# apple/ml-stable-diffusion

Measured on AMD Instinct MI355X. Metric: diffusion iter/s (UNet steps/s), SD2.1-base 512x512 fp16, higher is better.
Workload: dtype fp16; 1 GPU; BASELINE config 2: SD2.1-base (865.9 M-parameter UNet), random-init, denoising iteration at 512x512 (64x64 latents), CFG batch 2 per prompt, DDIM, device-resident loop; unet=sd21-base, latent=64, attention=ORIGINAL, prompts_per_gpu=1, global_batch=2, hip_graph=True, parallelism=dp1 (independent prompts per rank, no data-path collective)

## Files before the change

### include/sd_mi355x.h

```cpp
#ifndef SD_MI355X_H
#define SD_MI355X_H

#include <stddef.h>
#include <stdint.h>

#ifdef __cplusplus
extern "C" {
#endif

typedef enum sd_status {
  SD_OK = 0,
  SD_ERR_INVALID_ARGUMENT = -1,
  SD_ERR_NOT_FOUND = -2,
  SD_ERR_HIP = -3,
  SD_ERR_UNSUPPORTED = -4,
  SD_ERR_INTERNAL = -5
} sd_status;

typedef enum sd_dtype { SD_F16 = 0, SD_F32 = 1 } sd_dtype;

typedef enum sd_attention_impl {
  SD_ATTN_ORIGINAL = 0,
  SD_ATTN_SPLIT_EINSUM = 1,
  SD_ATTN_SPLIT_EINSUM_V2 = 2
// ... 77 lines not shown
  const void* const* additional_residuals;
  int32_t num_additional_residuals;
  void* noise_pred;
  void* const* residual_outputs;
  int32_t flags;
  const float* step_noise;
} sd_unet_io;

int sd_unet_forward(sd_unet* u, const sd_unet_io* io);

int sd_unet_time_forward(sd_unet* u, int warmup, int iters, float* ms_per_iter);

int sd_unet_profile(sd_unet* u, int iters, int cap, float* ms, double* flop, char* labels, int label_bytes,
                    int* n_ops);

int sd_tune_set_candidate(int tile, int staging, int splitk);
int sd_tune_set_plan_table(const char* rows, sd_unet* u, int* n_plans);

int sd_unet_denoise_loop(sd_unet* u, const sd_unet_io* io, float* latents, int n_images, int n_steps,
                         const float* timesteps, const float* coef, const float* sample_scale, int history,
                         float guidance_scale, float* history_io, float* ms_per_step);

typedef int (*sd_progress_fn)(void* user, int step, int n_steps, const float* latents, const float* denoised);
int sd_unet_denoise_loop_progress(sd_unet* u, const sd_unet_io* io, float* latents, int n_images, int n_steps,
                                  const float* timesteps, const float* coef, const float* sample_scale, int history,
                                  float guidance_scale, float* history_io, float* ms_per_step,
                                  const float* pred , int every,
                                  sd_progress_fn fn, void* user, int* steps_done);

int sd_unet_attach_controlnets(sd_unet* u, sd_unet* const* controlnets, int n);
int sd_controlnet_set_cond(sd_unet* controlnet, const void* controlnet_cond, int flags);

int sd_vae_decoder_create(const sd_unet_config* cfg, const sd_weights* w, int device, sd_unet** out);
int sd_vae_decode(sd_unet* vae, const void* z, sd_dtype z_dtype, float* image, int flags);
int sd_vae_encoder_create(const sd_unet_config* cfg, const sd_weights* w, int device, sd_unet** out);
int sd_vae_encode(sd_unet* vae, const void* x, sd_dtype x_dtype, float* moments, int flags);
int sd_vae_encode_latents(sd_unet* vae_encoder, const void* x, sd_dtype x_dtype, const float* eps, const float* noise, int n_images,
                          float scale_factor, float sa, float sb, float* latents, int flags);
int sd_op_vae_attention(const void* q, const void* k, const void* v, void* out, int B, int S, int C, int iters, float* ms);

typedef struct sd_text_encoder_config {
  int32_t vocab_size, hidden_size, intermediate_size, num_hidden_layers, num_attention_heads;
  int32_t max_position_embeddings;
  int32_t hidden_act;
  int32_t projection_dim;
  float layer_norm_eps;
  int32_t use_graph;
} sd_text_encoder_config;
typedef struct sd_text_encoder sd_text_encoder;
int sd_text_encoder_create(const sd_text_encoder_config* cfg, const sd_weights* w, int device, sd_text_encoder** out);
void sd_text_encoder_destroy(sd_text_encoder* t);
size_t sd_text_encoder_device_bytes(const sd_text_encoder* t);
int sd_text_encoder_encode(sd_text_encoder* t, const int32_t* input_ids, int eos_index, float* last_hidden_state,
                           float* hidden_embeds, float* pooled);

int sd_op_attention(int impl, const void* q, const void* k, const void* v, void* out, int B, int heads, int d,
                    int Sq, int Sk, int variant, int iters, float* ms);
int sd_op_layernorm(const void* x, const float* weight, const float* bias, void* out, int B, int C, int S, float eps,
                    int iters, float* ms);
int sd_op_groupnorm(const void* x, const float* weight, const float* bias, void* out, int B, int C, int H, int W,
                    int groups, float eps, int silu, int iters, float* ms);
int sd_op_groupnorm_shortcut(const void* x0, const void* x1, const float* gn_weight, const float* gn_bias, const void* w, const float* bias,
                             void* out_gn, void* out_sc, int B, int C0, int C1, int H, int W, int N, int groups, float eps, int silu,
                             int side, int iters, float* ms);
int sd_op_conv2d(const void* x, const void* w, const float* bias, const void* res, void* out, int B, int Cin, int H,
                 int W, int Cout, int ksize, int stride, int upsample, int tile, int splitk, int force_generic,
                 int iters, float* ms);
int sd_op_conv2d_ex(const void* x, const void* x1, const void* w, const float* bias, const float* temb, const void* res, void* out, int B,
                    int Cin, int C1, int H, int W, int Cout, int ksize, int stride, int upsample, int pad_mode, int twin_groups,
                    const float* twin_gamma, const float* twin_beta, float twin_eps, int twin_silu, void* out_twin, int tile, int splitk,
                    int force_generic, int* plan_out, int iters, float* ms);
int sd_op_conv2d_palettized(const void* x, const void* x1, const void* lut, int nbits, const uint8_t* indices, const float* bias,
                            const void* res, void* out, int B, int Cin, int C1, int H, int W, int Cout, int ksize, int upsample, int nw,
                            int* plan_out, int iters, float* ms);
int sd_op_palette_pack(const uint8_t* indices, int Cout, int Ctot, int ksize, int nbits, uint8_t* stream, size_t* bytes);
int sd_op_conv2d_w8a8(const void* x, const void* x1, const int8_t* wq, const float* w_scale, float act_absmax, const float* bias,
                      const void* res, void* out, int B, int Cin, int C1, int H, int W, int Cout, int ksize, int upsample, int nw,
                      int* plan_out, int iters, float* ms);
int sd_op_w8a8_pack(const int8_t* wq, int Cout, int Ctot, int ksize, int8_t* stream, size_t* bytes);
int sd_op_conv2d_w8a8_halo(const void* x, const void* x1, const int8_t* wq, const float* w_scale, float act_absmax, const float* bias,
                           const float* temb, const void* res, void* out, int B, int Cin, int C1, int H, int W, int Cout, int upsample,
                           int staging, int splitk, int* plan_out, int iters, float* ms);
int sd_op_w8a8_pack_halo(const int8_t* wq, int Cout, int Ctot, int8_t* packed, size_t* bytes);
int sd_op_gemm_w8a8(const void* x, const int8_t* wq, const float* w_scale, float act_absmax, const float* bias, const void* res, void* out, int B,
                    int Cin, int H, int W, int Cout, int bm, int* plan_out, int iters, float* ms);
int sd_op_w8a8_pack_gemm(const int8_t* wq, int Cout, int K, int8_t* packed, size_t* bytes);
int sd_op_layernorm_q8(const void* x, const float* ln_weight, const float* ln_bias, float act_absmax, float eps, int8_t* xq, int M, int C,
                       int iters, float* ms);
int sd_op_geglu_w8a8(const int8_t* xq, const int8_t* wq, const float* w_scale, float act_absmax, const float* bias, void* out, int M, int C,
                     int N2, int bm, int* plan_out, int iters, float* ms);
int sd_op_w8a8_pack_geglu(const int8_t* wq, int N2, int K, int8_t* packed, size_t* bytes);
int sd_op_quantize_weight(const float* w, int Cout, size_t per_row, int8_t* q, float* w_scale, double* sq_err);
int sd_op_absmax(const void* x, size_t n, float* absmax);
int sd_op_gemm_palettized(const void* x, const void* lut, int nbits, const uint8_t* indices, const float* bias, const void* res, void* out,
                          int B, int Cin, int H, int W, int Cout, int bm, int* plan_out, int iters, float* ms);
int sd_op_palette_pack_gemm(const uint8_t* indices, int Cout, int K, int nbits, uint8_t* stream, size_t* bytes);
int sd_op_geglu_palettized(const void* x, const float* ln_weight, const float* ln_bias, const void* lut, int nbits, const uint8_t* indices,
                           const float* bias, void* out, int M, int C, int N2, float eps, int bm, int* plan_out, int iters, float* ms);
int sd_op_palette_pack_geglu(const uint8_t* indices, int N2, int K, int nbits, uint8_t* stream, size_t* bytes);
int sd_op_conv2d_groupnorm(const void* x, const void* w, const float* bias, const void* res, const float* gn_weight,
                           const float* gn_bias, void* conv_out, void* out, int B, int Cin, int H, int W, int Cout, int ksize,
                           int groups, float eps, int silu, int tile, int producer_stats, int* entries, int iters, float* ms);
int sd_op_conv2d_groupnorm_proj(const void* x, const void* w, const float* bias, const void* res, const float* gn_weight,
                                const float* gn_bias, const void* proj_w, const float* proj_bias, void* conv_out, void* out, int B,
                                int Cin, int H, int W, int Cout, int ksize, int Nproj, int groups, float eps, int fold, int tile,
                                int* entries, int iters, float* ms);
int sd_op_conv2d_groupnorm_conv3x3(const void* x, const void* w, const float* bias, const void* res, const float* gn_weight,
                                   const float* gn_bias, const void* w2, const float* bias2, const void* res2, void* conv_out, void* out,
                                   int B, int Cin, int H, int W, int Cout, int ksize, int N2, int groups, float eps, int silu, int fold,
                                   int tile, int staging2, int* entries, int iters, float* ms);
int sd_op_ffn_out_proj(const void* g, const void* w1, const float* b1, const void* res1, const void* w2, const float* b2, const void* res2,
                       void* out, float* gn_sums, int B, int C, int S, int groups, int fused, int iters, float* ms);
int sd_op_fold_linear(const void* wp, const float* bp, const void* w2, const float* b2, void* wm_out, float* bm_out, int N, int J, int K);
int sd_op_cross_attention_fused(const void* x, const float* ln_weight, const float* ln_bias, const void* wq, const void* k,
                                const void* v, void* out, int B, int heads, int Sq, int Sk, float eps, int nst, int iters,
                                float* ms);
int sd_op_cross_attention_block(const void* x, const float* ln_weight, const float* ln_bias, const void* wq, const void* k, const void* v,
                                const void* wo, const float* bo, const void* a1, const void* wo1, const float* bo1, void* out, int B, int heads,
                                int Sq, int Sk, float eps, int fused, int iters, float* ms);
int sd_op_geglu(const void* x, const void* w, const float* bias, void* out, int M, int C, int N2, int iters, float* ms);
int sd_op_geglu_ln(const void* x, const float* ln_weight, const float* ln_bias, const void* w, const float* bias, void* out, int M, int C,
                   int N2, float eps, int kernel, int iters, float* ms);
int sd_op_qkv_ln(const void* x, const float* ln_weight, const float* ln_bias, const void* w, void* out_qk, void* out_vt, int B, int HW, int C,
                 float eps, float q_scale, int vt_perm, int kernel, int iters, float* ms);
int sd_op_gn_proj_qkv(const void* x_in, const void* conv_w, const float* gn_weight, const float* gn_bias, const void* proj_w,
                      const float* proj_bias, const float* ln_weight, const float* ln_bias, const void* wqkv, void* out_h, void* out_qk,
                      void* out_vt, int B, int H, int W, int C, int groups, float gn_eps, float ln_eps, float q_scale, int vt_perm, int fused,
                      int* entries, int iters, float* ms);
int sd_op_timestep_embedding(const float* t, float* out, int n, int dim, int flip_sin_to_cos, float freq_shift);
int sd_op_posterior_noise(const float* moments, const float* eps, const float* noise, float* out, int Cz, int h, int w, int n_images,
                          float scale_factor, float sa, float sb, int iters, float* ms);
int sd_op_sched_step(const float* noise_pred, float* latents, float* hist, const float* coef, const float* pred, const float* step_noise,
                     float guidance, int cfg, int history, int n_images, int n, float* denoised, int* step_after);
int sd_op_conv_plan(int ksize, int stride, int up, int C0, int C1, int N, int B, int Ho, int Wo, int out_mode, int flags, int n_trans,
                    int n_twins, int gnf_groups, int tile, int staging, int splitk, int copies, int* plan, unsigned long long* workspace_bytes);
int sd_op_conv_plan_kernel(int ksize, int stride, int up, int C0, int C1, int N, int B, int Ho, int Wo, int out_mode, int flags, int n_trans,
                           int n_twins, int gnf_groups, int tile, int staging, int splitk, int copies, char* text, int text_bytes);
int sd_numpy_randn(uint32_t seed, double* out, size_t n);
int sd_torch_randn(uint32_t seed, double* out, size_t n);
int sd_philox_randn(uint64_t seed, uint32_t offset, double* out, size_t n);
int sd_calibrate(int device, float* out9);
int sd_selftest_mfma(void);

typedef struct sd_safety_checker_config {
  int32_t batch, image_size , patch_size , hidden_size, intermediate_size,
          num_hidden_layers, num_attention_heads, projection_dim, num_concepts ,
          num_special , hidden_act ;
  float layer_norm_eps;
  int32_t use_graph;
} sd_safety_checker_config;
typedef struct sd_safety_checker sd_safety_checker;
int sd_safety_checker_create(const sd_safety_checker_config* cfg, const sd_weights* w, int device, sd_safety_checker** out);
void sd_safety_checker_destroy(sd_safety_checker* c);
size_t sd_safety_checker_device_bytes(const sd_safety_checker* c);
int sd_safety_checker_run(sd_safety_checker* c, const void* clip_input, float adjustment, float* has_nsfw,
                          float* concept_scores, float* image_embeds, float* last_hidden_state, int flags);
float sd_safety_checker_last_ms(const sd_safety_checker* c);
int sd_op_vit_attention(const void* qkv, void* out, int B, int S, int heads, int d, int iters, float* ms);
int sd_op_safety_head(const float* image_embeds, const float* concept_embeds, const float* special_embeds,
                      const float* concept_w, const float* special_w, float adjustment, int B, int P,
                      int n_concepts, int n_special, float* has_nsfw, float* concept_scores);

typedef struct sd_image_post {
  int32_t resize_h, resize_w;
  float image_mean[3], image_std[3];
} sd_image_post;
// ... 27 lines not shown
```

### ml-stable-diffusion_amd/csrc/capi_ops.cpp

```cpp
#include <algorithm>
#include <climits>
#include <cmath>
#include <cstring>
#include <initializer_list>

#include "capi_util.h"
#include "conv_plan.h"
#include "weight_prep.h"

namespace sd {
namespace {

const half_t* f16(const void* p) { return reinterpret_cast<const half_t*>(p); }

half_t* upload_nhwc(Scratch& sc, const void* x, int B, int C, int H, int W) {
  const half_t* src = f16(x);
  std::vector<half_t> t((size_t)B * C * H * W);
  for (int b = 0; b < B; ++b)
    for (int c = 0; c < C; ++c)
      for (int p = 0; p < H * W; ++p) t[((size_t)b * H * W + p) * C + c] = src[((size_t)b * C + c) * H * W + p];
  return sc.dev<half_t>(t.size(), t.data());
}
half_t* upload_tokens(Scratch& sc, const void* x, int B, int C, int S) { return upload_nhwc(sc, x, B, C, 1, S); }

// ... 429 lines not shown
    conv2d_op(x, w, bias, res, out, B, Cin, H, W, Cout, ksize, stride, upsample, tile, splitk, force_generic, iters, ms, e);
  });
}

int sd_op_conv2d_palettized(const void* x, const void* x1, const void* lut, int nbits, const uint8_t* indices, const float* bias,
                            const void* res, void* out, int B, int Cin, int C1, int H, int W, int Cout, int ksize, int upsample, int nw,
                            int* plan_out, int iters, float* ms) {
  return guarded([&] {
    SD_REQUIRE(lut && indices, kInvalidArgument, "NULL argument");
    SD_REQUIRE(palette_bits_ok(nbits), kInvalidArgument, "conv2d_palettized: nbits = %d, not one of 1, 2, 4, 6, 8", nbits);
    SD_REQUIRE(nw == 0 || nw == 4 || nw == 8, kInvalidArgument, "conv2d_palettized: nw = %d, not 0, 4 or 8", nw);
    SD_REQUIRE(B > 0 && Cin > 0 && C1 >= 0 && Cout > 0 && H > 0 && W > 0, kInvalidArgument, "conv2d_palettized: empty problem");
    ConvOpExtra e;
    e.x1 = x1; e.C1 = C1;
    e.plan_out = plan_out;
    e.cw.kind = WeightSource::PalWstream; e.cw.lut = lut; e.cw.indices = indices; e.cw.bits = nbits;
    e.nw = nw;
    conv2d_op(x, nullptr, bias, res, out, B, Cin, H, W, Cout, ksize, 1, upsample, 0, 0, 0, iters, ms, e);
  });
}

int sd_op_conv2d_w8a8(const void* x, const void* x1, const int8_t* wq, const float* w_scale, float act_absmax, const float* bias,
                      const void* res, void* out, int B, int Cin, int C1, int H, int W, int Cout, int ksize, int upsample, int nw,
                      int* plan_out, int iters, float* ms) {
  return guarded([&] {
    SD_REQUIRE(x && wq && w_scale && out, kInvalidArgument, "NULL argument");
    SD_REQUIRE(nw == 0 || nw == 4 || nw == 8, kInvalidArgument, "conv2d_w8a8: nw = %d, not 0, 4 or 8", nw);
    SD_REQUIRE(B > 0 && Cin > 0 && C1 >= 0 && Cout > 0 && H > 0 && W > 0 && (C1 == 0 || x1), kInvalidArgument, "conv2d_w8a8: empty problem");
    SD_REQUIRE((ksize == 1 || ksize == 3) && (upsample == 0 || upsample == 1), kInvalidArgument, "conv2d_w8a8: ksize %d upsample %d", ksize, upsample);
    ConvDesc d;
    d.C0 = Cin;
    if (C1 > 0) d.x1 = f16(x1), d.C1 = C1;
    d.B = B; d.Hi = H; d.Wi = W; d.Ho = H * (upsample ? 2 : 1); d.Wo = W * (upsample ? 2 : 1);
    d.ksize = ksize; d.up = upsample ? 2 : 1; d.N = Cout;
    SD_REQUIRE(conv_fast_path_ok(d) && wstream_shape_ok(d), kInvalidArgument,
               "conv2d_w8a8: shape not eligible for plan tile 17 (wstream.hip: k=%d C0=%d C1=%d N=%d %dx%d)", ksize, Cin, C1, Cout, d.Ho, d.Wo);
    (void)w8a8_host_copy("conv2d_w8a8", wq, w_scale, act_absmax, Cout, Cin + C1, ksize);
    ConvOpExtra e;
    e.x1 = x1; e.C1 = C1;
    e.plan_out = plan_out;
    e.cw.kind = WeightSource::I8Wstream; e.cw.q = wq; e.cw.w_scale = w_scale; e.cw.act_absmax = act_absmax;
    e.nw = nw;
    conv2d_op(x, nullptr, bias, res, out, B, Cin, H, W, Cout, ksize, 1, upsample, 0, 0, 0, iters, ms, e);
  });
}

int sd_op_conv2d_w8a8_halo(const void* x, const void* x1, const int8_t* wq, const float* w_scale, float act_absmax, const float* bias, const float* temb,
                           const void* res, void* out, int B, int Cin, int C1, int H, int W, int Cout, int upsample, int staging, int splitk, int* plan_out,
                           int iters, float* ms) {
  return guarded([&] {
    SD_REQUIRE(x && wq && w_scale && out, kInvalidArgument, "NULL argument");
    SD_REQUIRE(B > 0 && Cin > 0 && C1 >= 0 && Cout > 0 && H > 0 && W > 0 && (C1 == 0 || x1), kInvalidArgument, "conv2d_w8a8_halo: empty problem");
    SD_REQUIRE((upsample == 0 || upsample == 1) && staging >= 0 && staging <= 5 && staging != 1 && splitk >= 0, kInvalidArgument,
               "conv2d_w8a8_halo: upsample %d staging %d (plan tile 7's ring codes 0, 2-5) splitk %d", upsample, staging, splitk);
    ConvDesc d;
    d.C0 = Cin;
    if (C1 > 0) d.x1 = f16(x1), d.C1 = C1;
    d.B = B; d.Hi = H; d.Wi = W; d.Ho = H * (upsample ? 2 : 1); d.Wo = W * (upsample ? 2 : 1);
    d.ksize = 3; d.up = upsample ? 2 : 1; d.N = Cout;
    SD_REQUIRE(conv_fast_path_ok(d) && halo_ks_ok(d), kInvalidArgument,
               "conv2d_w8a8_halo: shape not eligible for plan tile 18 (conv3x3_halo_i8.hip: C0=%d C1=%d N=%d %dx%d)", Cin, C1, Cout, d.Ho, d.Wo);
    SD_REQUIRE(Cin + C1 <= kHaloI8MaxCtot, kInvalidArgument, "conv2d_w8a8_halo: %d input channels, the exact int32 sums of plan tile 18 hold up to %d",
               Cin + C1, kHaloI8MaxCtot);
    (void)w8a8_host_copy("conv2d_w8a8_halo", wq, w_scale, act_absmax, Cout, Cin + C1, 3, WeightSource::I8Halo);
    ConvOpExtra e;
    e.x1 = x1; e.C1 = C1;
    e.temb = temb;
    e.plan_out = plan_out;
    e.cw.kind = WeightSource::I8Halo; e.cw.q = wq; e.cw.w_scale = w_scale; e.cw.act_absmax = act_absmax;
    e.nw = staging;
    conv2d_op(x, nullptr, bias, res, out, B, Cin, H, W, Cout, 3, 1, upsample, 0, splitk, 0, iters, ms, e);
  });
}

int sd_op_w8a8_pack_halo(const int8_t* wq, int Cout, int Ctot, int8_t* packed, size_t* bytes) {
  return guarded([&] {
    SD_REQUIRE(wq && bytes, kInvalidArgument, "NULL argument");
    SD_REQUIRE(Cout > 0 && Ctot > 0 && Ctot % 64 == 0, kInvalidArgument, "w8a8_pack_halo: Cout %d Ctot %d", Cout, Ctot);
    *bytes = (size_t)Cout * Ctot * 9;
    if (packed) halo_i8_pack(wq, Cout, Ctot, 3, packed);
  });
}

int sd_op_gemm_w8a8(const void* x, const int8_t* wq, const float* w_scale, float act_absmax, const float* bias, const void* res, void* out, int B,
                    int Cin, int H, int W, int Cout, int bm, int* plan_out, int iters, float* ms) {
  return guarded([&] {
    SD_REQUIRE(bm == 0 || bm == 32 || bm == 64, kInvalidArgument, "gemm_w8a8: bm = %d, not 0, 32 or 64", bm);
    SD_REQUIRE(x && wq && w_scale && out && plan_out, kInvalidArgument, "NULL argument");
    SD_REQUIRE(B > 0 && Cin > 0 && Cout > 0 && H > 0 && W > 0, kInvalidArgument, "gemm_w8a8: empty problem");
    ConvDesc d;
    d.C0 = Cin;
    d.B = B; d.Hi = H; d.Wi = W; d.Ho = H; d.Wo = W;
    d.N = Cout;
    const int code = conv_plan_pin(WeightSource::I8Gemm, bm).staging;
    SD_REQUIRE(conv_fast_path_ok(d) && smgemm_shape_ok(d, code), kInvalidArgument,
               "gemm_w8a8: shape not eligible for plan tile 19 (smgemm_i8.hip: Cin=%d Cout=%d M=%d bm=%d - Cin a multiple of 64, Cout of 80, M of the "
               "tile height, at least 2 x 2 tiles and a multiple of 8 of them)", Cin, Cout, B * H * W, bm);
    SD_REQUIRE(smgemm_i8_shape_ok(d, code), kInvalidArgument, "gemm_w8a8: K = %d, the exact int32 sums of plan tile 19 hold up to %d", Cin, kSmI8MaxK);
    (void)w8a8_host_copy("gemm_w8a8", wq, w_scale, act_absmax, Cout, Cin, 1, WeightSource::I8Gemm);
    Scratch sc;
    d.x0 = upload_nhwc(sc, x, B, Cin, H, W);
    d.bias = bias ? sc.dev<float>(Cout, bias) : nullptr;
    if (res) d.res = upload_nhwc(sc, res, B, Cout, H, W);
    half_t* dout = sc.dev<half_t>((size_t)B * H * W * Cout);
    d.out = dout;
    HostWeights h;
    h.kind = WeightSource::I8Gemm; h.q = wq; h.w_scale = w_scale; h.act_absmax = act_absmax;
    upload_compressed(sc, d, "gemm_w8a8", h, bm);
    const ConvPlan p = conv_plan(d);
    plan_out[0] = p.tile; plan_out[1] = p.staging; plan_out[2] = p.splitk; plan_out[3] = p.slab ? 1 : 0;
    ConvWorkspace ws;
    sc.timed(iters, ms, [&] { launch_conv(d, ws, sc.stream); });
    download_nchw(dout, out, B, Cout, H, W);
  });
}

int sd_op_w8a8_pack_gemm(const int8_t* wq, int Cout, int K, int8_t* packed, size_t* bytes) {
  return guarded([&] {
    SD_REQUIRE(wq && bytes, kInvalidArgument, "NULL argument");
    SD_REQUIRE(Cout > 0 && K > 0 && Cout % 16 == 0 && K % 64 == 0, kInvalidArgument, "w8a8_pack_gemm: Cout %d K %d", Cout, K);
    *bytes = smgemm_i8_bytes(Cout, K);
    if (packed) smgemm_i8_pack(wq, Cout, K, packed);
  });
}

int sd_op_layernorm_q8(const void* x, const float* ln_weight, const float* ln_bias, float act_absmax, float eps, int8_t* xq, int M, int C,
                       int iters, float* ms) {
  return guarded([&] {
    SD_REQUIRE(x && xq, kInvalidArgument, "NULL argument");
    SD_REQUIRE(M > 0 && C > 0, kInvalidArgument, "layernorm_q8: empty problem");
    SD_REQUIRE((ln_weight == nullptr) == (ln_bias == nullptr), kInvalidArgument, "layernorm_q8: ln_weight and ln_bias go together");
    SD_REQUIRE(C % 8 == 0 && C <= 2048, kInvalidArgument, "layernorm_q8: C = %d, not a multiple of 8 up to 2048", C);
    SD_REQUIRE(w8a8_absmax_ok(act_absmax), kInvalidArgument, "layernorm_q8: act_absmax = %g, not a positive finite number", (double)act_absmax);
    const float inv_s = 1.0f / (act_absmax / 127.0f);
    SD_REQUIRE(std::isfinite(inv_s) && inv_s > 0.f, kInvalidArgument, "layernorm_q8: act_absmax = %g has no finite inverse scale", (double)act_absmax);
    Scratch sc;
    const half_t* dx = sc.dev<half_t>((size_t)M * C, f16(x));
    const float* dw = ln_weight ? sc.dev<float>(C, ln_weight) : nullptr;
    const float* db = ln_bias ? sc.dev<float>(C, ln_bias) : nullptr;
    int8_t* dq = sc.dev<int8_t>((size_t)M * C);
    sc.timed(iters, ms, [&] { launch_layernorm_q8(dx, dw, db, dq, M, C, eps, inv_s, sc.stream); });
    SD_HIP(hipMemcpy(xq, dq, (size_t)M * C, hipMemcpyDeviceToHost));
  });
}

int sd_op_geglu_w8a8(const int8_t* xq, const int8_t* wq, const float* w_scale, float act_absmax, const float* bias, void* out, int M, int C,
                     int N2, int bm, int* plan_out, int iters, float* ms) {
  return guarded([&] {
    SD_REQUIRE(bm == 0 || bm == 128 || bm == 256, kInvalidArgument, "geglu_w8a8: bm = %d, not 0, 128 or 256", bm);
    SD_REQUIRE(xq && wq && w_scale && out && plan_out, kInvalidArgument, "NULL argument");
    SD_REQUIRE(M > 0 && C > 0 && N2 > 0, kInvalidArgument, "geglu_w8a8: empty problem");
    ConvDesc d = token_gemm(nullptr, C, nullptr, nullptr, nullptr, nullptr, 1, M, N2);
    d.out_mode = kOutGeglu;
    const int code = conv_plan_pin(WeightSource::I8Geglu, bm).staging;
    SD_REQUIRE(conv_fast_path_ok(d) && smgeglu_shape_ok(d, code), kInvalidArgument,
               "geglu_w8a8: shape not eligible for plan tile 20 (smgeglu_i8.hip: M=%d C=%d N2=%d bm=%d - C a multiple of 64, N2 of 160, M of the "
               "tile height, at least 2 x 2 tiles and a multiple of 8 of them)", M, C, N2, bm);
    SD_REQUIRE(smgeglu_i8_shape_ok(d, code), kInvalidArgument, "geglu_w8a8: K = %d, the exact int32 sums of plan tile 20 hold up to %d", C, kSmI8MaxK);
    (void)w8a8_host_copy("geglu_w8a8", wq, w_scale, act_absmax, N2, C, 1, WeightSource::I8Geglu);
    for (size_t i = 0; i < (size_t)M * C; ++i)
      SD_REQUIRE(xq[i] != -128, kInvalidArgument, "geglu_w8a8: activation value -128 at element %zu, the symmetric range is [-127, 127]", i);
    Scratch sc;
    d.x0_i8 = sc.dev<int8_t>((size_t)M * C, xq);
    if (bias) {
      std::vector<float> bi(N2);
      for (int o = 0; o < N2; ++o) bi[geglu_row(o, N2)] = bias[o];
// ... 631 lines not shown
    half_t* dvt = sc.dev<half_t>((size_t)B * C * HW);
    half_t* dwp_t = sc.dev<half_t>((size_t)C * C);
    half_t* dwq_t = sc.dev<half_t>((size_t)N * C);
    launch_xattn_out_retile_nk(dwp, dwp_t, C, C, sc.stream);
    launch_xattn_out_retile_nk(fq.w, dwq_t, N, C, sc.stream);
    ConvDesc pd = conv_desc(dnorm, C, dwp, dpb, nullptr, dh, B, H, W, C);
    ConvDesc qd = qkv_desc(dh, fq, ln_eps, dqk, dvt, B, H, W, C, q_scale, vt_perm);
    SD_REQUIRE(conv_fast_path_ok(d) && conv_fast_path_ok(pd) && conv_fast_path_ok(qd), kInvalidArgument, "gn_proj_qkv: off the MFMA path");
    ConvWorkspace ws = workspace_for(sc, {d, pd, qd});
    int n_entries = 0;
    static const bool want_clk = tune_env_set("SD_GQ_CLOCK");
    const size_t n_clk = (size_t)(M / 32) * 5 * 16;
    long long* dclk = want_clk && fused ? sc.dev<long long>(n_clk) : nullptr;
    sc.timed(iters, ms, [&] {
      n_entries = launch_conv(d, ws, sc.stream);
      const bool have = n_entries >= 1 && n_entries <= 128;
      if (fused) {
        GnProjQkvDesc g;
        g.clk = dclk;
        g.tok = fused == 2 ? 64 : (fused == 3 ? 32 : 0);
        g.x = dx;
        if (have) {
          g.gn_partial = partial; g.gn_gamma = dgw; g.gn_beta = dgb; g.gn_entries = n_entries;
        } else {
          launch_groupnorm(dx, C, nullptr, 0, partial, dgw, dgb, dnorm, B, HW, groups, gn_eps, 0, sc.stream, n_entries);
          g.x = dnorm;
        }
        g.gn_groups = groups; g.gn_eps = gn_eps;
        g.wp_t = dwp_t; g.p_bias = dpb; g.h = dh;
        g.wqkv_t = dwq_t; g.qkv_bias = fq.bias; g.qkv_colsum = fq.colsum; g.ln_eps = ln_eps;
        g.qk = dqk; g.vt = dvt; g.M = M; g.C = C; g.S = HW; g.ldT = HW; g.vt_perm = vt_perm != 0; g.q_scale = q_scale;
        launch_gn_proj_qkv(g, sc.stream);
      } else {
        launch_groupnorm(dx, C, nullptr, 0, partial, dgw, dgb, dnorm, B, HW, groups, gn_eps, 0, sc.stream, n_entries);
        launch_conv(pd, ws, sc.stream);
        launch_conv(qd, ws, sc.stream);
      }
    });
    if (entries) *entries = (fused && n_entries >= 1 && n_entries <= 128) ? n_entries : 0;
    if (dclk) {
      std::vector<long long> hc(n_clk);
      SD_HIP(hipMemcpy(hc.data(), dclk, n_clk * sizeof(long long), hipMemcpyDeviceToHost));
      static const char* names[13] = {"start -> group statistics folded", "-> constants in LDS", "-> normalised tile in LDS", "-> proj_in MFMAs issued",
                                      "-> h tile in LDS", "-> q MFMAs", "-> q stored", "-> k MFMAs", "-> k stored", "-> v MFMAs", "-> V^T stored", "", ""};
      const size_t nw = n_clk / 16;
      double total = 0;
      for (int ph = 1; ph <= 11; ++ph) {
        double sum = 0, mx = 0;
        for (size_t w = 0; w < nw; ++w) {
          const double dlt = (double)(hc[w * 16 + ph] - hc[w * 16 + ph - 1]);
          sum += dlt;
          mx = std::max(mx, dlt);
        }
        total += sum / nw;
        fprintf(stderr, "gn_proj_qkv phase %2d  mean %8.0f  max %8.0f cycles   %s\n", ph, sum / nw, mx, names[ph - 1]);
      }
      fprintf(stderr, "gn_proj_qkv mean wave %8.0f cycles (%zu waves; the XCDs' counters are not synchronised: no launch-wide span)\n", total, nw);
    }
    SD_HIP(hipMemcpy(out_h, dh, (size_t)M * C * 2, hipMemcpyDeviceToHost));
    SD_HIP(hipMemcpy(out_qk, dqk, (size_t)M * 2 * C * 2, hipMemcpyDeviceToHost));
    SD_HIP(hipMemcpy(out_vt, dvt, (size_t)B * C * HW * 2, hipMemcpyDeviceToHost));
  });
}

static ConvPlan query_conv_plan(int ksize, int stride, int up, int C0, int C1, int N, int B, int Ho, int Wo, int out_mode, int flags, int n_trans,
                                int n_twins, int gnf_groups, int tile, int staging, int splitk, int copies, ConvWeightCopies& c) {
  SD_REQUIRE(ksize >= 1 && stride >= 1 && up >= 1 && C0 >= 1 && C1 >= 0 && N >= 1 && B >= 1 && Ho >= 1 && Wo >= 1 &&
                 n_trans >= 0 && n_twins >= 0 && n_twins <= 2 && gnf_groups >= 0 && copies >= -1 && copies <= 7,
             kInvalidArgument, "bad conv_plan arguments");
  static const float present[4] = {};
  const half_t* ph = reinterpret_cast<const half_t*>(present);
  ConvDesc d;
  d.x0 = d.w = ph;
  d.C0 = C0;
  if (C1 > 0) d.x1 = ph, d.C1 = C1;
  d.B = B; d.Ho = Ho; d.Wo = Wo; d.Hi = Ho * stride / up; d.Wi = Wo * stride / up;
  d.ksize = ksize; d.stride = stride; d.up = up; d.N = N; d.out_mode = out_mode;
  if (flags & 1) d.ln_colsum = present;
  if (flags & 2) d.temb = present;
  if (flags & 4) d.res = ph;
  if (flags & 8) d.gn_partial = const_cast<float*>(present), d.gn_groups = 32;
  if (flags & 16) d.bias = present;
  if (flags & 32) d.pad = 0;
  if (n_trans > 0) d.out_t = const_cast<half_t*>(ph), d.n_trans = n_trans, d.ldT = Ho * Wo;
  d.n_twins = n_twins;
  if (gnf_groups > 0) {
    d.gnf_partial = d.gnf_gamma = d.gnf_beta = present;
    d.gnf_groups = gnf_groups;
    d.gnf_entries = 1;
    d.gnf_silu = ksize == 3 ? 1 : 0;
  }
  d.tile = tile; d.staging = staging; d.splitk = splitk;
  if (tile == 17) {
    d.w = nullptr;
    d.cw.kind = WeightSource::I8Wstream;
    d.cw.stream = d.cw.scale = present;
    d.cw.inv_s = 1.f;
  }
  if (tile == 18) {
    d.w = nullptr;
    d.cw.kind = WeightSource::I8Halo;
    d.cw.stream = d.cw.scale = present;
    d.cw.inv_s = 1.f;
  }
  if (tile == 19) {
    d.w = nullptr;
    d.cw.kind = WeightSource::I8Gemm;
    d.cw.stream = d.cw.scale = present;
    d.cw.inv_s = 1.f;
  }
  if (tile == 20) {
    d.w = nullptr;
    d.cw.kind = WeightSource::I8Geglu;
    d.cw.stream = d.cw.scale = present;
    d.cw.inv_s = 1.f;
    d.x0_i8 = reinterpret_cast<const int8_t*>(present);
  }
  c = conv_plan_copies(d);
  if (copies < 0) copies = (c.wstream ? 1 : 0) | (c.wsgemm ? 2 : 0) | (c.bvgemm ? 4 : 0);
  if (copies & 1) d.w_tiled = ph;
  if (copies & 2) d.w_ws = ph;
  if (copies & 4) d.w_bv = ph;
  return conv_plan(d);
}

int sd_op_conv_plan(int ksize, int stride, int up, int C0, int C1, int N, int B, int Ho, int Wo, int out_mode, int flags, int n_trans,
                    int n_twins, int gnf_groups, int tile, int staging, int splitk, int copies, int* plan, unsigned long long* workspace_bytes) {
  return guarded([&] {
    SD_REQUIRE(plan && workspace_bytes, kInvalidArgument, "bad conv_plan arguments");
    ConvWeightCopies c;
    const ConvPlan p = query_conv_plan(ksize, stride, up, C0, C1, N, B, Ho, Wo, out_mode, flags, n_trans, n_twins, gnf_groups, tile, staging, splitk, copies, c);
    plan[0] = p.tile; plan[1] = p.staging; plan[2] = p.splitk; plan[3] = p.slab ? 1 : 0;
    plan[4] = c.wstream ? 1 : 0; plan[5] = c.wsgemm ? 1 : 0; plan[6] = c.bvgemm ? 1 : 0;
    *workspace_bytes = p.workspace_bytes;
  });
}

int sd_op_conv_plan_kernel(int ksize, int stride, int up, int C0, int C1, int N, int B, int Ho, int Wo, int out_mode, int flags, int n_trans,
                           int n_twins, int gnf_groups, int tile, int staging, int splitk, int copies, char* text, int text_bytes) {
  return guarded([&] {
    SD_REQUIRE(text && text_bytes >= 1, kInvalidArgument, "bad conv_plan_kernel arguments");
    ConvWeightCopies c;
    const std::string name = conv_plan_kernel_name(
        query_conv_plan(ksize, stride, up, C0, C1, N, B, Ho, Wo, out_mode, flags, n_trans, n_twins, gnf_groups, tile, staging, splitk, copies, c));
    SD_REQUIRE((int)name.size() < text_bytes, kInvalidArgument, "conv_plan_kernel: the text buffer holds %d bytes, the line needs %zu", text_bytes, name.size() + 1);
    memcpy(text, name.c_str(), name.size() + 1);
  });
}

int sd_op_timestep_embedding(const float* t, float* out, int n, int dim, int flip_sin_to_cos, float freq_shift) {
  return guarded([&] {
    SD_REQUIRE(t && out && n > 0 && dim > 0 && dim % 2 == 0, kInvalidArgument, "bad arguments");
    SD_REQUIRE(flip_sin_to_cos == 1, kUnsupported, "flip_sin_to_cos=False is not on the path");
    Scratch sc;
    float* dt = sc.dev<float>(n, t);
    float* dout = sc.dev<float>((size_t)n * dim);
    std::vector<float> f = timestep_freq_table(dim, freq_shift);
    float* df = sc.dev<float>(f.size(), f.data());
    launch_timestep_embedding(dt, df, dout, n, dim, sc.stream);
    SD_HIP(hipStreamSynchronize(sc.stream));
    SD_HIP(hipMemcpy(out, dout, (size_t)n * dim * sizeof(float), hipMemcpyDeviceToHost));
  });
}

int sd_op_posterior_noise(const float* moments, const float* eps, const float* noise, float* out, int Cz, int h, int w, int n_images,
                          float scale_factor, float sa, float sb, int iters, float* ms) {
// ... 440 lines not shown
```

### ml-stable-diffusion_amd/csrc/conv_plan.cpp

```cpp
#include "conv_plan.h"

#include <algorithm>
#include <cstring>

namespace sd {

namespace {

constexpr int BK = kConvBK;

struct Dims {
  int Ctot, M, N, K, HoWo, nk_total, tiles_x, tiles_y;
};
Dims dims_of(const ConvDesc& d) {
  Dims a;
  a.Ctot = d.C0 + (d.x1 ? d.C1 : 0);
  a.M = d.B * d.Ho * d.Wo;
  a.N = d.N;
  a.K = d.ksize * d.ksize * a.Ctot;
  a.HoWo = d.Ho * d.Wo;
  a.nk_total = a.K / BK;
  a.tiles_x = cdiv(d.Wo, 16);
  a.tiles_y = cdiv(d.Ho, 8);
  return a;
// ... 104 lines not shown
    tile_dims(c, bm, bn);
    if (geglu && c != 1 && c != 4) return false;
    if (d.out_t && d.n_trans % bn != 0) return false;
    return true;
  };
  if (!tile_ok(p.tile)) p.tile = 0;
  auto blocks_of = [&](int c) {
    int bm, bn;
    tile_dims(c, bm, bn);
    const long mt = is_halo(c) ? (long)d.B * a.tiles_x * a.tiles_y : cdiv(a.M, bm);
    return mt * cdiv(a.N, bn);
  };
  auto ksteps = [&](int c) { return is_halo(c) ? a.Ctot / BK : a.nk_total; };
  auto max_split = [&](int c) {
    const int per_min = is_halo(c) ? 2 : 16;
    int s = 1;
    while (split_ok && s < 16 && ksteps(c) / (s * 2) >= per_min) s *= 2;
    return s;
  };
  const bool pinned = p.tile != 0 || p.splitk != 0 || p.staging != 0 || i8_halo(d);
  if (i8_halo(d)) p.tile = 7;
  if (!pinned && g_tune.tile != 0 && tile_ok(g_tune.tile)) {
    p.tile = g_tune.tile;
    p.staging = g_tune.staging;
    p.splitk = g_tune.splitk;
  } else if (!pinned) {
    auto match = [&](const TunedConv& t) { return table_match(t, d, a) && tile_ok(t.tile); };
    const TunedConv* hit = nullptr;
    for (const TunedConv& t : runtime_table())
      if (!hit && match(t)) hit = &t;
    for (int i = 0; i < kNumTuned && !hit; ++i)
      if (match(kTuned[i])) hit = &kTuned[i];
    if (hit) {
      p.tile = hit->tile;
      p.staging = hit->staging;
      p.splitk = hit->splitk;
    }
  }
  if (p.tile == 0 && tile_ok(9) && d.ksize == 3 && a.HoWo <= 64 && a.M <= 256) p.tile = 9;
  if (p.tile == 9) {
    p.splitk = 1;
    return p;
  }
  if (p.tile == 0 && tile_ok(7)) {
    p.tile = 7;
    if (p.staging == 0) p.staging = 3;
  }
  if (p.tile == 0) {
    p.tile = 3;
    for (int c : {1, 2, 4, 3}) {
      if (!tile_ok(c)) continue;
      if (blocks_of(c) * max_split(c) >= 384 || c == 3) { p.tile = c; break; }
    }
    if (!tile_ok(p.tile)) p.tile = 4;
  }
  if (p.splitk == 0) {
    p.splitk = 1;
    const int ms = max_split(p.tile);
    const long want = p.tile == 7 ? 192 : 384;
    while (blocks_of(p.tile) * p.splitk < want && p.splitk < ms) p.splitk *= 2;
  }
  if (!split_ok) p.splitk = 1;
  if (p.splitk > ksteps(p.tile)) p.splitk = ksteps(p.tile);
  if (p.splitk < 1) p.splitk = 1;
  return p;
}

bool plan_is_wstream(const ConvDesc& d0) {
  if (!wstream_shape_ok(d0)) return false;
  ConvDesc d = d0;
  static const half_t present = 0;
  d.w_tiled = &present;
  return choose_plan(d, dims_of(d)).tile == 9;
}

}

bool halo_ks_ok(const ConvDesc& d) {
  const int c1 = d.x1 ? d.C1 : 0;
  return d.ksize == 3 && d.stride == 1 && (d.up == 1 || d.up == 2) && d.pad < 0 && d.out_mode == kOutHalf && d.Wo >= 8 && d.Ho >= 8 &&
         d.C0 % BK == 0 && c1 % BK == 0 && d.N % 4 == 0;
}

bool gemm_pipe_ok(int ksize, int stride, int up, int M, int N, int K, int C0, int C1) {
  const size_t lim = (size_t)1 << 31;
  return ksize == 1 && stride == 1 && up == 1 && (size_t)M * std::max(C0, C1) * 2 < lim && (size_t)N * K * 2 < lim;
}

bool conv_fast_path_ok(const ConvDesc& d) {
  const int c1 = d.x1 ? d.C1 : 0;
  if (d.C0 % BK != 0 || c1 % BK != 0) return false;
  if (d.N % 4 != 0) return false;
  if (d.out_mode == kOutGeglu && d.N % 64 != 0) return false;
  if (!(d.ksize == 1 || d.ksize == 3)) return false;
  if (!(d.up == 1 || d.up == 2)) return false;
  return true;
}

namespace {

ConvPlan plan_codes(const ConvDesc& d) {
  const CompressedWeights& cw = d.cw;
  if (i8_halo(d))
    SD_REQUIRE(conv_fast_path_ok(d) && cw.stream && cw.scale && halo_i8_ok(d), kInvalidArgument,
               "plan tile 18 (conv3x3_halo_i8.hip, int8) needs the int8 weights, the scales and a 3x3 / stride-1 shape of the halo conv with "
               "at most %d input channels (k=%d stride=%d up=%d C0=%d C1=%d N=%d)", kHaloI8MaxCtot, d.ksize, d.stride, d.up, d.C0, d.x1 ? d.C1 : 0, d.N);
  if (i8_gemm(d))
    SD_REQUIRE(conv_fast_path_ok(d) && cw.stream && cw.scale && d.staging >= 0 && d.staging <= 2 && smgemm_i8_shape_ok(d, d.staging), kInvalidArgument,
               "plan tile 19 (smgemm_i8.hip, int8) needs the int8 weights, the scales and a single-source shape of the small-M GEMM with K <= %d "
               "(k=%d C0=%d C1=%d N=%d M=%d mode=%d)", kSmI8MaxK, d.ksize, d.C0, d.x1 ? d.C1 : 0, d.N, d.B * d.Ho * d.Wo, d.out_mode);
  if (i8_geglu(d))
    SD_REQUIRE(conv_fast_path_ok(d) && cw.stream && cw.scale && d.staging >= 0 && d.staging <= 2 && smgeglu_i8_shape_ok(d, d.staging), kInvalidArgument,
               "plan tile 20 (smgeglu_i8.hip, int8) needs the int8 weights, the scales and an un-folded shape of the GEGLU kernel with K <= %d "
               "(k=%d C0=%d C1=%d N=%d M=%d mode=%d ln=%d)", kSmI8MaxK, d.ksize, d.C0, d.x1 ? d.C1 : 0, d.N, d.B * d.Ho * d.Wo, d.out_mode, d.ln_colsum ? 1 : 0);
  if (!conv_fast_path_ok(d)) return ConvPlan{-1, 0, 1, false, 0};
  switch (cw.kind) {
    case WeightSource::Fp16: break;
    case WeightSource::PalWstream:
    case WeightSource::I8Wstream: {
      const bool i8 = i8_stream(d);
      SD_REQUIRE(cw.stream && (i8 ? cw.scale != nullptr : cw.lut != nullptr) && can_split(d) && wstream_shape_ok(d), kInvalidArgument, "%s",
                 i8 ? "plan tile 17 (wstream.hip, int8) needs the int8 stream, the scales and a shape of the weight stream"
                    : "plan tile 14 (wstream.hip, palettized) needs the index stream, the LUT and a shape of the weight stream");
      ConvPlan r{i8 ? 17 : 14, d.staging, 1, true, 0};
      r.splitk = wstream_splits(d, wstream_waves(d.staging));
      r.workspace_bytes = slab_bytes(dims_of(d), r.splitk, true);
      return r;
    }
    case WeightSource::I8Halo: {
      const Dims a = dims_of(d);
      const Plan p = choose_plan(d, a);
      ConvPlan r{18, p.staging, 1, true, 0};
      const int steps = a.Ctot / BK;
      r.splitk = cdiv(steps, cdiv(steps, p.splitk));
      r.slab = r.splitk > 1 || d.n_twins > 0;
      r.workspace_bytes = slab_bytes(a, r.splitk, r.slab);
      return r;
    }
    case WeightSource::PalGemm:
      SD_REQUIRE(cw.stream && cw.lut && palette_bits_ok(cw.bits) && !d.x1 && d.staging >= 0 && d.staging <= 2 && smgemm_shape_ok(d, d.staging), kInvalidArgument,
                 "plan tile 15 (smgemm.hip, palettized) needs the index stream, the LUT and a single-source shape of the small-M GEMM");
      return ConvPlan{15, smgemm_bm(d, d.staging) == 32 ? 1 : 2, 1, false, 0};
    case WeightSource::I8Gemm:
      return ConvPlan{19, smgemm_bm(d, d.staging) == 32 ? 1 : 2, 1, false, 0};
    case WeightSource::PalGeglu:
      SD_REQUIRE(cw.stream && cw.lut && palette_bits_ok(cw.bits) && (cw.ln_gamma != nullptr) == (d.ln_colsum != nullptr) && smgeglu_pal_shape_ok(d, d.staging),
                 kInvalidArgument,
                 "plan tile 16 (smgeglu.hip, palettized) needs the index stream, the LUT, the norm weight with the LayerNorm fold and a shape of "
                 "the GEGLU kernel with 128-row tiles");
      return ConvPlan{16, 1, 1, false, 0};
    case WeightSource::I8Geglu:
      return ConvPlan{20, smgeglu_bm(d, d.staging) == 128 ? 1 : 2, 1, false, 0};
  }
  const Switches& sw = switches();
  const bool free_choice = d.tile == 0 && d.splitk == 0 && d.staging == 0 && g_tune.tile == 0;
  if (d.w_ws && wsgemm_shape_ok(d) && (d.tile == 10 || (sw.wsgemm && free_choice && wsgemm_wanted(d)))) return ConvPlan{10, 0, 1, false, 0};
  SD_REQUIRE(d.tile != 10, kInvalidArgument, "plan tile 10 (wsgemm.hip) needs the pre-tiled weights and an eligible GEGLU shape");
  if (sw.bvgemm && d.w_bv && free_choice && bvgemm_wanted(d)) return ConvPlan{11, 0, 1, false, 0};
  if (d.tile == 11) {
    SD_REQUIRE(d.w_bv && bvgemm_shape_ok(d), kInvalidArgument, "plan tile 11 (bvgemm.hip) needs the pre-tiled weights and an eligible 1x1 shape");
    return ConvPlan{11, d.staging, 1, false, 0};
  }
  if (d.tile == 12 || (sw.smgemm && free_choice && smgemm_wanted(d))) return ConvPlan{12, d.tile == 12 ? d.staging : 0, 1, false, 0};
  if (d.tile == 13 || (sw.smgeglu && free_choice && smgeglu_wanted(d))) return ConvPlan{13, d.tile == 13 ? d.staging : 0, 1, false, 0};

  const Dims a = dims_of(d);
  Plan p = choose_plan(d, a);
  const bool twins = d.n_twins > 0;
  if (d.gnf_partial && d.ksize == 3) {
    SD_REQUIRE(conv_gn_loader_ok(d) && d.gnf_silu == 1 && d.gnf_gamma && d.gnf_beta && d.gnf_entries >= 1 && d.gnf_entries <= 128 && !twins, kInvalidArgument,
               "GroupNorm in the conv loader: Ctot=%d groups=%d entries=%d up=%d", a.Ctot, d.gnf_groups, d.gnf_entries, d.up);
    p.tile = 7;
    if (p.staging != 2 && p.staging != 3) p.staging = 3;
    p.splitk = 1;
  } else if (d.gnf_partial) {
    SD_REQUIRE(d.ksize == 1 && d.stride == 1 && !d.x1 && d.out_mode == kOutHalf && !d.ln_colsum && !d.out_t && !twins &&
                   gemm_pipe_ok(d.ksize, d.stride, d.up, a.M, a.N, a.K, d.C0, 0) &&
                   d.gnf_gamma && d.gnf_beta && d.gnf_groups >= 1 && d.gnf_groups <= 32 && a.K % d.gnf_groups == 0 && a.K <= 2048 &&
                   d.gnf_entries >= 1 && d.gnf_entries <= 128 && a.HoWo % 64 == 0,
               kInvalidArgument, "GroupNorm fold: K=%d groups=%d entries=%d HoWo=%d", a.K, d.gnf_groups, d.gnf_entries, a.HoWo);
    p.tile = 3;
    if (p.staging != 6 && p.staging != 7 && p.staging != 8) p.staging = 6;
    p.splitk = 1;
  }
  ConvPlan r{p.tile, p.staging, 1, true, 0};
  if (p.tile == 9) {
    r.splitk = wstream_splits(d, wstream_waves(p.staging));
  } else {
    const int steps = p.tile == 7 ? a.Ctot / BK : a.nk_total;
    r.splitk = cdiv(steps, cdiv(steps, p.splitk));
    r.slab = r.splitk > 1 || twins;
  }
  r.workspace_bytes = slab_bytes(a, r.splitk, r.slab);
  return r;
}

void decode_plan(const ConvDesc& d, ConvPlan& p) {
  const Dims a = dims_of(d);
  int code = p.staging;
  switch (p.tile) {
    case -1: p.kernel = ConvKernel::Generic; return;
    case 9: case 14: case 17:
      p.kernel = p.tile == 9 ? ConvKernel::Wstream : p.tile == 14 ? ConvKernel::WstreamPal : ConvKernel::WstreamI8;
      p.waves = wstream_waves(code);
      return;
    case 10: p.kernel = ConvKernel::Wsgemm; return;
    case 11:
      p.kernel = ConvKernel::Bvgemm;
      p.variant = code >= 1 && code <= 6 ? code : bvgemm_auto_variant(d);
      return;
    case 12: case 15: case 19:
      p.kernel = p.tile == 12 ? ConvKernel::Smgemm : p.tile == 15 ? ConvKernel::SmgemmPal : ConvKernel::SmgemmI8;
      p.bm = code >= 0 && code <= 2 ? smgemm_bm(d, code) : 0;
      return;
    case 13: case 16: case 20:
      p.kernel = p.tile == 13 ? ConvKernel::Smgeglu : p.tile == 16 ? ConvKernel::SmgegluPal : ConvKernel::SmgegluI8;
      p.bm = code >= 0 && code <= 2 ? smgeglu_bm(d, code) : 0;
      return;
    default: break;
  }
  if (p.tile == 18) {
    tile_dims(7, p.bm, p.bn);
    p.kernel = ConvKernel::HaloI8;
    p.stages = code >= 3 ? 4 : code == 2 ? 3 : 2;
    return;
  }
  tile_dims(p.tile, p.bm, p.bn);
  if (p.tile == 7) {
    p.kernel = ConvKernel::HaloKs;
    if (d.gnf_partial) p.stages = code >= 3 && halo_gnl_lds_bytes(4, a.Ctot) <= kLdsBudget ? 4 : 3;
    else p.stages = code >= 5 ? 8 : code == 4 ? 6 : code == 3 ? 4 : code == 2 ? 3 : 2;
    return;
  }
  p.kernel = ConvKernel::Igemm;
  p.stages = 2;
  const bool lnf = d.ln_colsum != nullptr;
  auto fits = [&](int nst, int kgroups = 1) { return ring_fits(p.bm, p.bn, nst, kgroups); };
  if (lnf && code == 1) code = 0;
  if (code == 1) {
    p.reg_staged = true;
    return;
  }
  if (!lnf && d.out_mode == kOutHalfT) {
    if (code >= 2) p.stages = 3;
    return;
  }
  if (code == 12 || code == 13) {
    const bool two_groups = !lnf && cdiv(a.nk_total, p.splitk) >= 4;
    if (two_groups && code == 13 && fits(4, 2)) p.stages = 4, p.kgroups = 2;
    else if (two_groups && fits(3, 2)) p.stages = 3, p.kgroups = 2;
    if (p.kgroups == 2) return;
    code -= 10;
  }
  if (code >= 6 && code <= 8 && gemm_pipe_ok(d.ksize, d.stride, d.up, a.M, a.N, a.K, d.C0, d.x1 ? d.C1 : 0)) {
    p.kernel = ConvKernel::GemmPipe;
    p.stages = code == 8 ? 2 : (code == 7 && fits(4)) ? 4 : 3;
    return;
  }
  if (code >= 6) code = 3;
  const int asked = code >= 5 ? 8 : code == 4 ? 6 : code == 3 ? 4 : code == 2 ? 3 : 2;
  for (int nst : {8, 6, 4, 3, 2})
    if (nst <= asked && fits(nst)) {
      p.stages = nst;
      return;
    }
}

}

ConvPlan conv_plan(const ConvDesc& d) {
  ConvPlan p = plan_codes(d);
  decode_plan(d, p);
  return p;
}

std::string conv_plan_kernel_name(const ConvPlan& p) {
  const std::string tile = std::to_string(p.bm) + "x" + std::to_string(p.bn), ring = " ring" + std::to_string(p.stages);
  switch (p.kernel) {
    case ConvKernel::Igemm: return "igemm " + tile + ring + (p.kgroups == 2 ? " kg2" : "") + (p.reg_staged ? " regs" : "");
    case ConvKernel::GemmPipe: return "gemm_pipe " + tile + ring;
    case ConvKernel::HaloKs: return "halo_ks" + ring;
    case ConvKernel::HaloI8: return "halo_i8" + ring;
    case ConvKernel::Wstream: return "wstream waves" + std::to_string(p.waves);
    case ConvKernel::WstreamPal: return "wstream_pal waves" + std::to_string(p.waves);
    case ConvKernel::WstreamI8: return "wstream_i8 waves" + std::to_string(p.waves);
    case ConvKernel::Wsgemm: return "wsgemm";
    case ConvKernel::Bvgemm: return "bvgemm v" + std::to_string(p.variant);
    case ConvKernel::Smgemm: return "smgemm bm" + std::to_string(p.bm);
    case ConvKernel::SmgemmPal: return "smgemm_pal bm" + std::to_string(p.bm);
    case ConvKernel::SmgemmI8: return "smgemm_i8 bm" + std::to_string(p.bm);
    case ConvKernel::Smgeglu: return "smgeglu bm" + std::to_string(p.bm);
    case ConvKernel::SmgegluPal: return "smgeglu_pal bm" + std::to_string(p.bm);
    case ConvKernel::SmgegluI8: return "smgeglu_i8 bm" + std::to_string(p.bm);
    default: return "generic";
  }
}

size_t conv_workspace_bytes(const ConvDesc& d) {
  if (!conv_fast_path_ok(d) || pal_gemm(d) || pal_geglu(d) || i8_gemm(d) || i8_geglu(d)) return 0;
  const Dims a = dims_of(d);
  const Plan p = choose_plan(d, a);
  int splits = (switches().tuning && can_split(d)) ? std::max(p.splitk, 16) : p.splitk;
  const bool stream = can_stream(d) || ((pal_stream(d) || i8_stream(d)) && can_split(d) && wstream_shape_ok(d));
  if (stream) splits = std::max(splits, wstream_splits(d, 4));
  return slab_bytes(a, splits, d.n_twins > 0 || stream);
}

ConvWeightCopies conv_plan_copies(const ConvDesc& d0) {
  ConvWeightCopies c{false, false, false};
  if (!conv_fast_path_ok(d0)) return c;
  ConvDesc d = d0;
  d.w_tiled = d.w_ws = d.w_bv = nullptr;
  const Switches& sw = switches();
  const int k = d.ksize, M = d.B * d.Ho * d.Wo;
  const bool ws_candidate = sw.tuning ? ((k == 3 && M <= 512) || (k == 1 && M <= 128)) : plan_is_wstream(d);
  c.wstream = sw.wstream && wstream_shape_ok(d) && ws_candidate;
  c.wsgemm = sw.wsgemm && wsgemm_wanted(d);
  c.bvgemm = sw.bvgemm && !c.wsgemm && bvgemm_wanted(d);
  return c;
}

namespace {
ConvPlan fp16_plan(const ConvDesc& d0, const ConvWeightCopies& c) {
  static const half_t present = 0;
  ConvDesc d = d0;
  d.cw = CompressedWeights{};
  d.w_tiled = c.wstream ? &present : nullptr;
  d.w_ws = c.wsgemm ? &present : nullptr;
  d.w_bv = c.bvgemm ? &present : nullptr;
  return conv_plan(d);
}
}

WeightPin conv_plan_pin(WeightSource kind, int n) {
  switch (kind) {
    case WeightSource::PalWstream: return {kind, 14, n == 4 ? 4 : 0};
    case WeightSource::I8Wstream: return {kind, 17, n == 4 ? 4 : 0};
    case WeightSource::I8Halo: return {kind, 18, n};
    case WeightSource::PalGemm: return {kind, 15, n == 32 ? 1 : n == 64 ? 2 : 0};
    case WeightSource::I8Gemm: return {kind, 19, n == 32 ? 1 : n == 64 ? 2 : 0};
    case WeightSource::PalGeglu: return {kind, 16, n == 128 ? 1 : n == 256 ? 2 : 0};
    case WeightSource::I8Geglu: return {kind, 20, n == 128 ? 1 : n == 256 ? 2 : 0};
    default: return {};
  }
}

WeightPin conv_plan_weights(const ConvDesc& d, StoredWeights held, bool opt_in) {
  if (held == StoredWeights::Fp16 || !conv_fast_path_ok(d)) return {};
  const Switches& sw = switches();
  const bool palette = held == StoredWeights::Palette, one_by_one = opt_in && palette && d.ksize == 1 && !d.x1;
  if (one_by_one && d.out_mode == kOutGeglu && sw.smgeglu) {
    const ConvPlan p = fp16_plan(d, conv_plan_copies(d));
    if (p.kernel == ConvKernel::Smgeglu && smgeglu_pal_shape_ok(d, 0)) return conv_plan_pin(WeightSource::PalGeglu, p.bm);
  }
  if (opt_in && held == StoredWeights::W8A8 && d.ksize == 1 && !d.x1 && d.out_mode == kOutGeglu && sw.smgeglu) {
    const ConvPlan p = fp16_plan(d, conv_plan_copies(d));
    ConvDesc plain = d;
    plain.ln_colsum = nullptr;
    if (p.kernel == ConvKernel::Smgeglu && smgeglu_i8_shape_ok(plain, p.bm == 128 ? 1 : 2)) return conv_plan_pin(WeightSource::I8Geglu, p.bm);
  }
  if (sw.wstream && !d.ln_colsum && plan_is_wstream(d)) {
    const ConvPlan p = fp16_plan(d, {true, false, false});
    if (p.kernel == ConvKernel::Wstream) return conv_plan_pin(palette ? WeightSource::PalWstream : WeightSource::I8Wstream, p.waves);
  }
  if (one_by_one && d.out_mode == kOutHalf && sw.smgemm && !d.ln_colsum) {
    const ConvPlan p = fp16_plan(d, conv_plan_copies(d));
    if (p.kernel == ConvKernel::Smgemm) return conv_plan_pin(WeightSource::PalGemm, p.bm);
  }
  if (opt_in && held == StoredWeights::W8A8 && d.ksize == 1 && !d.x1 && d.out_mode == kOutHalf && sw.smgemm && !d.ln_colsum) {
    const ConvPlan p = fp16_plan(d, conv_plan_copies(d));
    if (p.kernel == ConvKernel::Smgemm && smgemm_i8_shape_ok(d, 0)) return conv_plan_pin(WeightSource::I8Gemm, p.bm);
  }
  if (held == StoredWeights::W8A8 && halo_i8_ok(d)) {
    const ConvPlan p = fp16_plan(d, conv_plan_copies(d));
    if (p.kernel == ConvKernel::HaloKs) {
      WeightPin pin = conv_plan_pin(WeightSource::I8Halo, p.staging);
      pin.splitk = p.splitk;
      return pin;
    }
  }
  return {};
}

bool conv_plan_is_tuned(const ConvDesc& d) {
  if (!conv_fast_path_ok(d)) return false;
  const Dims a = dims_of(d);
  for (int i = 0; i < kNumTuned; ++i)
    if (table_match(kTuned[i], d, a)) return true;
  return false;
}

int conv_plan_table_set(const char* text) {
  std::vector<TunedConv>& t = runtime_table();
  t.clear();
  if (!text) return 0;
  const char* p = text;
  while (*p) {
    const char* e = strchr(p, '\n');
    std::string line(p, e ? (size_t)(e - p) : strlen(p));
    TunedConv r;
    if (parse_plan_row(line.c_str(), r)) t.push_back(r);
    if (!e) break;
    p = e + 1;
  }
  return (int)t.size();
}

void conv_tune_set_candidate(int tile, int staging, int splitk) {
  g_tune.tile = tile;
  g_tune.staging = staging;
  g_tune.splitk = splitk;
}

void conv_plan_log(const ConvDesc& d, const ConvPlan& p, int n_fast) {
  static const bool on = tune_env_set("SD_LOG_CONVS");
  if (!on) return;
  const Dims a = dims_of(d);
  const int c1 = d.x1 ? d.C1 : 0;
  if (p.tile == 9 || p.tile == 14 || p.tile == 17)
    fprintf(stderr, "[sd conv] k%d up%d C0=%d C1=%d M=%d N=%d K=%d tile=%d nw=%d slabs=%d twins=%d bits=%d\n", d.ksize, d.up, d.C0, c1, a.M, a.N,
            a.K, p.tile, p.waves, p.splitk, d.n_twins, p.tile == 14 ? d.cw.bits : p.tile == 17 ? 8 : 16);
  else if (p.tile == 12 || p.tile == 13)
    fprintf(stderr, "[sd conv] k1 s1 up1 C0=%d C1=%d M=%d N=%d K=%d mode=%d tile=%d bm=%d n_fast=%d\n", d.C0, c1, a.M, a.N, a.K, d.out_mode, p.tile, p.bm,
            n_fast);
  else if (p.tile == 15 || p.tile == 16)
    fprintf(stderr, "[sd conv] k1 s1 up1 C0=%d C1=%d M=%d N=%d K=%d mode=%d tile=%d bm=%d n_fast=%d bits=%d\n", d.C0, c1, a.M, a.N, a.K, d.out_mode,
            p.tile, p.bm, n_fast, d.cw.bits);
  else if (p.tile == 19 || p.tile == 20)
    fprintf(stderr, "[sd conv] k1 s1 up1 C0=%d C1=%d M=%d N=%d K=%d mode=%d tile=%d bm=%d n_fast=%d bits=8\n", d.C0, c1, a.M, a.N, a.K, d.out_mode, p.tile,
            p.bm, n_fast);
  else if (p.tile == 18)
    fprintf(stderr, "[sd conv] k%d s%d up%d C0=%d C1=%d M=%d N=%d K=%d mode=%d tile=%d splitk=%d bits=8\n", d.ksize, d.stride, d.up, d.C0, c1, a.M, a.N,
            a.K, d.out_mode, p.tile, p.splitk);
  else
    fprintf(stderr, "[sd conv] k%d s%d up%d C0=%d C1=%d M=%d N=%d K=%d mode=%d tile=%d splitk=%d\n", d.ksize, d.stride, d.up, d.C0, c1, a.M, a.N,
            a.K, d.out_mode, p.tile, p.splitk);
}

bool choose_tile_order(double a_bytes, double w_bytes, double nbm, double nbn, bool ab_switch) {
  const double l2 = 3.5e6;
  const double m_fast_cost = w_bytes + a_bytes * (a_bytes <= l2 ? std::min(8.0, nbn) : nbn);
  const double n_fast_cost = a_bytes + w_bytes * (w_bytes <= l2 ? std::min(8.0, nbm) : nbm);
  static const int forced = tune_env_int("SD_TILE_ORDER", -1);
  if (ab_switch && forced == 2) return nbn > 1 && a_bytes * (nbn - 1) > 7.0 * w_bytes;
  if (ab_switch && forced >= 0) return forced != 0;
  return nbn > 1 && n_fast_cost < m_fast_cost;
}

bool conv_reduce_stats_on() { return switches().reduce_stats; }

}
```

### ml-stable-diffusion_amd/csrc/conv_plan.h

```cpp
#pragma once
#include <string>

#include "kernels.h"

namespace sd {

enum class ConvKernel { Generic, Igemm, GemmPipe, HaloKs, HaloI8, Wstream, WstreamPal, WstreamI8, Wsgemm, Bvgemm, Smgemm, SmgemmPal, SmgemmI8, Smgeglu, SmgegluPal, SmgegluI8 };

struct ConvPlan {
  int tile;
  int staging;
  int splitk;
  bool slab;
  size_t workspace_bytes;
  ConvKernel kernel = ConvKernel::Generic;
  int bm = 0, bn = 0;
  int stages = 0;
  int kgroups = 1;
  bool reg_staged = false;
  int waves = 0;
  int variant = 0;
};
ConvPlan conv_plan(const ConvDesc& d);

struct ConvWeightCopies {
  bool wstream, wsgemm, bvgemm;
};
ConvWeightCopies conv_plan_copies(const ConvDesc& d);

enum class StoredWeights { Fp16, Palette, W8A8 };
struct WeightPin {
  WeightSource kind = WeightSource::Fp16;
  int tile = 0, staging = 0;
  int splitk = 0;
};
WeightPin conv_plan_weights(const ConvDesc& d, StoredWeights held, bool opt_in);
WeightPin conv_plan_pin(WeightSource kind, int n);

void conv_plan_log(const ConvDesc& d, const ConvPlan& p, int n_fast = 0);

std::string conv_plan_kernel_name(const ConvPlan& p);

bool choose_tile_order(double a_bytes, double w_bytes, double nbm, double nbn, bool ab_switch);

bool conv_reduce_stats_on();

constexpr int kConvBK = 64;
bool halo_ks_ok(const ConvDesc& d);
bool gemm_pipe_ok(int ksize, int stride, int up, int M, int N, int K, int C0, int C1);

constexpr size_t kLdsBudget = 160 * 1024;
constexpr size_t ring_bytes(int bm, int bn, int nst) { return (size_t)nst * (bm + bn) * kConvBK * sizeof(half_t); }
constexpr bool ring_fits(int bm, int bn, int nst, int kgroups = 1) { return kgroups * ring_bytes(bm, bn, nst) + 2 * bn * sizeof(float) <= kLdsBudget; }
constexpr int kHaloLdsRows = 184;
constexpr size_t halo_lds_bytes(int bn, int d) {
  return ((size_t)2 * kHaloLdsRows * kConvBK + (size_t)d * bn * kConvBK) * sizeof(half_t) + bn * sizeof(float);
}
constexpr size_t halo_gnl_lds_bytes(int d, int ctot) {
  const size_t k_loop = halo_lds_bytes(64, d) - 64 * sizeof(float) + (((size_t)6 * ctot + 15) & ~(size_t)15);
  const size_t epilogue = 32 * 1024 + 128 * (64 + 8) * 2 + 64 * sizeof(float);
  return k_loop > epilogue ? k_loop : epilogue;
}
constexpr int kHaloI8Pitch = 20, kHaloI8Rows = 204;
constexpr size_t halo_i8_lds_bytes(int d) {
  return (size_t)kHaloLdsRows * kConvBK * sizeof(half_t) + (size_t)2 * kHaloI8Rows * kConvBK + (size_t)d * 64 * kConvBK + 2 * 64 * sizeof(float);
}
constexpr int kHaloI8MaxCtot = 14784;
static_assert(127LL * 127 * 9 * kHaloI8MaxCtot < (1LL << 31) && 127LL * 127 * 9 * (kHaloI8MaxCtot + 64) >= (1LL << 31), "int32 bound of plan tile 18");
constexpr int kSmI8MaxK = 133120;
static_assert(127LL * 127 * kSmI8MaxK < (1LL << 31) && 127LL * 127 * (kSmI8MaxK + 64) >= (1LL << 31), "int32 bound of plan tile 19");

}
```

### ml-stable-diffusion_amd/csrc/igemm.hip

```cpp
#include "igemm_device.h"

namespace sd {

namespace {

template <int BM, int BN, int WGM, int WGN, bool TRANS_OUT, bool GLDS, int NST, int DBG = 0, bool LNF = false, int KG = 1>
__global__ __launch_bounds__(256 * KG) void igemm_kernel(IgemmArgs a) {
  static_assert(WGM * WGN == 4, "4 waves");
  static_assert(KG == 1 || (KG == 2 && GLDS && NST >= 3 && !LNF && !TRANS_OUT && DBG == 0), "in-workgroup split-K: ring variants of the plain epilogue");
  static_assert(!(LNF && TRANS_OUT), "LayerNorm fold uses the in-lane row layout of the non-transposed tile");
  constexpr int TM = BM / WGM / 32;
  constexpr int TN = BN / WGN / 32;
  constexpr int XR = BM / 32;
  constexpr int WR = BN / 32;
  constexpr int ROW = GLDS ? BK : LDS_ROW;

  const bool prof = (DBG & 4) && blockIdx.x == 0 && blockIdx.y == 0 && threadIdx.x == 0;
  long long prof_t[4];
  long long prof_w0 = 0;
  if (prof) { prof_t[0] = clock64(); prof_w0 = wall_clock64(); }
  extern __shared__ __attribute__((aligned(16))) char smem[];
  const int kg = KG > 1 ? __builtin_amdgcn_readfirstlane((int)threadIdx.x >> 8) : 0;
  half_t* Xs = reinterpret_cast<half_t*>(smem) + (size_t)kg * NST * (BM + BN) * ROW;
  half_t* Ws = Xs + NST * BM * ROW;
// ... 926 lines not shown
int launch_slab_combine(const ConvDesc& d, IgemmArgs& a, hipStream_t s) {
  a.gn_partial = nullptr;
  if (conv_reduce_stats_on() && d.gn_partial && d.gn_groups >= 1 && d.gn_groups <= 256 && a.N % d.gn_groups == 0 && (a.N / d.gn_groups) % 4 == 0 &&
      a.HoWo <= 256 && d.out_mode == kOutHalf && !d.out_t) {
    int ppb = std::max(1, a.B * a.HoWo / 512);
    const int slabs = cdiv(a.HoWo, ppb);
    const size_t lds = (size_t)ppb * (a.N / 4) * 2 * sizeof(float);
    if (slabs <= kGnMaxSlabs && lds <= 64 * 1024) {
      a.gn_partial = d.gn_partial;
      a.gn_G = d.gn_groups;
      a.gn_cpg = a.N / d.gn_groups;
      a.gn_T = slabs;
      hipLaunchKernelGGL(splitk_reduce_stats_kernel, dim3(slabs, a.B), dim3(256), lds, s, a, ppb);
      return slabs;
    }
  }
  const size_t total4 = (size_t)a.M * a.N / 4;
  const int blocks = (int)std::min<size_t>((total4 + 255) / 256, 2048);
  hipLaunchKernelGGL(splitk_reduce_kernel, dim3(blocks), dim3(256), 0, s, a);
  return 0;
}

half_t* g_zero_chunk = nullptr;

}

const half_t* device_zero_chunk() {
  if (!g_zero_chunk) {
    SD_HIP(hipMalloc(reinterpret_cast<void**>(&g_zero_chunk), 256));
    SD_HIP(hipMemset(g_zero_chunk, 0, 256));
    SD_HIP(hipDeviceSynchronize());
  }
  return g_zero_chunk;
}

const half_t* zero_chunk() {
  SD_REQUIRE(g_zero_chunk, kInternal, "conv launch before any handle allocated the zero chunk (device_zero_chunk)");
  return g_zero_chunk;
}

int launch_conv(const ConvDesc& d, const ConvWorkspace& ws, hipStream_t s) {
  SD_REQUIRE(conv_fast_path_ok(d), kInvalidArgument, "launch_conv: shape not MFMA-tileable (C0=%d C1=%d N=%d k=%d)",
             d.C0, d.C1, d.N, d.ksize);
  SD_REQUIRE(!d.ln_colsum || (d.ksize == 1 && !d.x1 && d.bias && d.out_mode != kOutHalfT), kInvalidArgument,
             "LayerNorm fold needs a 1x1 single-source GEMM with a (folded) bias");
  SD_REQUIRE(!d.out_t || (d.out_mode == kOutHalf && d.n_trans % 64 == 0 && d.n_trans < d.N && (d.Ho * d.Wo) % 8 == 0 &&
                          d.ldT % 8 == 0 && !d.res && !d.temb),
             kInvalidArgument, "fused q|k|v: n_trans %d N %d HoWo %d ldT %d", d.n_trans, d.N, d.Ho * d.Wo, d.ldT);
  SD_REQUIRE(!d.vt_perm || (d.out_t && (d.Ho * d.Wo) % 16 == 0), kInvalidArgument, "permuted V^T needs the fused q|k|v epilogue and HoWo %% 16 == 0");
  SD_REQUIRE(d.q_cols == 0 || (d.out_t && d.q_cols % 4 == 0 && d.q_cols <= d.n_trans), kInvalidArgument, "pre-scaled queries need the fused q|k|v epilogue (q_cols %d)", d.q_cols);
  const ConvPlan p = conv_plan(d);
  switch (p.kernel) {
    case ConvKernel::Wsgemm: launch_wsgemm(d, s); return 0;
    case ConvKernel::Bvgemm: launch_bvgemm(d, p, s); return 0;
    case ConvKernel::Smgemm: launch_smgemm(d, p, s); return 0;
    case ConvKernel::Smgeglu: launch_smgeglu(d, p, s); return 0;
    case ConvKernel::SmgegluPal: launch_smgeglu_pal(d, p, s); return 0;
    case ConvKernel::SmgemmPal: launch_smgemm_pal(d, p, s); return 0;
    case ConvKernel::SmgemmI8: launch_smgemm_i8(d, p, s); return 0;
    case ConvKernel::SmgegluI8: launch_smgeglu_i8(d, p, s); return 0;
    default: break;
  }
  IgemmArgs a = planned_args(d, p, ws.partial);
  const bool twins = d.n_twins > 0;
  SD_REQUIRE(!twins || (d.out_mode == kOutHalf && !d.ln_colsum && !d.out_t && !d.debug && reduce_twin_ok(a.HoWo, a.N, d.n_twins, d.twin)),
             kInvalidArgument, "GroupNorm twins need a plain fp16 output and whole (sample, group) slices (HoWo=%d N=%d)", a.HoWo, a.N);
  const bool have_ws = !p.slab || (ws.partial && ws.partial_bytes >= p.workspace_bytes);
  if (p.kernel == ConvKernel::Wstream || p.kernel == ConvKernel::WstreamPal || p.kernel == ConvKernel::WstreamI8) SD_REQUIRE(have_ws, kInternal, "wstream workspace too small (%zu < %zu)", ws.partial_bytes, p.workspace_bytes);
  SD_REQUIRE(have_ws, kInternal, "split-K workspace too small (%zu < %zu)", ws.partial_bytes, p.workspace_bytes);
  conv_plan_log(d, p);
  int gn_entries = 0;
  switch (p.kernel) {
    case ConvKernel::Wstream:
      launch_wstream(d, ws.partial, p.waves, s);
      break;
    case ConvKernel::WstreamPal:
      launch_wstream_pal(d, ws.partial, p.waves, s);
      break;
    case ConvKernel::WstreamI8:
      launch_wstream_i8(d, ws.partial, p.waves, s);
      break;
    case ConvKernel::HaloKs: gn_entries = launch_halo_ks(d, p, ws.partial, s); break;
    case ConvKernel::HaloI8: gn_entries = launch_halo_i8(d, p, ws.partial, s); break;
    case ConvKernel::Igemm:
    case ConvKernel::GemmPipe: {
      const bool trans = d.out_mode == kOutHalfT;
      set_tile_order(a, p.bm, p.bn);
      if (d.debug && d.debug < 64) {
        const bool ok = p.bm == 128 && p.bn == 128 ? launch_debug_mode<128, 128>(a, d.debug, s) : launch_debug_mode<64, 64>(a, d.debug, s);
        SD_REQUIRE(ok && !trans, kInvalidArgument, "no ablation kernel for debug mode %d", d.debug);
        return 0;
      }
      if (!trans) gn_entries = setup_gn_stats(d, a, p.bm);
      if (p.bm == 128 && p.bn == 128) launch_tile<128, 128>(a, p, trans, s);
      else if (p.bm == 128) launch_tile<128, 64>(a, p, trans, s);
      else if (p.bn == 64) launch_tile<64, 64>(a, p, trans, s);
      else launch_tile<64, 128>(a, p, trans, s);
      break;
    }
    default: SD_REQUIRE(false, kInternal, "launch_conv: plan '%s' has no launcher here", conv_plan_kernel_name(p).c_str());
  }
  if (twins) {
    launch_reduce_twin(a.partial, a.splitk, a.M, a.N, a.HoWo, a.bias, a.temb, a.temb_stride, a.res, a.out, d.n_twins, d.twin, s);
  } else if (a.slab) {
    gn_entries = launch_slab_combine(d, a, s);
  }
  SD_HIP(hipGetLastError());
  return gn_entries;
}

bool gn_side_gemm_ok(const ConvDesc& d) {
  if (!(d.ksize == 1 && d.stride == 1 && d.up == 1 && d.out_mode == kOutHalf && !d.ln_colsum && !d.out_t && d.n_twins == 0 && !d.gnf_partial &&
        !d.gn_partial && !d.temb && !d.debug && conv_fast_path_ok(d)))
    return false;
  const int M = d.B * d.Ho * d.Wo, c1 = d.x1 ? d.C1 : 0;
  return gemm_pipe_ok(d.ksize, d.stride, d.up, M, d.N, d.C0 + c1, d.C0, c1) && M >= 256;
}

namespace {
constexpr int kSideD = 4;
IgemmArgs side_args(const ConvDesc& d) {
  SD_REQUIRE(gn_side_gemm_ok(d), kInvalidArgument, "side GEMM: not a plain 1x1 GEMM of the pipelined kernel (C0=%d C1=%d N=%d)", d.C0, d.C1, d.N);
  IgemmArgs a = make_args(d);
  a.splitk = 1;
  a.slab = 0;
  set_tile_order(a, 64, 64);
  return a;
}
constexpr size_t kSideLds = (size_t)kSideD * (64 + 64) * BK * sizeof(half_t) + 2 * 64 * sizeof(float);
}

void launch_gn_apply_side(const half_t* x0, int C0, const half_t* x1, int C1, const float* partial, int entries, const float* gamma,
                          const float* beta, half_t* y, int B, int HW, int G, float eps, int silu, int slabs, int ppb, const ConvDesc& side,
                          hipStream_t s) {
  IgemmArgs a = side_args(side);
  GnSideArgs g{x0, x1, C0, x1 ? C1 : 0, partial, entries, gamma, beta, y, HW, G, eps, silu, ppb, slabs, B, 0};
  g.n_gn_pad = (slabs * B + 7) / 8 * 8;
  auto k = gn_apply_side_kernel<kSideD>;
  static DynLdsOnce once;
  once.set(k, kSideLds);
  hipLaunchKernelGGL(k, dim3(g.n_gn_pad + cdiv(a.M, 64) * cdiv(a.N, 64)), dim3(256), kSideLds, s, g, a);
  SD_HIP(hipGetLastError());
}

void launch_gn_fused_side(int vw, const half_t* x0, int C0, const half_t* x1, int C1, const float* gamma, const float* beta, half_t* y, int B,
                          int HW, int G, float eps, int silu, const ConvDesc& side, hipStream_t s) {
  IgemmArgs a = side_args(side);
  GnSideArgs g{x0, x1, C0, x1 ? C1 : 0, nullptr, 0, gamma, beta, y, HW, G, eps, silu, 0, G, B, 0};
  g.n_gn_pad = (G * B + 7) / 8 * 8;
  const dim3 grid(g.n_gn_pad + cdiv(a.M, 64) * cdiv(a.N, 64));
  static DynLdsOnce o8, o4, o2;
  if (vw == 8) {
    auto k = gn_fused_side_kernel<8, kSideD>;
    o8.set(k, kSideLds);
    hipLaunchKernelGGL(k, grid, dim3(256), kSideLds, s, g, a);
  } else if (vw == 4) {
    auto k = gn_fused_side_kernel<4, kSideD>;
    o4.set(k, kSideLds);
    hipLaunchKernelGGL(k, grid, dim3(256), kSideLds, s, g, a);
  } else {
    auto k = gn_fused_side_kernel<2, kSideD>;
    o2.set(k, kSideLds);
    hipLaunchKernelGGL(k, grid, dim3(256), kSideLds, s, g, a);
  }
  SD_HIP(hipGetLastError());
}
// ... 3 lines not shown
```

### ml-stable-diffusion_amd/csrc/igemm_device.h

```cpp
#pragma once
#include <cstdio>
#include <cstdlib>
#include <cstring>
#include <string>
#include <type_traits>

#include "conv_plan.h"

namespace sd {

const half_t* zero_chunk();

int launch_halo_ks(const ConvDesc& d, const ConvPlan& p, float* partial, hipStream_t s);
int launch_halo_i8(const ConvDesc& d, const ConvPlan& p, float* partial, hipStream_t s);

namespace {

constexpr int BK = kConvBK;
constexpr int LDS_ROW = BK + 8;

struct IgemmArgs {
  const half_t* x0;
  const half_t* x1;
  const half_t* w;
  const float* bias;
  const float* temb;
  const half_t* res;
  half_t* out;
  float* partial;
  int C0, C1, Ctot;
  int B, Hi, Wi, Ho, Wo, HoWo;
  int ksize, stride, up, pad;
  int M, N, K;
  int temb_stride;
  int nk_total, nk_per_split, splitk;
  int slab;
  int out_mode, ldT;
  int debug;
  long long* prof;
  const half_t* zeros;
  int tiles_x, tiles_y;
  const float* ln_colsum;
  float ln_eps;
  int n_trans, ldo;
  half_t* out_t;
  int vt_perm;
  int res_pre;
  float* gn_partial;
  int gn_G, gn_cpg, gn_T;
  int n_fast;
  const float* gnf_partial;
  const float* gnf_gamma;
  const float* gnf_beta;
  float gnf_eps;
  int gnf_G, gnf_entries;
  float q_scale;
  int q_cols;
};

constexpr int kGnScratchFloats = 256 * 17;

template <int BN>
__device__ __forceinline__ void tile_gn_stats(const IgemmArgs& a, float* scratch, const float (&fs)[8], const float (&fq)[8],
                                              int n_blk, int b, int mt) {
  constexpr int OWC = BN / 8;
  const int tid = threadIdx.x;
  float* chan = scratch + kGnScratchFloats;
#pragma unroll
  for (int e = 0; e < 8; ++e) {
    scratch[tid * 17 + e] = fs[e];
    scratch[tid * 17 + 8 + e] = fq[e];
  }
  __syncthreads();
  for (int cc = tid; cc < 2 * BN; cc += 256) {
    const int which = cc / BN, ch = cc - which * BN;
    const int cl = ch >> 3, e = ch & 7;
    float s = 0.f;
#pragma unroll 4
    for (int k = 0; k < 256 / OWC; ++k) s += scratch[(k * OWC + cl) * 17 + which * 8 + e];
    chan[cc] = s;
  }
  __syncthreads();
  const int g0 = n_blk / a.gn_cpg;
  const int g = g0 + tid;
  const int n_end = min(n_blk + BN, a.N);
  if (tid < BN && g < a.gn_G && g * a.gn_cpg < n_end) {
    const int gs = g * a.gn_cpg, ge = gs + a.gn_cpg;
    const int lo = max(gs, n_blk), hi = min(ge, n_end);
    float s = 0.f, q = 0.f;
    for (int c = lo; c < hi; ++c) {
      s += chan[c - n_blk];
      q += chan[BN + c - n_blk];
    }
    float* dst = a.gn_partial + (((size_t)b * a.gn_G + g) * kGnMaxSlabs + (size_t)mt * 2) * 2;
    if (gs < n_blk) {
      dst[2] = s;
      dst[3] = q;
// ... 352 lines not shown
```

### ml-stable-diffusion_amd/csrc/kernels.h

```cpp
#pragma once
#include "sd_common.h"

namespace sd {

enum OutMode : int {
  kOutHalf = 0,
  kOutHalfT = 1,
  kOutGeglu = 2,
};

struct GnTwin {
  half_t* y = nullptr;
  int ld = 0, c_off = 0;
  int cpg = 0;
  const float* gamma = nullptr;
  const float* beta = nullptr;
  float eps = 1e-5f;
  int silu = 0;
};

enum class WeightSource { Fp16, PalWstream, PalGemm, PalGeglu, I8Wstream, I8Halo, I8Gemm, I8Geglu };
struct CompressedWeights {
  WeightSource kind = WeightSource::Fp16;
  const void* stream = nullptr;
  const half_t* lut = nullptr;
  int bits = 0;
  const float* ln_gamma = nullptr;
  const float* scale = nullptr;
  float inv_s = 0.f;
  bool palettized() const { return kind == WeightSource::PalWstream || kind == WeightSource::PalGemm || kind == WeightSource::PalGeglu; }
  const uint8_t* pal() const { return palettized() ? static_cast<const uint8_t*>(stream) : nullptr; }
  bool int8() const { return kind == WeightSource::I8Wstream || kind == WeightSource::I8Halo || kind == WeightSource::I8Gemm || kind == WeightSource::I8Geglu; }
  const int8_t* i8() const { return int8() ? static_cast<const int8_t*>(stream) : nullptr; }
};

struct ConvDesc {
  const half_t* x0 = nullptr;
  const half_t* x1 = nullptr;
  const int8_t* x0_i8 = nullptr;
  int C0 = 0, C1 = 0;
  const half_t* w = nullptr;
  const float* bias = nullptr;
  const float* temb = nullptr;
  int temb_stride = 0;
  const half_t* res = nullptr;
  half_t* out = nullptr;
  int B = 1, Hi = 1, Wi = 1;
  int Ho = 1, Wo = 1;
  int ksize = 1, stride = 1, up = 1;
  int pad = -1;
  int N = 0;
  int out_mode = kOutHalf;
  int ldT = 0;
  int tile = 0;
  int splitk = 0;
  long long* prof = nullptr;
  int debug = 0;
  int staging = 0;
  const float* ln_colsum = nullptr;
  float ln_eps = 1e-5f;
  half_t* out_t = nullptr;
  int n_trans = 0;
  int vt_perm = 0;
  float q_scale = 1.f;
  int q_cols = 0;
  float* gn_partial = nullptr;
  int gn_groups = 0;
  const float* gnf_partial = nullptr;
  const float* gnf_gamma = nullptr;
  const float* gnf_beta = nullptr;
  float gnf_eps = 1e-6f;
  int gnf_groups = 0, gnf_entries = 0;
  int gnf_silu = 0;
  const half_t* w_tiled = nullptr;
  CompressedWeights cw;
  const half_t* w_ws = nullptr;
  const half_t* w_bv = nullptr;
  GnTwin twin[2];
  int n_twins = 0;
};

constexpr int kGnMaxSlabs = 256;

struct ConvWorkspace {
  float* partial = nullptr;
  size_t partial_bytes = 0;
};

size_t conv_workspace_bytes(const ConvDesc& d);
const half_t* device_zero_chunk();
int launch_conv(const ConvDesc& d, const ConvWorkspace& ws, hipStream_t s);
struct ConvPlan;
bool conv_fast_path_ok(const ConvDesc& d);
bool conv_gn_loader_ok(const ConvDesc& d);
void conv_tune_set_candidate(int tile, int staging, int splitk);
bool conv_plan_is_tuned(const ConvDesc& d);
int conv_plan_table_set(const char* text);

bool wstream_shape_ok(const ConvDesc& d);
int wstream_splits(const ConvDesc& d, int nw);
size_t wstream_tiled_halves(int N, int Ctot, int ksize);
void launch_wstream_retile(const half_t* w, half_t* wt, int N, int Ctot, int ksize, hipStream_t s);
int launch_wstream(const ConvDesc& d, float* partial, int nw, hipStream_t s);
int launch_wstream_pal(const ConvDesc& d, float* partial, int nw, hipStream_t s);
int launch_wstream_i8(const ConvDesc& d, float* partial, int nw, hipStream_t s);
bool reduce_twin_ok(int HW, int N, int n_twins, const GnTwin* tw);
void launch_reduce_twin(const float* partial, int S, int M, int N, int HW, const float* bias, const float* temb, int temb_stride,
                        const half_t* res, half_t* out, int n_twins, const GnTwin* tw, hipStream_t s);

bool wsgemm_shape_ok(const ConvDesc& d);
bool wsgemm_wanted(const ConvDesc& d);
size_t wsgemm_tiled_halves(int N);
void launch_wsgemm_retile(const half_t* w, half_t* wt, int N, bool geglu, hipStream_t s);
void launch_wsgemm(const ConvDesc& d, hipStream_t s);

bool bvgemm_shape_ok(const ConvDesc& d);
size_t bvgemm_tiled_halves(int N, int K);
void launch_bvgemm_retile(const half_t* w, half_t* wt, int N, int K, bool geglu, hipStream_t s);
void launch_bvgemm(const ConvDesc& d, const ConvPlan& p, hipStream_t s);
int bvgemm_auto_variant(const ConvDesc& d);
bool bvgemm_wanted(const ConvDesc& d);

bool smgemm_shape_ok(const ConvDesc& d, int variant);
bool smgemm_wanted(const ConvDesc& d);
void launch_smgemm(const ConvDesc& d, const ConvPlan& p, hipStream_t s);
int smgemm_bm(const ConvDesc& d, int variant);
void launch_smgemm_pal(const ConvDesc& d, const ConvPlan& p, hipStream_t s);
bool smgemm_i8_shape_ok(const ConvDesc& d, int variant);
void launch_smgemm_i8(const ConvDesc& d, const ConvPlan& p, hipStream_t s);

void launch_wfold(const half_t* wp, const float* bp, const half_t* w2, const float* b2, half_t* merged, float* bm, int N, int J, int K,
                  hipStream_t s);

bool smgeglu_shape_ok(const ConvDesc& d, int variant);
bool smgeglu_wanted(const ConvDesc& d);
int smgeglu_bm(const ConvDesc& d, int variant);
void launch_smgeglu(const ConvDesc& d, const ConvPlan& p, hipStream_t s);
size_t smgeglu_prof_entries(const ConvDesc& d, int variant);
bool smgeglu_pal_shape_ok(const ConvDesc& d, int variant);
void launch_smgeglu_pal(const ConvDesc& d, const ConvPlan& p, hipStream_t s);
bool smgeglu_i8_shape_ok(const ConvDesc& d, int variant);
void launch_smgeglu_i8(const ConvDesc& d, const ConvPlan& p, hipStream_t s);

void run_calibration(int device, float* out);

int launch_conv_generic(const ConvDesc& d, int act_silu_out, hipStream_t s);

void launch_conv_small_n(const ConvDesc& d, float* out_nchw_f32, hipStream_t s);

enum AttnImpl : int { kAttnOriginal = 0, kAttnSplitEinsum = 1, kAttnSplitEinsumV2 = 2 };

struct AttnDesc {
  const half_t* q = nullptr;
  const half_t* k = nullptr;
  const half_t* vt = nullptr;
  half_t* out = nullptr;
  int B = 1, heads = 1, d = 64, Sq = 0, Sk = 0;
  int ldq = 0, ldk = 0, ldv = 0, ldo = 0;
  int impl = kAttnOriginal;
  int variant = 0;
  int vt_perm = 0;
  int q_prescaled = 0;
// ... 199 lines not shown
```

### ml-stable-diffusion_amd/csrc/net.cpp

```cpp
#include "net.h"

#include <algorithm>
#include <type_traits>

#include "conv_plan.h"
#include "weight_prep.h"

namespace sd {

Net::Net(const sd_unet_config& cfg, const WeightStore& ws, int device)
    : cfg_(cfg), ws_(&ws), f32_(cfg.compute_fp32 != 0), pal_tensors_((int)ws.palettes()), i8_marked_((int)ws.w8a8_marks()) {
  SD_REQUIRE(cfg.n_levels >= 1 && cfg.n_levels <= SD_MAX_LEVELS, kInvalidArgument, "n_levels=%d", cfg.n_levels);
  SD_REQUIRE(cfg.batch >= 1 && cfg.height >= 1 && cfg.width >= 1, kInvalidArgument, "bad batch/size");
  SD_REQUIRE(cfg.norm_num_groups >= 1 && cfg.norm_num_groups <= 64, kUnsupported, "norm_num_groups=%d",
             cfg.norm_num_groups);
  open(device);
}

void Net::seal() {
  ll_.seal();
  ws_ = nullptr;
}

Tensor Net::new_tensor(int B, int H, int W, int C) {
  Tensor t;
  t.B = B;
  t.H = H;
  t.W = W;
  t.C = C;
  t.p = ll_.arena.alloc_n<half_t>(t.numel() * (f32_ ? 2 : 1));
  return t;
}

half_t* Net::upload_conv_weight(const std::string& name, int cout, int cin, int k, bool geglu) {
  const HostTensor& t = ws_->get(name + ".weight");
  const size_t expect = (size_t)cout * cin * k * k;
  SD_REQUIRE(t.numel() == expect, kInvalidArgument, "%s.weight has %zu elements, expected %zu (%d,%d,%d,%d)",
             name.c_str(), t.numel(), expect, cout, cin, k, k);
  std::vector<half_t> host(expect);
  retile_ohwi(t.data.data(), cout, cin, k, geglu, host.data());
  half_t* d = ll_.arena.alloc_n<half_t>(expect);
  SD_HIP(hipMemcpy(d, host.data(), expect * sizeof(half_t), hipMemcpyHostToDevice));
  return d;
}

float* Net::upload_conv_weight_f32(const std::string& name, int cout, int cin, int k) {
  const HostTensor& t = ws_->get(name + ".weight");
  const size_t expect = (size_t)cout * cin * k * k;
  SD_REQUIRE(t.numel() == expect, kInvalidArgument, "%s.weight has %zu elements, expected %zu (%d,%d,%d,%d)", name.c_str(), t.numel(), expect,
             cout, cin, k, k);
  std::vector<float> host(expect);
  retile_ohwi(t.data.data(), cout, cin, k, false, host.data());
  float* d = ll_.arena.alloc_n<float>(expect);
  SD_HIP(hipMemcpy(d, host.data(), expect * sizeof(float), hipMemcpyHostToDevice));
  return d;
}

float* Net::upload_vec(const std::string& name, int n, bool geglu) {
  const HostTensor& t = ws_->get(name);
  SD_REQUIRE((int)t.numel() == n, kInvalidArgument, "%s has %zu elements, expected %d", name.c_str(), t.numel(), n);
  std::vector<float> host(t.data);
  if (geglu)
    for (int o = 0; o < n; ++o) host[geglu_row(o, n)] = t.data[o];
  float* d = ll_.arena.alloc_n<float>(n);
  SD_HIP(hipMemcpy(d, host.data(), (size_t)n * sizeof(float), hipMemcpyHostToDevice));
  return d;
}

namespace {
struct ConvGeom {
  int Ho, Wo, pad;
};
ConvGeom conv_geom(const std::string& name, const Tensor& x, const ConvArgs& a) {
  const int Hup = x.H * a.up, Wup = x.W * a.up, pad = a.k / 2;
  if (a.pad >= 0) {
    SD_REQUIRE(a.pad == 0 && a.stride == 2 && a.k == 3, kUnsupported, "%s: explicit padding %d", name.c_str(), a.pad);
    return {(Hup + 1 - a.k) / a.stride + 1, (Wup + 1 - a.k) / a.stride + 1, 0};
  }
  return {(Hup + 2 * pad - a.k) / a.stride + 1, (Wup + 2 * pad - a.k) / a.stride + 1, -1};
}
}

Tensor Net::conv(std::vector<Op>& ops, const std::string& name, const Tensor& x, const ConvArgs& a) {
  if (f32_) return conv_f32(ops, name, x, a);
  const int cin = x.C + (a.x2 ? a.x2->C : 0);
  const bool geglu = a.out_mode == kOutGeglu;
  const float* b = a.bias ? upload_vec(name + ".bias", a.cout, geglu) : nullptr;
  const WeightPin pin = weight_plan(name, x, a, false);
  const WeightSource could = ws_->observe() && !ws_->palette(name + ".weight") && !a.silu_out
                                 ? conv_plan_weights(conv_shape(name, x, a), StoredWeights::W8A8, ws_->observe_gemms() && a.keep_compressed).kind
                                 : WeightSource::Fp16;
  if (could == WeightSource::I8Wstream || (could == WeightSource::I8Halo && ws_->observe() >= 2) || could == WeightSource::I8Gemm) {
    float* slot = ll_.arena.alloc_n<float>(1);
    observed_.push_back({name + ".weight", slot});
    const half_t *p0 = x.p, *p1 = a.x2 ? a.x2->p : nullptr;
    const size_t n0 = x.numel(), n1 = a.x2 ? a.x2->numel() : 0;
    ops.push_back([=](hipStream_t s) { launch_absmax_half(p0, n0, p1, n1, slot, s); });
    ops.back().label = "absmax " + name;
  }
  if (pin.kind != WeightSource::Fp16) return conv_w(ops, name, upload_compressed(name, pin, cin, a), b, x, a);
  return conv_w(ops, name, upload_conv_weight(name, a.cout, cin, a.k, geglu), b, x, a);
}

WeightPin Net::weight_plan(const std::string& name, const Tensor& x, const ConvArgs& a, bool ln) const {
  if (f32_ || a.silu_out) return {};
  const StoredWeights held = ws_->palette(name + ".weight") ? StoredWeights::Palette
                             : ws_->w8a8(name + ".weight")  ? StoredWeights::W8A8
                                                            : StoredWeights::Fp16;
  ConvDesc d = conv_shape(name, x, a);
  static const float present = 0.f;
  if (ln) d.ln_colsum = d.bias = &present;
  return conv_plan_weights(d, held, a.keep_compressed);
}

bool Net::observes_geglu(const std::string& name, const Tensor& x, const ConvArgs& a, bool ln) const {
  if (f32_ || !ws_->observe() || !ws_->observe_geglus() || ws_->palette(name + ".weight") || a.out_mode != kOutGeglu) return false;
  ConvDesc d = conv_shape(name, x, a);
  static const float present = 0.f;
  if (ln) d.ln_colsum = d.bias = &present;
  return conv_plan_weights(d, StoredWeights::W8A8, a.keep_compressed).kind == WeightSource::I8Geglu;
}

void Net::observe_tensor(std::vector<Op>& ops, const std::string& name, const Tensor& t) {
  float* slot = ll_.arena.alloc_n<float>(1);
  observed_.push_back({name + ".weight", slot});
  const half_t* p0 = t.p;
  const size_t n0 = t.numel();
  ops.push_back([=](hipStream_t s) { launch_absmax_half(p0, n0, nullptr, 0, slot, s); });
  ops.back().label = "absmax " + name;
}

ConvWeights Net::upload_compressed(const std::string& name, const WeightPin& pin, int cin, const ConvArgs& a, const std::string& ln_name) {
  const std::string wname = name + ".weight";
  const size_t expect = (size_t)a.cout * cin * a.k * a.k;
  auto up = [this](const auto* host, size_t n) {
    auto* d = ll_.arena.alloc_n<std::remove_cv_t<std::remove_pointer_t<decltype(host)>>>(n);
    SD_HIP(hipMemcpy(d, host, n * sizeof(*host), hipMemcpyHostToDevice));
    return d;
  };
  size_t bytes = 0;
  CompressedWeights cw;
  if (pin.kind == WeightSource::I8Wstream || pin.kind == WeightSource::I8Halo || pin.kind == WeightSource::I8Gemm ||
      pin.kind == WeightSource::I8Geglu) {
    const W8A8Mark* i8 = ws_->w8a8(wname);
    SD_REQUIRE(i8 && ws_->get(wname).numel() == expect && i8->q.size() == expect && i8->w_scale.size() == (size_t)a.cout, kInvalidArgument,
               "%s: expected %zu W8A8 values (%d,%d,%d,%d)", wname.c_str(), expect, a.cout, cin, a.k, a.k);
    cw = upload_w8a8(up, pin.kind, wname.c_str(), i8->q.data(), i8->w_scale.data(), i8->act_absmax, a.cout, cin, a.k, &bytes);
    ++i8_applied_;
    i8_bytes_ += bytes;
    i8_names_.push_back(wname);
  } else {
    const Palette* pal = ws_->palette(wname);
    SD_REQUIRE(pal && ws_->get(wname).numel() == expect && pal->indices.size() == expect, kInvalidArgument,
               "%s has %zu elements, expected %zu (%d,%d,%d,%d)", wname.c_str(), ws_->get(wname).numel(), expect, a.cout, cin, a.k, a.k);
    SD_REQUIRE(palette_bits_ok(pal->nbits) && pal->lut.size() == (size_t)1 << pal->nbits, kInternal, "%s: a palette of %zu entries for %d bits",
               wname.c_str(), pal->lut.size(), pal->nbits);
    cw = upload_palettized(up, pin.kind, wname.c_str(), reinterpret_cast<const half_t*>(pal->lut.data()), pal->nbits, pal->indices.data(), a.cout,
                           cin, a.k, &bytes);
    if (!ln_name.empty()) cw.ln_gamma = upload_vec(ln_name + ".weight", cin);
    ++pal_streamed_;
    pal_stream_bytes_ += bytes;
  }
  return ConvWeights(cw, pin);
}

int Net::activation_range(int index, std::string* name, float* absmax) {
  if (index < 0 || index >= (int)observed_.size()) return (int)observed_.size();
  SD_HIP(hipSetDevice(ll_.device));
  SD_HIP(hipStreamSynchronize(ll_.stream));
  SD_HIP(hipMemcpy(absmax, observed_[(size_t)index].second, sizeof(float), hipMemcpyDeviceToHost));
  *name = observed_[(size_t)index].first;
  return (int)observed_.size();
}

Tensor Net::conv_f32(std::vector<Op>& ops, const std::string& name, const Tensor& x, const ConvArgs& a) {
  const int cout = a.cout, k = a.k;
  const float* b = a.bias ? upload_vec(name + ".bias", cout) : nullptr;
  SD_REQUIRE(!a.x2 && !a.temb && !a.ln_colsum && a.out_mode == kOutHalf && !a.silu_out, kInternal, "%s: not a VAE conv", name.c_str());
  const float* w = upload_conv_weight_f32(name, cout, x.C, k);
  const ConvGeom g = conv_geom(name, x, a);
  Tensor out = new_tensor(x.B, g.Ho, g.Wo, cout);
  ConvF32Desc fd;
  fd.x = x.f();
  fd.w = w;
  fd.w_kind = 1;
  fd.bias = b;
  fd.res = reinterpret_cast<const float*>(a.res);
  fd.out = out.f();
  fd.B = x.B; fd.Hi = x.H; fd.Wi = x.W; fd.Cin = x.C; fd.Ho = g.Ho; fd.Wo = g.Wo; fd.N = cout;
  fd.ksize = k; fd.stride = a.stride; fd.up = a.up; fd.pad = g.pad;
  ops.push_back([fd](hipStream_t s) { launch_conv_f32(fd, s); });
  char buf[256];
  snprintf(buf, sizeof(buf), "conv%dx%d fp32 %d->%d @%dx%d %s", k, k, x.C, cout, g.Ho, g.Wo, name.c_str());
  ops.back().label = buf;
  ops.back().flop = 2.0 * x.B * g.Ho * g.Wo * (double)cout * x.C * k * k;
  return out;
}

ConvDesc Net::conv_shape(const std::string& name, const Tensor& x, const ConvArgs& a) const {
  const Tensor* x2 = a.x2;
  const bool ln = a.ln_colsum != nullptr;
  ConvDesc d;
  d.x0 = x.p;
  d.C0 = x.C;
  if (x2) {
    SD_REQUIRE(x2->B == x.B && x2->H == x.H && x2->W == x.W, kInternal, "%s: concat shape mismatch", name.c_str());
    d.x1 = x2->p;
    d.C1 = x2->C;
  }
  d.temb = a.temb;
  d.temb_stride = kTembCap;
  d.res = a.res;
  d.B = x.B;
  d.Hi = x.H;
  d.Wi = x.W;
  const ConvGeom g = conv_geom(name, x, a);
  d.Ho = g.Ho;
  d.Wo = g.Wo;
  d.pad = g.pad;
  d.ksize = a.k;
  d.stride = a.stride;
  d.up = a.up;
  d.N = a.cout;
  d.out_mode = a.out_mode;
  d.ldT = a.ldT;
  d.ln_colsum = a.ln_colsum;
  d.x0_i8 = a.x_i8;
  if (ln) {
    d.vt_perm = a.vt_perm ? 1 : 0;
    d.q_scale = a.q_scale;
    d.q_cols = a.q_cols;
  }
  return d;
}

Tensor Net::conv_w(std::vector<Op>& ops, const std::string& name, const ConvWeights& weights, const float* bias, const Tensor& x, const ConvArgs& a) {
  const Tensor* x2 = a.x2;
  const int cout = a.cout, k = a.k;
  const bool geglu = a.out_mode == kOutGeglu, ln = a.ln_colsum != nullptr;
  const half_t* w = weights.w;
  ConvDesc d = conv_shape(name, x, a);
  d.w = w;
  d.bias = bias;
  d.cw = weights.cw;
  d.tile = weights.pin.tile;
  d.staging = weights.pin.staging;
  d.splitk = weights.pin.splitk;
  Tensor out;
  if (ln && a.n_trans > 0) {
    out = new_tensor(x.B, d.Ho, d.Wo, a.n_trans);
    *a.vt_out = ll_.arena.alloc_n<half_t>((size_t)x.B * (cout - a.n_trans) * a.ldT);
    d.out_t = *a.vt_out;
    d.n_trans = a.n_trans;
  } else if (a.out_mode == kOutHalfT) {
    out.B = x.B; out.H = 1; out.W = a.ldT; out.C = cout;
    out.p = ll_.arena.alloc_n<half_t>((size_t)x.B * cout * a.ldT);
  } else {
    out = new_tensor(x.B, d.Ho, d.Wo, geglu ? cout / 2 : cout);
  }
  d.out = out.p;
  SD_REQUIRE(!ln || (conv_fast_path_ok(d) && !a.silu_out), kInternal, "%s: LayerNorm fold / fused q|k|v off the MFMA path",
             name.c_str());
  std::shared_ptr<GnHook> hook;
  if (a.out_mode == kOutHalf && !(ln && a.n_trans > 0)) {
    hook = std::make_shared<GnHook>();
    out.gn = hook;
    hook->ops_pos = (int)ops.size();
    hook->ops_list = &ops;
  }
  auto with_hook = [hook](const ConvDesc& d0) {
    ConvDesc dd = d0;
    if (hook) {
      dd.gn_partial = hook->partial;
      dd.gn_groups = hook->groups;
    }
    return dd;
  };
  const int cin = x.C + (x2 ? x2->C : 0);
  if (conv_fast_path_ok(d) && !a.silu_out) {
    const ConvWeightCopies copies = d.cw.kind != WeightSource::Fp16 ? ConvWeightCopies{false, false, false} : conv_plan_copies(d);
    if (copies.wstream && !ln) {
      half_t* wt = ll_.arena.alloc_n<half_t>(wstream_tiled_halves(cout, cin, k));
      launch_wstream_retile(w, wt, cout, cin, k, ll_.stream);
      d.w_tiled = wt;
    }
    if (copies.wsgemm) {
      half_t* wt = ll_.arena.alloc_n<half_t>(wsgemm_tiled_halves(cout));
      launch_wsgemm_retile(w, wt, cout, geglu, ll_.stream);
      d.w_ws = wt;
    }
    if (copies.bvgemm) {
      half_t* wt = ll_.arena.alloc_n<half_t>(bvgemm_tiled_halves(cout, x.C));
      launch_bvgemm_retile(w, wt, cout, x.C, geglu, ll_.stream);
      d.w_bv = wt;
    }
    ll_.ws_need = std::max(ll_.ws_need, conv_workspace_bytes(d));
    ops.push_back([this, d, hook, with_hook](hipStream_t s) {
      const int n = launch_conv(with_hook(d), ll_.ws_conv, s);
      if (hook) hook->produced(n);
    });
  } else {
    const int so = a.silu_out ? 1 : 0;
    ops.push_back([d, so, hook, with_hook](hipStream_t s) {
      const int n = launch_conv_generic(with_hook(d), so, s);
      if (hook) hook->produced(n);
    });
  }
  char buf[320];
  const int kind = d.out_t ? 3 : (geglu ? 2 : (ln ? 1 : 0));
  const WeightSource src = d.cw.kind;
  const std::string lnmark = ln ? "+ln" : "", palmark = "+pal" + std::to_string(d.cw.bits);
  const std::string mark = src == WeightSource::PalGeglu ? palmark + lnmark : lnmark + (d.cw.i8() ? "+w8a8" : src != WeightSource::Fp16 ? palmark : "");
  snprintf(buf, sizeof(buf), "%s%s %d->%d @%dx%d M=%d K=%d %s #%d,%d,%d,%d,%d,%d,%d",
           k == 3 ? "conv3x3" : (geglu ? (src == WeightSource::PalGeglu ? "geglu" : "geglu1x1") : "gemm1x1"), mark.c_str(), cin, cout, d.Ho, d.Wo,
           x.B * d.Ho * d.Wo, cin * k * k, name.c_str(), kind, k, a.stride, a.up, cin, cout, x.B * d.Ho * d.Wo);
  ops.back().label = buf;
  ops.back().flop = 2.0 * x.B * d.Ho * d.Wo * (double)cout * cin * k * k;
  return out;
}

void Net::conv_small_n(std::vector<Op>& ops, const std::string& name, const Tensor& x, int cout, half_t* out_nhwc, float* out_nchw) {
  if (f32_) {
    ConvF32Desc fd;
    fd.x = x.f(); fd.w = upload_conv_weight_f32(name, cout, x.C, 3); fd.w_kind = 1; fd.bias = upload_vec(name + ".bias", cout);
    fd.out = out_nhwc ? reinterpret_cast<float*>(out_nhwc) : new_tensor(x.B, x.H, x.W, cout).f();
    fd.B = x.B; fd.Hi = x.H; fd.Wi = x.W; fd.Cin = x.C; fd.Ho = x.H; fd.Wo = x.W; fd.N = cout; fd.ksize = 3;
    ops.push_back([=](hipStream_t s) {
      launch_conv_f32(fd, s);
      if (out_nchw) launch_nhwc_to_nchw_f32f32(fd.out, out_nchw, fd.B, fd.N, fd.Ho, fd.Wo, s);
    });
  } else {
    ConvDesc d;
    d.x0 = x.p;
    d.C0 = x.C;
    d.w = upload_conv_weight(name, cout, x.C, 3, false);
    d.bias = upload_vec(name + ".bias", cout);
    d.out = out_nhwc;
    d.B = x.B; d.Hi = x.H; d.Wi = x.W; d.Ho = x.H; d.Wo = x.W;
    d.ksize = 3; d.stride = 1; d.up = 1; d.N = cout;
    ops.push_back([=](hipStream_t s) { launch_conv_small_n(d, out_nchw, s); });
  }
  ops.back().label = "conv3x3 small-N " + name + (out_nchw ? " -> fp32 NCHW" : "");
  ops.back().flop = 2.0 * x.M() * (double)cout * x.C * 9;
}

Tensor Net::group_norm_f32(std::vector<Op>& ops, const std::string& name, const Tensor& x, float eps, bool silu) {
  const int C = x.C, G = cfg_.norm_num_groups;
  void* scratch = ll_.arena.alloc(groupnorm_f32_scratch_bytes(x.B, G));
  const float* gamma = upload_vec(name + ".weight", C);
  const float* beta = upload_vec(name + ".bias", C);
  Tensor y = new_tensor(x.B, x.H, x.W, C);
  const float* xp = x.f();
  float* yp = y.f();
  const int B = x.B, HW = x.H * x.W, si = silu ? 1 : 0;
  ops.push_back([=](hipStream_t s) { launch_groupnorm_f32(xp, scratch, gamma, beta, yp, B, HW, C, G, eps, si, s); });
  ops.back().label = "groupnorm fp32 C=" + std::to_string(C) + " @" + std::to_string(x.H) + "x" + std::to_string(x.W) + " " + name;
  return y;
}

Tensor Net::group_norm(std::vector<Op>& ops, const std::string& name, const Tensor& x, const Tensor* x2, float eps,
                       bool silu, const ConvDesc* side, const std::string& side_label, double side_flop) {
  SD_REQUIRE(!side || !f32_, kInternal, "%s: side GEMM on the fp32 path", name.c_str());
  const int C = x.C + (x2 ? x2->C : 0);
  const int G = cfg_.norm_num_groups;
  SD_REQUIRE(C % G == 0, kUnsupported, "%s: %d channels not divisible by %d groups", name.c_str(), C, G);
  if (f32_) {
    SD_REQUIRE(!x2, kInternal, "%s: concat GroupNorm on the fp32 path", name.c_str());
    return group_norm_f32(ops, name, x, eps, silu);
  }
  const float* gamma = upload_vec(name + ".weight", C);
  const float* beta = upload_vec(name + ".bias", C);
  Tensor y = new_tensor(x.B, x.H, x.W, C);
  float* partial = ll_.arena.alloc_n<float>(groupnorm_scratch_floats(x.B, x.H * x.W, G));
  const half_t* p0 = x.p;
  const half_t* p1 = x2 ? x2->p : nullptr;
  const int C0 = x.C, C1 = x2 ? x2->C : 0, B = x.B, HW = x.H * x.W, si = silu ? 1 : 0;
  half_t* yp = y.p;
  std::shared_ptr<GnHook> hook;
  if (!x2 && x.gn && !x.gn->partial && groupnorm_wants_producer_stats(HW, C, G)) {
    SD_REQUIRE(x.gn->ops_list == &ops && x.gn->ops_pos >= 0 && x.gn->ops_pos < (int)ops.size(), kInternal,
               "%s: GroupNorm producer statistics need the producing op earlier in the same launch list", name.c_str());
    hook = x.gn;
    hook->partial = partial;
    hook->groups = G;
  }
  const std::string label = "groupnorm C=" + std::to_string(C) + " @" + std::to_string(x.H) + "x" + std::to_string(x.W) + " " + name;
  if (side) {
    const ConvDesc sd = *side;
    ops.push_back([=](hipStream_t s) {
      launch_groupnorm(p0, C0, p1, C1, partial, gamma, beta, yp, B, HW, G, eps, si, s, hook ? hook->consume() : 0, &sd);
    });
    ops.back().label = label + " || " + side_label;
    ops.back().flop = side_flop;
    return y;
  }
// ... 154 lines not shown
```

### ml-stable-diffusion_amd/csrc/net.h

```cpp
#pragma once
#include "../../include/sd_mi355x.h"
#include "conv_plan.h"
#include "launch_list.h"

namespace sd {

constexpr int kTembCap = 65536;
inline int round_up(int x, int a) { return (x + a - 1) / a * a; }

struct GnHook {
  float* partial = nullptr;
  int groups = 0;
  int entries = 0;
  bool fresh = false;
  void produced(int n) {
    entries = n;
    fresh = true;
  }
  int consume() {
    const int n = fresh ? entries : 0;
    fresh = false;
    return n;
  }
  int ops_pos = -1;
  const void* ops_list = nullptr;
};

struct Tensor {
  half_t* p = nullptr;
  int B = 0, H = 0, W = 0, C = 0;
  std::shared_ptr<GnHook> gn;
  int M() const { return B * H * W; }
  size_t numel() const { return (size_t)B * H * W * C; }
  float* f() const { return reinterpret_cast<float*>(p); }
};

struct OpTime {
  std::string label;
  double flop;
  float ms;
};

struct ConvArgs {
  const Tensor* x2 = nullptr;
  int cout = 0;
  int k = 1, stride = 1, up = 1;
  bool bias = true;
  const float* temb = nullptr;
  const half_t* res = nullptr;
  int out_mode = kOutHalf;
  int ldT = 0;
  bool silu_out = false;
  int pad = -1;
  const float* ln_colsum = nullptr;
  int n_trans = 0;
  half_t** vt_out = nullptr;
  bool vt_perm = false;
  float q_scale = 1.f;
  int q_cols = 0;
  bool keep_compressed = false;
  const int8_t* x_i8 = nullptr;
};

struct ConvWeights {
  const half_t* w = nullptr;
  CompressedWeights cw;
  WeightPin pin;
  ConvWeights(const half_t* fp16) : w(fp16) {}
  ConvWeights(const CompressedWeights& c, const WeightPin& p) : cw(c), pin(p) {}
};

class Net {
 public:
  virtual ~Net() { close(); }
  Net(const Net&) = delete;
  float time_forward(int warmup, int iters);
  std::vector<OpTime> profile(int iters);
  virtual void set_attention(int impl);
  void drop_graphs() { invalidate_graphs(); }
  size_t device_bytes() const { return ll_.arena.bytes(); }
  size_t arena_used_bytes() const { return ll_.arena.used(); }
  void palette_info(int* n_palettized, int* n_streamed, size_t* stream_bytes) const {
    *n_palettized = pal_tensors_;
    *n_streamed = pal_streamed_;
    *stream_bytes = pal_stream_bytes_;
  }
  void w8a8_info(int* n_marked, int* n_applied, size_t* bytes) const {
    *n_marked = i8_marked_;
    *n_applied = i8_applied_;
    *bytes = i8_bytes_;
  }
  int activation_range(int index, std::string* name, float* absmax);
  const std::vector<std::string>& w8a8_applied() const { return i8_names_; }
  const sd_unet_config& config() const { return cfg_; }

 protected:
  Net(const sd_unet_config& cfg, const WeightStore& ws, int device);
  void open(int device) { ll_.open(device); }
  void seal();
  void close() { ll_.close(); }

  Tensor new_tensor(int B, int H, int W, int C);
  half_t* upload_conv_weight(const std::string& name, int cout, int cin, int k, bool geglu);
  float* upload_conv_weight_f32(const std::string& name, int cout, int cin, int k);
  float* upload_vec(const std::string& name, int n, bool geglu = false);
  Tensor conv(std::vector<Op>& ops, const std::string& name, const Tensor& x, const ConvArgs& a);
  Tensor conv_w(std::vector<Op>& ops, const std::string& name, const ConvWeights& w, const float* bias, const Tensor& x, const ConvArgs& a);
  WeightPin weight_plan(const std::string& name, const Tensor& x, const ConvArgs& a, bool ln) const;
  ConvWeights upload_compressed(const std::string& name, const WeightPin& pin, int cin, const ConvArgs& a, const std::string& ln_name = std::string());
  bool observes_geglu(const std::string& name, const Tensor& x, const ConvArgs& a, bool ln) const;
  void observe_tensor(std::vector<Op>& ops, const std::string& name, const Tensor& t);
  void conv_small_n(std::vector<Op>& ops, const std::string& name, const Tensor& x, int cout, half_t* out_nhwc, float* out_nchw);
  Tensor group_norm(std::vector<Op>& ops, const std::string& name, const Tensor& x, const Tensor* x2, float eps,
                    bool silu, const ConvDesc* side = nullptr, const std::string& side_label = std::string(), double side_flop = 0);
  Tensor resnet(std::vector<Op>& ops, const std::string& p, const Tensor& x, const Tensor* x2, int cout, const float* temb);

  void run_ops(const std::vector<Op>& ops) { run_ops_on(ops, ll_.stream); }
  void run_ops_on(const std::vector<Op>& ops, hipStream_t s);
  virtual void run_eager() { run_ops(ll_.ops); }
  void run_forward();
  virtual void invalidate_graphs();
  virtual std::vector<const std::vector<Op>*> forward_lists() const { return {&ll_.ops}; }

  sd_unet_config cfg_;
  const WeightStore* ws_ = nullptr;
  bool f32_ = false;
  LaunchList ll_;
  bool have_inputs_ = false;

 private:
  ConvDesc conv_shape(const std::string& name, const Tensor& x, const ConvArgs& a) const;
  int pal_tensors_ = 0, pal_streamed_ = 0;
  size_t pal_stream_bytes_ = 0;
  int i8_marked_ = 0, i8_applied_ = 0;
  size_t i8_bytes_ = 0;
  std::vector<std::pair<std::string, float*>> observed_;
  std::vector<std::string> i8_names_;
  Tensor conv_f32(std::vector<Op>& ops, const std::string& name, const Tensor& x, const ConvArgs& a);
  Tensor group_norm_f32(std::vector<Op>& ops, const std::string& name, const Tensor& x, float eps, bool silu);
};

struct EventList {
  std::vector<hipEvent_t> ev;
  explicit EventList(size_t n) {
    ev.reserve(n);
    for (size_t i = 0; i < n; ++i) {
      hipEvent_t e = nullptr;
      SD_HIP(hipEventCreate(&e));
      ev.push_back(e);
    }
  }
  ~EventList() {
    for (hipEvent_t e : ev) (void)hipEventDestroy(e);
  }
  hipEvent_t operator[](size_t i) const { return ev[i]; }
};

}

struct sd_unet {
  std::unique_ptr<sd::Net> impl;
};
```

### ml-stable-diffusion_amd/csrc/unet.cpp

```cpp
#include "unet.h"
#include "conv_plan.h"
#include "weight_prep.h"

#ifndef SD_GN_QKV_DEFAULT
#define SD_GN_QKV_DEFAULT 1
#endif

#include <algorithm>
#include <cmath>
#include <cstdlib>
#include <cstring>

namespace sd {

namespace {

const sd_unet_config& checked_size(const sd_unet_config& cfg) {
  if (!cfg.is_controlnet && cfg.n_levels >= 1 && cfg.n_levels <= SD_MAX_LEVELS) {
    const int q = 1 << (cfg.n_levels - 1);
    SD_REQUIRE(cfg.height % q == 0 && cfg.width % q == 0, kInvalidArgument,
               "latent size %dx%d: a UNet of %d levels needs height and width that divide by %d", cfg.height, cfg.width, cfg.n_levels, q);
  }
  return cfg;
}
// ... 599 lines not shown
    }
  }

  Tensor h;
  if (cn) {
    in_cond_ = ll_.arena.alloc_n<half_t>((size_t)B * 3 * H * 8 * W * 8);
    Tensor c = new_tensor(B, H * 8, W * 8, 3);
    {
      half_t* src = in_cond_;
      Tensor cc = c;
      cond_ops_.push_back([=](hipStream_t s) { launch_nchw_to_nhwc(src, 0, cc.p, B, 3, cc.H, cc.W, s); });
    }
    const std::string p = "controlnet_cond_embedding";
    int ch = (int)ws_->get(p + ".conv_in.weight").shape[0];
    Tensor e = conv(cond_ops_, p + ".conv_in", c, {.cout = ch, .k = 3, .silu_out = true});
    for (int i = 0; ws_->has(p + ".blocks." + std::to_string(i) + ".weight"); ++i) {
      const int co = (int)ws_->get(p + ".blocks." + std::to_string(i) + ".weight").shape[0];
      e = conv(cond_ops_, p + ".blocks." + std::to_string(i), e, {.cout = co, .k = 3, .stride = 1 + (i % 2), .silu_out = true});
    }
    e = conv(cond_ops_, p + ".conv_out", e, {.cout = C0, .k = 3});
    SD_REQUIRE(e.H == H && e.W == W, kInvalidArgument, "controlnet_cond must be 8x the latent size");
    h = conv(ll_.ops, "conv_in", x_in_, {.cout = C0, .k = 3, .res = e.p});
  } else {
    h = conv(ll_.ops, "conv_in", x_in_, {.cout = C0, .k = 3});
  }

  std::vector<Tensor> skips;
  down_and_mid(ll_.ops, h, skips);

  for (auto& t : skips) res_shapes_.push_back({t.B, t.C, t.H, t.W});
  res_shapes_.push_back({h.B, h.C, h.H, h.W});

  if (cn) {
    for (size_t i = 0; i < skips.size(); ++i)
      cn_out_.push_back(conv(ll_.ops, "controlnet_down_blocks." + std::to_string(i), skips[i], {.cout = skips[i].C}));
    cn_out_.push_back(conv(ll_.ops, "controlnet_mid_block", h, {.cout = h.C}));
    for (auto& t : cn_out_) {
      float* o = ll_.arena.alloc_n<float>(t.numel());
      res_out_.push_back(o);
      Tensor tt = t;
      out_ops_.push_back([=](hipStream_t s) { launch_nhwc_to_nchw_f32(tt.p, o, tt.B, tt.C, tt.H, tt.W, s); });
    }
    finalize_temb();
  } else {
    if (cfg_.support_controlnet) {
      std::vector<Tensor> added;
      for (size_t i = 0; i < res_shapes_.size(); ++i) {
        const auto& sh = res_shapes_[i];
        half_t* src = ll_.arena.alloc_n<half_t>((size_t)sh[0] * sh[1] * sh[2] * sh[3]);
        in_res_nchw_.push_back(src);
        Tensor r = new_tensor(sh[0], sh[2], sh[3], sh[1]);
        const Tensor base = (i + 1 == res_shapes_.size()) ? h : skips[i];
        Tensor sum = new_tensor(sh[0], sh[2], sh[3], sh[1]);
        ll_.ops.push_back([=](hipStream_t s) {
          if (attached_.empty()) {
            launch_nchw_to_nhwc(src, 0, r.p, r.B, r.C, r.H, r.W, s);
            launch_add_half(base.p, r.p, sum.p, r.numel(), s);
          } else {
            const half_t* srcs[4] = {base.p, nullptr, nullptr, nullptr};
            for (size_t k = 0; k < attached_.size(); ++k) srcs[1 + k] = attached_[k]->cn_out_[i].p;
            launch_sum_half(srcs, 1 + (int)attached_.size(), sum.p, r.numel(), s);
          }
        });
        ll_.ops.back().label = "controlnet residual add " + std::to_string(i);
        if (cn_join_pos_ < 0) cn_join_pos_ = (int)ll_.ops.size() - 1;
        added.push_back(sum);
      }
      for (size_t i = 0; i < skips.size(); ++i) skips[i] = added[i];
      h = added.back();
    }
    for (int i = 0; i < n; ++i) {
      const int lvl = n - 1 - i;
      const int cout = cfg_.block_out_channels[lvl];
      const std::string p = "up_blocks." + std::to_string(i);
      for (int j = 0; j < cfg_.layers_per_block + 1; ++j) {
        Tensor skip = skips.back();
        skips.pop_back();
        h = time_resnet(ll_.ops, p + ".resnets." + std::to_string(j), h, &skip, cout);
        if (cfg_.up_cross_attn[i])
          h = transformer(ll_.ops, p + ".attentions." + std::to_string(j), h, cfg_.attention_head_dim[lvl],
                          cfg_.transformer_layers_per_block[lvl]);
      }
      if (i != n - 1)
        h = conv(ll_.ops, p + ".upsamplers.0.conv", h, {.cout = cout, .k = 3, .up = 2});
    }
    SD_REQUIRE(skips.empty(), kInternal, "skip stack not empty");
    Tensor t = group_norm(ll_.ops, "conv_norm_out", h, nullptr, cfg_.norm_eps, true);
    noise_pred_ = ll_.arena.alloc_n<float>((size_t)B * cfg_.out_channels * H * W);
    float* np = noise_pred_;
    if (cfg_.out_channels <= 8 && t.C % 8 == 0) {
      conv_small_n(ll_.ops, "conv_out", t, cfg_.out_channels, nullptr, np);
    } else {
      ConvDesc d;
      d.x0 = t.p;
      d.C0 = t.C;
      d.w = upload_conv_weight("conv_out", cfg_.out_channels, t.C, 3, false);
      d.bias = upload_vec("conv_out.bias", cfg_.out_channels);
      d.B = B; d.Hi = H; d.Wi = W; d.Ho = H; d.Wo = W;
      d.ksize = 3; d.stride = 1; d.up = 1; d.N = cfg_.out_channels;
      Tensor o = new_tensor(B, H, W, cfg_.out_channels);
      d.out = o.p;
      ll_.ops.push_back([=](hipStream_t s) {
        launch_conv_generic(d, 0, s);
        launch_nhwc_to_nchw_f32(o.p, np, o.B, o.C, o.H, o.W, s);
      });
    }
    finalize_temb();
  }

  {
    half_t* w = temb_w_all_;
    float* b = temb_b_all_;
    float* emb = emb_;
    float* out = temb_all_;
    const int N = temb_used_;
    time_ops_.push_back([=](hipStream_t s) { launch_gemv(w, b, emb, tdim, out, kTembCap, B, N, tdim, 1, 0, 0, s); });
    time_ops_.back().label = "time_emb_proj of all resnets: one batched GEMV N=" + std::to_string(N);
  }
}

void UNet::invalidate_graphs() {
  Net::invalidate_graphs();
  if (loop_graph_) { (void)hipGraphExecDestroy(loop_graph_); loop_graph_ = nullptr; }
}

void UNet::set_attention(int impl) {
  Net::set_attention(impl);
  for (UNet* cn : attached_) cn->set_attention(impl);
}

void UNet::run_main(bool with_time) {
  if (with_time) run_ops(time_ops_);
  for (size_t i = 0; i < ll_.ops.size(); ++i) {
    if (cn_forked_ && (int)i == cn_join_pos_) {
      SD_HIP(hipStreamWaitEvent(ll_.stream, ev_cn_join_, 0));
      cn_forked_ = false;
    }
    static const bool poison = tune_env_set("SD_POISON_LDS");
    if (poison) launch_lds_poison(ll_.stream);
    ll_.ops[i](ll_.stream);
  }
  SD_REQUIRE(!cn_forked_, kInternal, "forked ControlNets were never joined");
}

void UNet::attach_controlnets(const std::vector<UNet*>& cns) {
  SD_REQUIRE(!cfg_.is_controlnet, kInvalidArgument, "attach_controlnets needs a UNet handle");
  SD_REQUIRE(cns.empty() || cfg_.support_controlnet, kInvalidArgument,
             "this UNet was built without support_controlnet (unet.py:1009-1022)");
  SD_REQUIRE(cns.size() <= 3, kUnsupported, "at most 3 ControlNets per UNet handle, got %zu", cns.size());
  for (UNet* cn : cns) {
    SD_REQUIRE(cn && cn->cfg_.is_controlnet, kInvalidArgument, "attach_controlnets: handle is not a ControlNet");
    SD_REQUIRE(cn->ll_.device == ll_.device, kInvalidArgument, "ControlNet lives on device %d, UNet on %d", cn->ll_.device, ll_.device);
    SD_REQUIRE(cn->cfg_.batch == cfg_.batch && cn->cfg_.height == cfg_.height && cn->cfg_.width == cfg_.width &&
                   cn->cfg_.cross_attention_dim == cfg_.cross_attention_dim && cn->cfg_.context_len == cfg_.context_len,
               kInvalidArgument, "ControlNet static shapes differ from the UNet's");
    SD_REQUIRE(cn->res_shapes_ == res_shapes_, kInvalidArgument, "ControlNet residual shapes differ from the UNet's skips");
  }
  SD_HIP(hipSetDevice(ll_.device));
  SD_HIP(hipStreamSynchronize(ll_.stream));
  for (UNet* old : attached_)
    if (std::find(cns.begin(), cns.end(), old) == cns.end()) old->have_cond_ = false;
  attached_ = cns;
  for (UNet* cn : attached_) cn->set_attention(cfg_.attention_impl);
  invalidate_graphs();
  have_ctx_ = false;
}

// ... 309 lines not shown
```

### ml-stable-diffusion_amd/csrc/weight_prep.h

```cpp
#pragma once
#include <algorithm>
#include <cmath>
#include <cstddef>
#include <cstdint>
#include <vector>

#include "kernels.h"

namespace sd {

inline int geglu_row(int o, int n) {
  const int half_n = n / 2;
  const bool gate = o >= half_n;
  const int j = gate ? o - half_n : o;
  return (j / 32) * 64 + (gate ? 32 : 0) + (j % 32);
}

template <typename S, typename D>
void retile_ohwi(const S* src, int cout, int cin, int k, bool geglu, D* dst) {
  const int kk = k * k;
  for (int o = 0; o < cout; ++o) {
    const int dst_o = geglu ? geglu_row(o, cout) : o;
    for (int c = 0; c < cin; ++c)
      for (int t = 0; t < kk; ++t) dst[((size_t)dst_o * kk + t) * cin + c] = (D)src[((size_t)o * cin + c) * kk + t];
  }
}

template <typename W>
void fold_layernorm_rows(const W* w, const float* bias, const float* gamma, const float* beta, int cout, int cin, int row0,
                         bool geglu, half_t* w_out, float* colsum, float* bias_out) {
  for (int o = 0; o < cout; ++o) {
    const int dst = geglu ? geglu_row(o, cout) : row0 + o;
    double cs = 0.0, bb = bias ? (double)bias[o] : 0.0;
    for (int c = 0; c < cin; ++c) {
      const float wv = (float)w[(size_t)o * cin + c];
      const half_t h = gamma ? (half_t)(wv * gamma[c]) : (half_t)w[(size_t)o * cin + c];
      w_out[(size_t)dst * cin + c] = h;
      cs += (double)(float)h;
      if (beta) bb += (double)wv * (double)beta[c];
    }
    colsum[dst] = (float)cs;
    bias_out[dst] = (float)bb;
  }
}

struct PalLaneWriter {
  int nbits;
  std::vector<uint8_t> bytes;
  uint64_t window = 0;
  int held = 0;
  size_t at = 0;
  PalLaneWriter(int nbits_, int words) : nbits(nbits_), bytes((size_t)words * 16 + 8, (uint8_t)0) {}
  void put(uint64_t index) {
    window |= index << held;
    held += nbits;
    while (held >= 8) {
      bytes[at++] = (uint8_t)window;
      window >>= 8;
      held -= 8;
    }
  }
  void flush(uint8_t* wave_block, int lane) {
    if (held) bytes[at++] = (uint8_t)window;
    for (size_t q = 0; (q + 1) * 16 + 8 <= bytes.size(); ++q)
      std::copy(bytes.begin() + q * 16, bytes.begin() + (q + 1) * 16, wave_block + (q * 64 + lane) * 16);
    std::fill(bytes.begin(), bytes.end(), (uint8_t)0);
    window = 0;
    held = 0;
    at = 0;
  }
};

inline int wstream_pal_words(int taps, int nbits) { return (2 * taps * 8 * nbits + 127) / 128; }
inline size_t wstream_pal_bytes(int N, int Ctot, int ksize, int nbits) {
  return (size_t)(N / 32) * (Ctot / 32) * wstream_pal_words(ksize * ksize, nbits) * 64 * 16;
}
inline void wstream_pal_pack(const uint8_t* indices, int N, int Ctot, int ksize, int nbits, uint8_t* dst) {
  const int taps = ksize * ksize, nslices = Ctot / 32, Q = wstream_pal_words(taps, nbits), nf = 2 * taps;
  PalLaneWriter w(nbits, Q);
  for (int strip = 0; strip < N / 32; ++strip)
    for (int slice = 0; slice < nslices; ++slice)
      for (int lane = 0; lane < 64; ++lane) {
        const int n = strip * 32 + (lane & 31);
        for (int j = 0; j < nf; ++j) {
          const uint8_t* src = indices + ((size_t)n * Ctot + slice * 32 + (j & 1) * 16 + (lane >> 5) * 8) * taps + (j >> 1);
          for (int e = 0; e < 8; ++e) w.put(src[(size_t)e * taps]);
        }
        w.flush(dst + ((size_t)strip * nslices + slice) * Q * 1024, lane);
      }
}

inline double w8a8_quantize_weight(const float* w, int N, size_t per_row, int8_t* q, float* scale) {
  double err = 0.0;
  for (int n = 0; n < N; ++n) {
    const float* row = w + (size_t)n * per_row;
    float amax = 0.f;
    for (size_t i = 0; i < per_row; ++i) {
      SD_REQUIRE(std::isfinite(row[i]), kInvalidArgument, "w8a8 quantizer: row %d element %zu is not finite", n, i);
      amax = std::max(amax, std::fabs(row[i]));
    }
    const float s = amax > 0.f ? amax / 127.0f : 1.0f;
    scale[n] = s;
    for (size_t i = 0; i < per_row; ++i) {
      const float r = std::min(std::max(std::nearbyintf(row[i] / s), -127.0f), 127.0f);
      q[(size_t)n * per_row + i] = (int8_t)r;
      const double dlt = (double)row[i] - (double)r * (double)s;
      err += dlt * dlt;
// ... 134 lines not shown
```

### ml-stable-diffusion_amd/python_hip_stable_diffusion/_lib.py

```python
import ctypes as C
import os

import numpy as np

_HERE = os.path.dirname(os.path.abspath(__file__))
LIB_PATH = os.environ.get("SD_MI355X_LIB", os.path.join(os.path.dirname(_HERE), "lib", "libsdmi355.so"))

SD_MAX_LEVELS = 6
SD_FLAG_DEVICE_PTRS = 1
ATTENTION_IMPLEMENTATIONS = {"ORIGINAL": 0, "SPLIT_EINSUM": 1, "SPLIT_EINSUM_V2": 2}


class LibraryNotBuilt(ImportError):
    pass


class UNetConfig(C.Structure):
    _fields_ = [
        ("batch", C.c_int32), ("in_channels", C.c_int32), ("out_channels", C.c_int32),
        ("height", C.c_int32), ("width", C.c_int32), ("n_levels", C.c_int32),
        ("block_out_channels", C.c_int32 * SD_MAX_LEVELS),
        ("down_cross_attn", C.c_int32 * SD_MAX_LEVELS),
        ("up_cross_attn", C.c_int32 * SD_MAX_LEVELS),
        ("layers_per_block", C.c_int32),
        ("attention_head_dim", C.c_int32 * SD_MAX_LEVELS),
        ("transformer_layers_per_block", C.c_int32 * SD_MAX_LEVELS),
        ("cross_attention_dim", C.c_int32), ("context_len", C.c_int32),
        ("norm_num_groups", C.c_int32), ("norm_eps", C.c_float),
        ("flip_sin_to_cos", C.c_int32), ("freq_shift", C.c_float),
        ("addition_time_embed_dim", C.c_int32), ("projection_class_embeddings_input_dim", C.c_int32),
        ("num_time_ids", C.c_int32), ("support_controlnet", C.c_int32), ("is_controlnet", C.c_int32),
        ("is_vae_decoder", C.c_int32),
        ("attention_impl", C.c_int32), ("use_graph", C.c_int32), ("compute_fp32", C.c_int32),
    ]


class UNetIO(C.Structure):
    _fields_ = [
        ("sample", C.c_void_p), ("timestep", C.c_void_p), ("encoder_hidden_states", C.c_void_p),
        ("time_ids", C.c_void_p), ("text_embeds", C.c_void_p), ("controlnet_cond", C.c_void_p),
        ("additional_residuals", C.POINTER(C.c_void_p)), ("num_additional_residuals", C.c_int32),
        ("noise_pred", C.c_void_p), ("residual_outputs", C.POINTER(C.c_void_p)), ("flags", C.c_int32),
        ("step_noise", C.c_void_p),
    ]


class SafetyCheckerConfig(C.Structure):
    _fields_ = [("batch", C.c_int32), ("image_size", C.c_int32), ("patch_size", C.c_int32), ("hidden_size", C.c_int32),
                ("intermediate_size", C.c_int32), ("num_hidden_layers", C.c_int32), ("num_attention_heads", C.c_int32),
                ("projection_dim", C.c_int32), ("num_concepts", C.c_int32), ("num_special", C.c_int32), ("hidden_act", C.c_int32),
                ("layer_norm_eps", C.c_float), ("use_graph", C.c_int32)]


class ImagePost(C.Structure):
    _fields_ = [("resize_h", C.c_int32), ("resize_w", C.c_int32), ("image_mean", C.c_float * 3), ("image_std", C.c_float * 3)]


class TextEncoderConfig(C.Structure):
    _fields_ = [("vocab_size", C.c_int32), ("hidden_size", C.c_int32), ("intermediate_size", C.c_int32),
                ("num_hidden_layers", C.c_int32), ("num_attention_heads", C.c_int32),
                ("max_position_embeddings", C.c_int32), ("hidden_act", C.c_int32), ("projection_dim", C.c_int32),
                ("layer_norm_eps", C.c_float), ("use_graph", C.c_int32)]


ACTS = {"quick_gelu": 0, "gelu": 1}

PROGRESS_FN = C.CFUNCTYPE(C.c_int, C.c_void_p, C.c_int, C.c_int, C.POINTER(C.c_float), C.POINTER(C.c_float))

_lib = None

_P, _I, _F = C.c_void_p, C.c_int, C.c_float
_FP = C.POINTER(C.c_float)
SYMBOLS = [
    ("sd_last_error", C.c_char_p, []),
    ("sd_version", C.c_char_p, []),
    ("sd_device_count", _I, []),
    ("sd_weights_create", _I, [C.POINTER(_P)]),
    ("sd_weights_add", _I, [_P, C.c_char_p, _P, _I, C.POINTER(C.c_int64), _I]),
    ("sd_weights_load_safetensors", _I, [_P, C.c_char_p, C.c_char_p]),
    ("sd_weights_count", _I, [_P]),
    ("sd_weights_destroy", None, [_P]),
    ("sd_weights_tensor_info", _I, [_P, _I, C.c_char_p, _I, C.POINTER(C.c_int64), C.POINTER(_I)]),
    ("sd_weights_palettize", _I, [_P, C.c_char_p, _I, C.POINTER(C.c_double)]),
    ("sd_weights_add_palettized", _I, [_P, C.c_char_p, _P, _I, _P, C.POINTER(C.c_int64), _I]),
    ("sd_weights_palette_bits", _I, [_P, C.c_char_p]),
    ("sd_weights_read_palette", _I, [_P, C.c_char_p, _P, _P, _FP]),
    ("sd_weights_quantize_w8a8", _I, [_P, C.c_char_p, _F, C.POINTER(C.c_double)]),
    ("sd_weights_w8a8_info", _I, [_P, C.c_char_p, _FP]),
    ("sd_weights_observe_activations", _I, [_P, _I]),
    ("sd_weights_observe_gemms", _I, [_P, _I]),
    ("sd_weights_observe_geglus", _I, [_P, _I]),
    ("sd_unet_w8a8_info", _I, [_P, C.POINTER(_I), C.POINTER(_I), C.POINTER(C.c_size_t)]),
    ("sd_unet_w8a8_layer", _I, [_P, _I, C.c_char_p, _I]),
    ("sd_unet_activation_ranges", _I, [_P, _I, C.c_char_p, _I, _FP]),
    ("sd_op_conv2d_w8a8", _I, [_P, _P, _P, _FP, _F, _FP, _P, _P, _I, _I, _I, _I, _I, _I, _I, _I, _I, C.POINTER(_I), _I, _FP]),
    ("sd_op_w8a8_pack", _I, [_P, _I, _I, _I, _P, C.POINTER(C.c_size_t)]),
    ("sd_op_conv2d_w8a8_halo", _I, [_P, _P, _P, _FP, _F, _FP, _FP, _P, _P, _I, _I, _I, _I, _I, _I, _I, _I, _I, C.POINTER(_I), _I, _FP]),
    ("sd_op_w8a8_pack_halo", _I, [_P, _I, _I, _P, C.POINTER(C.c_size_t)]),
    ("sd_op_gemm_w8a8", _I, [_P, _P, _FP, _F, _FP, _P, _P, _I, _I, _I, _I, _I, _I, C.POINTER(_I), _I, _FP]),
    ("sd_op_w8a8_pack_gemm", _I, [_P, _I, _I, _P, C.POINTER(C.c_size_t)]),
    ("sd_op_layernorm_q8", _I, [_P, _FP, _FP, _F, _F, _P, _I, _I, _I, _FP]),
    ("sd_op_geglu_w8a8", _I, [_P, _P, _FP, _F, _FP, _P, _I, _I, _I, _I, C.POINTER(_I), _I, _FP]),
    ("sd_op_w8a8_pack_geglu", _I, [_P, _I, _I, _P, C.POINTER(C.c_size_t)]),
    ("sd_op_quantize_weight", _I, [_FP, _I, C.c_size_t, _P, _FP, C.POINTER(C.c_double)]),
    ("sd_op_absmax", _I, [_P, C.c_size_t, _FP]),
    ("sd_unet_create", _I, [C.POINTER(UNetConfig), _P, _I, C.POINTER(_P)]),
    ("sd_unet_destroy", None, [_P]),
    ("sd_unet_set_attention", _I, [_P, _I]),
    ("sd_unet_num_residuals", _I, [_P]),
    ("sd_unet_device_bytes", C.c_size_t, [_P]),
    ("sd_unet_arena_used_bytes", C.c_size_t, [_P]),
    ("sd_unet_palette_info", _I, [_P, C.POINTER(_I), C.POINTER(_I), C.POINTER(C.c_size_t)]),
    ("sd_unet_forward", _I, [_P, C.POINTER(UNetIO)]),
    ("sd_unet_time_forward", _I, [_P, _I, _I, _FP]),
    ("sd_unet_denoise_loop", _I, [_P, C.POINTER(UNetIO), _FP, _I, _I, _FP, _FP, _FP, _I, _F, _FP, _FP]),
    ("sd_unet_denoise_loop_progress", _I, [_P, C.POINTER(UNetIO), _FP, _I, _I, _FP, _FP, _FP, _I, _F, _FP, _FP, _FP, _I, _P, _P,
                                           C.POINTER(_I)]),
    ("sd_tune_set_candidate", _I, [_I, _I, _I]),
    ("sd_tune_set_plan_table", _I, [C.c_char_p, C.c_void_p, C.POINTER(C.c_int)]),
    ("sd_unet_profile", _I, [_P, _I, _I, _FP, C.POINTER(C.c_double), C.c_char_p, _I, C.POINTER(_I)]),
    ("sd_unet_attach_controlnets", _I, [_P, C.POINTER(_P), _I]),
    ("sd_controlnet_set_cond", _I, [_P, _P, _I]),
    ("sd_vae_decoder_create", _I, [C.POINTER(UNetConfig), _P, _I, C.POINTER(_P)]),
    ("sd_vae_decode", _I, [_P, _P, _I, _FP, _I]),
    ("sd_vae_encoder_create", _I, [C.POINTER(UNetConfig), _P, _I, C.POINTER(_P)]),
    ("sd_vae_encode", _I, [_P, _P, _I, _FP, _I]),
    ("sd_vae_encode_latents", _I, [_P, _P, _I, _FP, _FP, _I, _F, _F, _F, _FP, _I]),
    ("sd_text_encoder_create", _I, [_P, _P, _I, C.POINTER(_P)]),
    ("sd_text_encoder_destroy", None, [_P]),
    ("sd_text_encoder_device_bytes", C.c_size_t, [_P]),
    ("sd_text_encoder_encode", _I, [_P, C.POINTER(C.c_int32), _I, _FP, _FP, _FP]),
    ("sd_op_attention", _I, [_I, _P, _P, _P, _P, _I, _I, _I, _I, _I, _I, _I, _FP]),
    ("sd_op_layernorm", _I, [_P, _FP, _FP, _P, _I, _I, _I, _F, _I, _FP]),
    ("sd_op_groupnorm", _I, [_P, _FP, _FP, _P, _I, _I, _I, _I, _I, _F, _I, _I, _FP]),
    ("sd_op_groupnorm_shortcut", _I, [_P, _P, _FP, _FP, _P, _FP, _P, _P, _I, _I, _I, _I, _I, _I, _I, _F, _I, _I, _I, _FP]),
    ("sd_op_conv2d", _I, [_P, _P, _FP, _P, _P, _I, _I, _I, _I, _I, _I, _I, _I, _I, _I, _I, _I, _FP]),
    ("sd_op_conv2d_ex", _I, [_P, _P, _P, _FP, _FP, _P, _P, _I, _I, _I, _I, _I, _I, _I, _I, _I, _I, _I, _FP, _FP, _F, _I, _P, _I, _I, _I,
                             C.POINTER(_I), _I, _FP]),
    ("sd_op_conv2d_palettized", _I, [_P, _P, _P, _I, _P, _FP, _P, _P, _I, _I, _I, _I, _I, _I, _I, _I, _I, C.POINTER(_I), _I, _FP]),
    ("sd_op_palette_pack", _I, [_P, _I, _I, _I, _I, _P, C.POINTER(C.c_size_t)]),
    ("sd_op_gemm_palettized", _I, [_P, _P, _I, _P, _FP, _P, _P, _I, _I, _I, _I, _I, _I, C.POINTER(_I), _I, _FP]),
    ("sd_op_palette_pack_gemm", _I, [_P, _I, _I, _I, _P, C.POINTER(C.c_size_t)]),
    ("sd_op_geglu_palettized", _I, [_P, _FP, _FP, _P, _I, _P, _FP, _P, _I, _I, _I, C.c_float, _I, C.POINTER(_I), _I, _FP]),
    ("sd_op_palette_pack_geglu", _I, [_P, _I, _I, _I, _P, C.POINTER(C.c_size_t)]),
    ("sd_op_conv2d_groupnorm", _I, [_P, _P, _FP, _P, _FP, _FP, _P, _P, _I, _I, _I, _I, _I, _I, _I, _F, _I, _I, _I, C.POINTER(_I), _I, _FP]),
    ("sd_op_conv2d_groupnorm_proj", _I, [_P, _P, _FP, _P, _FP, _FP, _P, _FP, _P, _P, _I, _I, _I, _I, _I, _I, _I, _I, _F, _I, _I, C.POINTER(_I), _I, _FP]),
    ("sd_op_conv2d_groupnorm_conv3x3", _I, [_P, _P, _FP, _P, _FP, _FP, _P, _FP, _P, _P, _P, _I, _I, _I, _I, _I, _I, _I, _I, _F, _I, _I, _I, _I,
                                            C.POINTER(_I), _I, _FP]),
    ("sd_op_cross_attention_fused", _I, [_P, _FP, _FP, _P, _P, _P, _P, _I, _I, _I, _I, _F, _I, _I, _FP]),
    ("sd_op_ffn_out_proj", _I, [_P, _P, _FP, _P, _P, _FP, _P, _P, _FP, _I, _I, _I, _I, _I, _I, _FP]),
    ("sd_op_fold_linear", _I, [_P, _FP, _P, _FP, _P, _FP, _I, _I, _I]),
    ("sd_op_cross_attention_block", _I, [_P, _FP, _FP, _P, _P, _P, _P, _FP, _P, _P, _FP, _P, _I, _I, _I, _I, _F, _I, _I, _FP]),
    ("sd_op_geglu", _I, [_P, _P, _FP, _P, _I, _I, _I, _I, _FP]),
    ("sd_op_geglu_ln", _I, [_P, _FP, _FP, _P, _FP, _P, _I, _I, _I, C.c_float, _I, _I, _FP]),
    ("sd_op_qkv_ln", _I, [_P, _FP, _FP, _P, _P, _P, _I, _I, _I, C.c_float, C.c_float, _I, _I, _I, _FP]),
    ("sd_op_gn_proj_qkv", _I, [_P, _P, _FP, _FP, _P, _FP, _FP, _FP, _P, _P, _P, _P, _I, _I, _I, _I, _I, C.c_float, C.c_float, C.c_float, _I, _I,
                               C.POINTER(C.c_int), _I, _FP]),
    ("sd_op_timestep_embedding", _I, [_FP, _FP, _I, _I, _I, _F]),
    ("sd_op_posterior_noise", _I, [_FP, _FP, _FP, _FP, _I, _I, _I, _I, _F, _F, _F, _I, _FP]),
    ("sd_op_sched_step", _I, [_FP, _FP, _FP, _FP, _FP, _FP, _F, _I, _I, _I, _I, _FP, C.POINTER(_I)]),
    ("sd_op_conv_plan", _I, [_I] * 18 + [C.POINTER(C.c_int), C.POINTER(C.c_ulonglong)]),
    ("sd_op_conv_plan_kernel", _I, [_I] * 18 + [C.c_char_p, _I]),
    ("sd_numpy_randn", _I, [C.c_uint32, C.POINTER(C.c_double), C.c_size_t]),
    ("sd_torch_randn", _I, [C.c_uint32, C.POINTER(C.c_double), C.c_size_t]),
    ("sd_philox_randn", _I, [C.c_uint64, C.c_uint32, C.POINTER(C.c_double), C.c_size_t]),
    ("sd_calibrate", _I, [_I, _FP]),
    ("sd_selftest_mfma", _I, []),
    ("sd_safety_checker_create", _I, [C.POINTER(SafetyCheckerConfig), _P, _I, C.POINTER(_P)]),
    ("sd_safety_checker_destroy", None, [_P]),
    ("sd_safety_checker_device_bytes", C.c_size_t, [_P]),
    ("sd_safety_checker_last_ms", C.c_float, [_P]),
    ("sd_safety_checker_run", _I, [_P, _P, _F, _FP, _FP, _FP, _FP, _I]),
    ("sd_op_vit_attention", _I, [_P, _P, _I, _I, _I, _I, _I, _FP]),
    ("sd_op_safety_head", _I, [_FP, _FP, _FP, _FP, _FP, _F, _I, _I, _I, _I, _FP, _FP]),
    ("sd_op_vae_attention", _I, [_P, _P, _P, _P, _I, _I, _I, _I, _FP]),
    ("sd_vae_decode_images", _I, [_P, _P, _I, _FP, _P, _P, C.POINTER(ImagePost), _F, _FP, _FP, _I]),
    ("sd_op_resample_coeffs", _I, [_I, _I, C.POINTER(_I), _P, _P]),
    ("sd_op_image_rgb8", _I, [_FP, _P, _I, _I, _I, _I, _FP]),
    ("sd_op_clip_input", _I, [_P, _P, _I, _I, _I, _I, _I, _I, _FP, _FP, _I, _FP]),
    ("sd_op_conv_f32", _I, [_FP, _P, _I, _FP, _FP, _FP, _I, _I, _I, _I, _I, _I, _I, _I, _I]),
    ("sd_op_groupnorm_f32", _I, [_FP, _FP, _FP, _FP, _I, _I, _I, _I, _I, _F, _I]),
# ... 156 lines not shown
    flags = np.empty(B, np.float32)
    scores = np.empty((B, nc), np.float32)
    check(lib().sd_op_safety_head(fptr(image_embeds), fptr(concept_embeds), fptr(special_embeds), fptr(concept_w), fptr(special_w),
                                  float(adjustment), B, P, nc, ns, fptr(flags), fptr(scores)))
    return flags > 0.5, scores


def resample_coeffs(in_size, out_size):
    ksize = C.c_int(0)
    check(lib().sd_op_resample_coeffs(int(in_size), int(out_size), C.byref(ksize), None, None))
    bounds = np.zeros((out_size, 2), np.int32)
    coeffs = np.zeros((out_size, ksize.value), np.int32)
    check(lib().sd_op_resample_coeffs(int(in_size), int(out_size), C.byref(ksize), ptr(bounds), ptr(coeffs)))
    return ksize.value, bounds, coeffs


def image_rgb8(image, iters=1):
    image = f32(image)
    if image.ndim != 4 or image.shape[1] != 3:
        raise ValueError("image_rgb8: image must be (B, 3, H, W)")
    B, _, H, W = image.shape
    out = np.empty((B, H, W, 3), np.uint8)
    ms = C.c_float(0)
    check(lib().sd_op_image_rgb8(fptr(image), ptr(out), B, H, W, iters, C.byref(ms)))
    return out, ms.value


def clip_input(rgb8, rh, rw, S, mean, std, out=None, iters=1):
    rgb8 = np.ascontiguousarray(rgb8, dtype=np.uint8)
    mean, std = f32(mean), f32(std)
    if rgb8.ndim != 4 or rgb8.shape[3] != 3 or mean.shape != (3,) or std.shape != (3,):
        raise ValueError("clip_input: rgb8 must be (B, H, W, 3), mean and std three floats each")
    B, H, W, _ = rgb8.shape
    n = B * 3 * S * S
    if out is None:
        out = np.empty(n, np.float16)
    if out.dtype != np.float16 or not out.flags.c_contiguous or out.size < n:
        raise ValueError("clip_input: out must be a C-contiguous float16 buffer of at least B * 3 * S * S elements")
    ms = C.c_float(0)
    check(lib().sd_op_clip_input(ptr(rgb8), ptr(out), B, H, W, int(rh), int(rw), int(S), fptr(mean), fptr(std), iters, C.byref(ms)))
    return out.reshape(-1)[:n].reshape(B, 3, S, S), ms.value


def layernorm(x, weight, bias, eps=1e-5, iters=1):
    x, weight, bias = f16(x), f32(weight), f32(bias)
    B, Cn, _, S = x.shape
    out = np.empty_like(x)
    ms = C.c_float(0)
    check(lib().sd_op_layernorm(ptr(x), fptr(weight), fptr(bias), ptr(out), B, Cn, S, eps, iters, C.byref(ms)))
    return out, ms.value


def groupnorm(x, weight, bias, groups=32, eps=1e-5, silu=False, iters=1):
    x, weight, bias = f16(x), f32(weight), f32(bias)
    B, Cn, H, W = x.shape
    out = np.empty_like(x)
    ms = C.c_float(0)
    check(lib().sd_op_groupnorm(ptr(x), fptr(weight), fptr(bias), ptr(out), B, Cn, H, W, groups, eps, int(silu),
                                iters, C.byref(ms)))
    return out, ms.value


def conv2d(x, w, bias=None, res=None, stride=1, upsample=False, tile=0, splitk=0, force_generic=False, iters=1):
    x, w = f16(x), f16(w)
    B, Cin, H, W = x.shape
    Cout, Cin2, k, k2 = w.shape
    if Cin2 != Cin or k != k2:
        raise ValueError("conv2d: weight shape does not match input")
    up = 2 if upsample else 1
    pad = k // 2
    Ho = (H * up + 2 * pad - k) // stride + 1
    Wo = (W * up + 2 * pad - k) // stride + 1
    bias = None if bias is None else f32(bias)
    res = None if res is None else f16(res)
    if res is not None and res.shape != (B, Cout, Ho, Wo):
        raise ValueError(f"conv2d: res must be (B, Cout, Ho, Wo) = {(B, Cout, Ho, Wo)}, got {res.shape}")
    out = np.empty((B, Cout, Ho, Wo), np.float16)
    ms = C.c_float(0)
    check(lib().sd_op_conv2d(ptr(x), ptr(w), fptr(bias), ptr(res), ptr(out), B, Cin, H, W, Cout, k, stride,
                             int(upsample), tile, splitk, int(force_generic), iters, C.byref(ms)))
    return out, ms.value


def conv2d_ex(x, w, bias=None, res=None, x1=None, temb=None, stride=1, upsample=False, pad_mode=0, twin=None, tile=0, splitk=0,
              force_generic=False, iters=1):
    x, w = f16(x), f16(w)
    x1 = None if x1 is None else f16(x1)
    B, Cin, H, W = x.shape
    C1 = 0 if x1 is None else x1.shape[1]
    Cout, Ctot, k, k2 = w.shape
    if Ctot != Cin + C1 or k != k2 or (x1 is not None and x1.shape != (B, C1, H, W)):
        raise ValueError("conv2d_ex: weight / second source shape does not match input")
    up = 2 if upsample else 1
    pad = k // 2
    Ho = (H * up + (1 if pad_mode else 2 * pad) - k) // stride + 1
    Wo = (W * up + (1 if pad_mode else 2 * pad) - k) // stride + 1
    bias = None if bias is None else f32(bias)
    res = None if res is None else f16(res)
    temb = None if temb is None else f32(temb)
    if (temb is not None and temb.shape != (B, Cout)) or (res is not None and res.shape != (B, Cout, Ho, Wo)):
        raise ValueError("conv2d_ex: temb must be (B, Cout), res (B, Cout, Ho, Wo)")
    groups, gamma, beta, eps, silu = (0, None, None, 0.0, False) if twin is None else twin
    gamma = None if gamma is None else f32(gamma)
    beta = None if beta is None else f32(beta)
    out = np.empty((B, Cout, Ho, Wo), np.float16)
    out_twin = None if twin is None else np.empty_like(out)
    plan = (C.c_int * 4)()
    ms = C.c_float(0)
    check(lib().sd_op_conv2d_ex(ptr(x), ptr(x1), ptr(w), fptr(bias), fptr(temb), ptr(res), ptr(out), B, Cin, C1, H, W, Cout, k, stride,
                                int(upsample), pad_mode, groups, fptr(gamma), fptr(beta), eps, int(silu), ptr(out_twin), tile, splitk,
                                int(force_generic), plan, iters, C.byref(ms)))
    return out, out_twin, list(plan), ms.value


def conv2d_palettized(x, lut, indices, nbits, bias=None, res=None, x1=None, upsample=False, nw=0, out=None, iters=1):
    x, lut = f16(x), f16(lut)
    indices = np.ascontiguousarray(indices, dtype=np.uint8)
    x1 = None if x1 is None else f16(x1)
    B, Cin, H, W = x.shape
    C1 = 0 if x1 is None else x1.shape[1]
    if indices.ndim != 4:
        raise ValueError("conv2d_palettized: indices must be (Cout, Cin + C1, k, k)")
    Cout, Ctot, k, k2 = indices.shape
    if Ctot != Cin + C1 or k != k2 or (x1 is not None and x1.shape != (B, C1, H, W)):
        raise ValueError("conv2d_palettized: indices / second source shape does not match input")
    if nbits not in (1, 2, 4, 6, 8) or lut.shape != (1 << nbits,):
        raise ValueError("conv2d_palettized: nbits must be 1, 2, 4, 6 or 8 and lut hold 2 ** nbits entries")
    up = 2 if upsample else 1
    Ho, Wo = H * up, W * up
    bias = None if bias is None else f32(bias)
    res = None if res is None else f16(res)
    if res is not None and res.shape != (B, Cout, Ho, Wo):
        raise ValueError("conv2d_palettized: res must be (B, Cout, Ho, Wo)")
    n = B * Cout * Ho * Wo
    if out is None:
        out = np.empty(n, np.float16)
    if out.dtype != np.float16 or not out.flags.c_contiguous or out.size < n:
        raise ValueError("conv2d_palettized: out must be a C-contiguous float16 buffer of at least B * Cout * Ho * Wo elements")
    plan = (C.c_int * 4)()
    ms = C.c_float(0)
    check(lib().sd_op_conv2d_palettized(ptr(x), ptr(x1), ptr(lut), nbits, ptr(indices), fptr(bias), ptr(res), ptr(out), B, Cin, C1, H, W,
                                        Cout, k, int(upsample), nw, plan, iters, C.byref(ms)))
    return out.reshape(-1)[:n].reshape(B, Cout, Ho, Wo), list(plan), ms.value


def conv2d_w8a8(x, wq, w_scale, act_absmax, bias=None, res=None, x1=None, upsample=False, nw=0, out=None, iters=1):
    x = f16(x)
    wq = np.ascontiguousarray(wq, dtype=np.int8)
    w_scale = f32(w_scale)
    x1 = None if x1 is None else f16(x1)
    B, Cin, H, W = x.shape
    C1 = 0 if x1 is None else x1.shape[1]
    if wq.ndim != 4:
        raise ValueError("conv2d_w8a8: wq must be (Cout, Cin + C1, k, k)")
    Cout, Ctot, k, k2 = wq.shape
    if Ctot != Cin + C1 or k != k2 or (x1 is not None and x1.shape != (B, C1, H, W)) or w_scale.shape != (Cout,):
        raise ValueError("conv2d_w8a8: wq / w_scale / second source shape does not match input")
    up = 2 if upsample else 1
    Ho, Wo = H * up, W * up
    bias = None if bias is None else f32(bias)
    res = None if res is None else f16(res)
    if res is not None and res.shape != (B, Cout, Ho, Wo):
        raise ValueError("conv2d_w8a8: res must be (B, Cout, Ho, Wo)")
    n = B * Cout * Ho * Wo
    if out is None:
        out = np.empty(n, np.float16)
# ... 669 lines not shown
```

Before: 242.3 it/s.

## Fold nearest-upsample 3x3 convs into four 2x2 sub-pixel phase convolutions

Adds a sub-pixel convolution path for the UNet's upsampler convs. Weights are pre-folded into four phase-specific 2x2 kernels, and a new halo-ring MFMA kernel reads the low-resolution input directly. This drops the redundant taps of a 3x3 conv over a nearest-upsampled image, cutting MACs from 9 to 4 per output, and skips materialising the upsampled input. In exchange it adds a new kernel with its own pipelining and wait-count logic, and sums fp16 weights on the host, which could overflow for extreme values (the fold checks for this).

```diff
diff --git a/include/sd_mi355x.h b/include/sd_mi355x.h
--- a/include/sd_mi355x.h
+++ b/include/sd_mi355x.h
@@ -183,6 +183,10 @@
                            const float* temb, const void* res, void* out, int B, int Cin, int C1, int H, int W, int Cout, int upsample,
                            int staging, int splitk, int* plan_out, int iters, float* ms);
 int sd_op_w8a8_pack_halo(const int8_t* wq, int Cout, int Ctot, int8_t* packed, size_t* bytes);
+int sd_op_subpixel_fold(const void* w, int w_f32, int Cout, int Cin, void* folded, size_t* halves);
+int sd_op_subpixel_refusal(int ksize, int stride, int up, int C0, int C1, int N, int B, int Hi, int Wi, int out_mode, char* text, int text_bytes);
+int sd_op_conv2d_subpixel(const void* x, const void* w, const float* bias, const void* res, void* out, int B, int Cin, int H, int W, int Cout,
+                          int splitk, int staging, int* plan_out, int iters, float* ms);
 int sd_op_gemm_w8a8(const void* x, const int8_t* wq, const float* w_scale, float act_absmax, const float* bias, const void* res, void* out, int B,
                     int Cin, int H, int W, int Cout, int bm, int* plan_out, int iters, float* ms);
 int sd_op_w8a8_pack_gemm(const int8_t* wq, int Cout, int K, int8_t* packed, size_t* bytes);
diff --git a/ml-stable-diffusion_amd/csrc/capi_ops.cpp b/ml-stable-diffusion_amd/csrc/capi_ops.cpp
--- a/ml-stable-diffusion_amd/csrc/capi_ops.cpp
+++ b/ml-stable-diffusion_amd/csrc/capi_ops.cpp
@@ -535,6 +535,68 @@
   });
 }
 
+int sd_op_subpixel_fold(const void* w, int w_f32, int Cout, int Cin, void* folded, size_t* halves) {
+  return guarded([&] {
+    SD_REQUIRE(w && halves, kInvalidArgument, "NULL argument");
+    SD_REQUIRE(Cout > 0 && Cin > 0, kInvalidArgument, "subpixel_fold: Cout %d Cin %d", Cout, Cin);
+    *halves = subpixel_fold_halves(Cout, Cin);
+    if (!folded) return;
+    if (w_f32) subpixel_fold(reinterpret_cast<const float*>(w), Cout, Cin, reinterpret_cast<half_t*>(folded));
+    else subpixel_fold(f16(w), Cout, Cin, reinterpret_cast<half_t*>(folded));
+  });
+}
+
+int sd_op_subpixel_refusal(int ksize, int stride, int up, int C0, int C1, int N, int B, int Hi, int Wi, int out_mode, char* text, int text_bytes) {
+  return guarded([&] {
+    SD_REQUIRE(text && text_bytes >= 1, kInvalidArgument, "bad subpixel_refusal arguments");
+    static const half_t present = 0;
+    ConvDesc d;
+    d.C0 = C0;
+    if (C1 > 0) d.x1 = &present, d.C1 = C1;
+    d.B = B; d.Hi = Hi; d.Wi = Wi;
+    d.Ho = stride > 0 ? Hi * up / stride : 0; d.Wo = stride > 0 ? Wi * up / stride : 0;
+    d.ksize = ksize; d.stride = stride; d.up = up; d.N = N; d.out_mode = out_mode;
+    const char* why = halo_sp_refusal(d);
+    const std::string line = why ? why : "";
+    SD_REQUIRE((int)line.size() < text_bytes, kInvalidArgument, "subpixel_refusal: the text buffer holds %d bytes, the line needs %zu", text_bytes, line.size() + 1);
+    memcpy(text, line.c_str(), line.size() + 1);
+  });
+}
+
+int sd_op_conv2d_subpixel(const void* x, const void* w, const float* bias, const void* res, void* out, int B, int Cin, int H, int W, int Cout, int splitk,
+                          int staging, int* plan_out, int iters, float* ms) {
+  return guarded([&] {
+    SD_REQUIRE(x && w && out && plan_out, kInvalidArgument, "NULL argument");
+    SD_REQUIRE(B > 0 && Cin > 0 && Cout > 0 && H > 0 && W > 0 && splitk >= 0 && staging >= 0 && staging <= 5 && staging != 1, kInvalidArgument,
+               "conv2d_subpixel: empty problem, splitk %d or staging %d (plan tile 7's ring codes 0, 2-5)", splitk, staging);
+    ConvDesc d;
+    d.C0 = Cin;
+    d.B = B; d.Hi = H; d.Wi = W; d.Ho = 2 * H; d.Wo = 2 * W;
+    d.ksize = 3; d.up = 2; d.N = Cout;
+    d.subpix = true;
+    d.staging = staging;
+    d.splitk = splitk;
+    SD_REQUIRE(conv_fast_path_ok(d) && halo_sp_ok(d), kInvalidArgument, "conv2d_subpixel: plan tile 21 (conv3x3_halo_sp.hip) does not take this shape: %s (Cin=%d Cout=%d %dx%d)",
+               halo_sp_refusal(d) ? halo_sp_refusal(d) : "off the MFMA path", Cin, Cout, H, W);
+    std::vector<half_t> folded(subpixel_fold_halves(Cout, Cin));
+    subpixel_fold(f16(w), Cout, Cin, folded.data());
+    Scratch sc;
+    d.x0 = upload_nhwc(sc, x, B, Cin, H, W);
+    d.w = sc.dev<half_t>(folded.size(), folded.data());
+    d.bias = bias ? sc.dev<float>(Cout, bias) : nullptr;
+    if (res) d.res = upload_nhwc(sc, res, B, Cout, d.Ho, d.Wo);
+    const size_t n_out = (size_t)B * d.Ho * d.Wo * Cout;
+    half_t* dout = guarded_buf<half_t>(sc, n_out, kOpGuard);
+    d.out = dout;
+    const ConvPlan p = conv_plan(d);
+    plan_out[0] = p.tile; plan_out[1] = p.staging; plan_out[2] = p.splitk; plan_out[3] = p.slab ? 1 : 0;
+    ConvWorkspace ws = workspace_for(sc, {d});
+    sc.timed(iters, ms, [&] { launch_conv(d, ws, sc.stream); });
+    check_guard(sc, dout, n_out, kOpGuard, "conv2d_subpixel");
+    download_nchw(dout, out, B, Cout, d.Ho, d.Wo);
+  });
+}
+
 int sd_op_gemm_w8a8(const void* x, const int8_t* wq, const float* w_scale, float act_absmax, const float* bias, const void* res, void* out, int B,
                     int Cin, int H, int W, int Cout, int bm, int* plan_out, int iters, float* ms) {
   return guarded([&] {
@@ -1332,6 +1394,7 @@
   if (flags & 8) d.gn_partial = const_cast<float*>(present), d.gn_groups = 32;
   if (flags & 16) d.bias = present;
   if (flags & 32) d.pad = 0;
+  if (flags & 64) d.subpix = true;
   if (n_trans > 0) d.out_t = const_cast<half_t*>(ph), d.n_trans = n_trans, d.ldT = Ho * Wo;
   d.n_twins = n_twins;
   if (gnf_groups > 0) {
diff --git a/ml-stable-diffusion_amd/csrc/conv3x3_halo_sp.hip b/ml-stable-diffusion_amd/csrc/conv3x3_halo_sp.hip
--- /dev/null
+++ b/ml-stable-diffusion_amd/csrc/conv3x3_halo_sp.hip
@@ -0,0 +1,363 @@
+#include "igemm_device.h"
+#include "halo_ring.h"
+
+namespace sd {
+
+namespace {
+
+constexpr int SP_TAPS = 4;
+constexpr int sp_mod4(int t) { return ((t % SP_TAPS) + SP_TAPS) % SP_TAPS; }
+constexpr int sp_x_issued(int tap) { return sp_mod4(tap) < 2 ? HALO_PPW / 2 : 0; }
+static_assert(2 * (HALO_PPW / 2) == HALO_PPW, "the halo pieces of a wave go out in two equal steps");
+
+template <int D, int WR>
+constexpr int sp_wait_count(int tap) {
+  int n = 0;
+  for (int i = 2; i <= D - 1; ++i) n += WR + sp_x_issued(tap - D + i);
+  const int halo = 2 * WR + sp_x_issued(2);
+  if (tap == SP_TAPS - 1 && n > halo) n = halo;
+  return n;
+}
+template <int D, int WR>
+constexpr int sp_wait_count_last(int tap) {
+  int n = 0;
+  for (int u = tap - D + 2; u <= tap - 1; ++u) n += (u < 0 || u + D < SP_TAPS) ? WR : 0;
+  return n;
+}
+template <int D, int WR>
+constexpr bool sp_counts_ok() {
+  for (int t = 0; t < SP_TAPS; ++t) {
+    if (sp_wait_count<D, WR>(t) > 63 || sp_wait_count<D, WR>(t) < 1) return false;
+    if (sp_wait_count_last<D, WR>(t) > 63) return false;
+  }
+  return true;
+}
+
+struct HaloSpArgs {
+  IgemmArgs a;
+  int phase_outer;
+};
+
+template <int D>
+__global__ __launch_bounds__(256, halo_lds_bytes(64, D) <= 80 * 1024 ? 2 : 1) void conv3x3_halo_sp_kernel(HaloSpArgs ha) {
+  const IgemmArgs& a = ha.a;
+  constexpr int BN = 64, BM = 128, WR = 2, ROWB = BK * 2;
+  static_assert(D >= 3 && D <= SP_TAPS, "rings of 3 or 4 stages: a weight tile goes out at most one chunk ahead");
+  static_assert(sp_counts_ok<D, WR>() && (D - 1) * WR <= 63, "vmcnt range");
+  static_assert(halo_lds_bytes(64, D) >= 32 * 1024 + BM * (BN + 8) * 2 + BN * 4, "epilogue buffers fit the K-loop buffers");
+  extern __shared__ __attribute__((aligned(16))) char smem[];
+  char* const Xh = smem;
+  char* const Ws = smem + 2 * HALO_LDS_ROWS * ROWB;
+  float* const sconst = reinterpret_cast<float*>(Ws + D * BN * ROWB);
+
+  const int tid = threadIdx.x, lane = tid & 63;
+  const int wave = __builtin_amdgcn_readfirstlane(tid >> 6);
+  const int wm = wave >> 1, wk = wave & 1;
+  const int H = a.Hi, W = a.Wi;
+  const int Ho = a.Ho, Wo = a.Wo;
+
+  const int n_tiles = (a.N + BN - 1) / BN;
+  const int sp_tiles = a.B * a.tiles_y * a.tiles_x;
+  const int m_tiles = 4 * sp_tiles;
+  const int nwg = m_tiles * n_tiles;
+  int bid = blockIdx.x;
+  {
+    int q = nwg >> 3, r = nwg & 7, xcd = bid & 7, idx = bid >> 3;
+    int base = (xcd < r) ? xcd * (q + 1) : r * (q + 1) + (xcd - r) * q;
+    bid = base + idx;
+  }
+  const int bn_idx = a.n_fast ? bid % n_tiles : bid / m_tiles, mt = a.n_fast ? bid / n_tiles : bid % m_tiles;
+  const int phase = ha.phase_outer ? mt / sp_tiles : mt & 3;
+  const int st_idx = ha.phase_outer ? mt - phase * sp_tiles : mt >> 2;
+  const int pa = phase >> 1, pb = phase & 1;
+  const int b = st_idx / (a.tiles_y * a.tiles_x);
+  const int trem = st_idx - b * (a.tiles_y * a.tiles_x);
+  const int ty = trem / a.tiles_x, tx = trem - ty * a.tiles_x;
+  const int y0 = ty * 8, x0 = tx * 16;
+  const int n_blk = bn_idx * BN;
+
+  const int nch = a.Ctot / BK;
+  const int split = blockIdx.y;
+  const int ch_begin = split * a.nk_per_split;
+  int ch_end = ch_begin + a.nk_per_split;
+  if (ch_end > nch) ch_end = nch;
+
+  constexpr unsigned kOob = 0x80000000u;
+  const __amdgpu_buffer_rsrc_t rs_w =
+      __builtin_amdgcn_make_buffer_rsrc(const_cast<half_t*>(a.w), 0, (int)((size_t)4 * a.N * a.K * 2), 0x00020000);
+  const __amdgpu_buffer_rsrc_t rs_x =
+      __builtin_amdgcn_make_buffer_rsrc(const_cast<half_t*>(a.x0), 0, (int)((size_t)a.B * H * W * a.C0 * 2), 0x00020000);
+  unsigned hoff[HALO_PPW];
+  auto piece_of = [&](int j) { return (wave + 4 * j < HALO_PIECES) ? wave + 4 * j : HALO_PIECES - 1; };
+#pragma unroll
+  for (int j = 0; j < HALO_PPW; ++j) {
+    const int p = piece_of(j);
+    const int hr = 8 * p + (lane >> 3);
+    const int hy = hr / HALO_W, hx = hr - hy * HALO_W;
+    const int iy = y0 - 1 + hy, ix = x0 - 1 + hx;
+    const bool ok = (hr < HALO_ROWS) && iy >= 0 && iy < H && ix >= 0 && ix < W;
+    const unsigned pix = (unsigned)((b * H + iy) * W + ix);
+    const unsigned sw = (unsigned)(((lane & 7) ^ ((hx >> 1) & 7)) * 16);
+    hoff[j] = ok ? pix * (unsigned)a.C0 * 2u + sw : kOob;
+  }
+  const int pchunk = tid & 7, lrow = tid >> 3;
+  const int wchunk = pchunk ^ ((lrow >> 1) & 7);
+  unsigned woff[WR];
+#pragma unroll
+  for (int i = 0; i < WR; ++i) {
+    int n = n_blk + lrow + 32 * i;
+    if (n > a.N - 1) n = a.N - 1;
+    woff[i] = (unsigned)(phase * a.N + n) * (unsigned)a.K * 2u + (unsigned)wchunk * 16u;
+  }
+  auto issue_x_piece = [&](int j, int ch, int xstage) {
+    char* dst = Xh + xstage * (HALO_LDS_ROWS * ROWB) + piece_of(j) * 1024;
+    dma16_to_lds(rs_x, dst, hoff[j], ch * BK * 2);
+  };
+  int iw_koff = ch_begin * BK * 2, iw_tap = 0, iw_step = 0;
+  auto issue_next_w = [&]() {
+    char* ws = Ws + ((unsigned)iw_step % D) * (BN * ROWB) + wave * 1024;
+#pragma unroll
+    for (int i = 0; i < WR; ++i)
+      dma16_to_lds(rs_w, ws + i * 4096, woff[i], iw_koff);
+    ++iw_step;
+    iw_koff += a.Ctot * 2;
+    if (++iw_tap == SP_TAPS) {
+      iw_tap = 0;
+      iw_koff += (BK - SP_TAPS * a.Ctot) * 2;
+    }
+  };
+
+  floatx16 acc[2][2];
+#pragma unroll
+  for (int i = 0; i < 2; ++i)
+#pragma unroll
+    for (int j = 0; j < 2; ++j)
+#pragma unroll
+      for (int r = 0; r < 16; ++r) acc[i][j][r] = 0.f;
+
+  const int frow = lane & 31, hi = lane >> 5;
+  int hrb[2];
+#pragma unroll
+  for (int i = 0; i < 2; ++i) {
+    const int ml = (wm * 2 + i) * 32 + frow;
+    hrb[i] = ((ml >> 4) * HALO_W + (ml & 15)) * ROWB;
+  }
+  const int hx0 = frow & 15;
+  int xsw[2][2], wsw[2];
+#pragma unroll
+  for (int s = 0; s < 2; ++s) {
+    const int kc = 2 * (2 * wk + s) + hi;
+#pragma unroll
+    for (int dx = 0; dx < 2; ++dx) xsw[dx][s] = (kc ^ (((hx0 + pb + dx) >> 1) & 7)) * 16;
+    wsw[s] = frow * ROWB + (kc ^ ((frow >> 1) & 7)) * 16;
+  }
+  int toffb[SP_TAPS];
+#pragma unroll
+  for (int t = 0; t < SP_TAPS; ++t) toffb[t] = ((pa + (t >> 1)) * HALO_W + pb + (t & 1)) * ROWB;
+
+  float const_b = 0.f, const_t = 0.f;
+  if (!a.slab && tid < BN && n_blk + tid < a.N) {
+    if (a.bias) const_b = a.bias[n_blk + tid];
+    if (a.temb) const_t = a.temb[(size_t)b * a.temb_stride + n_blk + tid];
+  }
+
+  auto read_step = [&](half8 (&xf)[2][2], half8 (&wf)[2][2], const char* xs, const char* ws, int tap) {
+#pragma unroll
+    for (int s = 0; s < 2; ++s) {
+#pragma unroll
+      for (int i = 0; i < 2; ++i) xf[s][i] = *reinterpret_cast<const half8*>(xs + hrb[i] + toffb[tap] + xsw[tap & 1][s]);
+#pragma unroll
+      for (int j = 0; j < 2; ++j) wf[s][j] = *reinterpret_cast<const half8*>(ws + j * 32 * ROWB + wsw[s]);
+    }
+  };
+  auto mfma_step = [&](half8 (&xf)[2][2], half8 (&wf)[2][2]) {
+#pragma unroll
+    for (int s = 0; s < 2; ++s)
+#pragma unroll
+      for (int i = 0; i < 2; ++i)
+#pragma unroll
+        for (int j = 0; j < 2; ++j) acc[i][j] = __builtin_amdgcn_mfma_f32_32x32x16_f16(wf[s][j], xf[s][i], acc[i][j], 0, 0, 0);
+  };
+
+  half8 xfA[2][2], wfA[2][2], xfB[2][2], wfB[2][2];
+  if (ch_begin < ch_end) {
+#pragma unroll
+    for (int j = 0; j < HALO_PPW; ++j) issue_x_piece(j, ch_begin, 0);
+#pragma unroll
+    for (int p = 0; p < D; ++p) {
+      asm volatile("" ::: "memory");
+      issue_next_w();
+    }
+    wait_vmcnt_barrier<(D - 1) * WR>();
+    read_step(xfA, wfA, Xh, Ws, 0);
+  }
+  int st = 0;
+  auto chunk = [&](auto last, int ch) {
+    constexpr bool LAST = decltype(last)::value;
+    const int xst = (ch - ch_begin) & 1;
+    auto step = [&](auto tap_c, half8 (&cx)[2][2], half8 (&cw)[2][2], half8 (&nx)[2][2], half8 (&nw)[2][2]) {
+      constexpr int tap = decltype(tap_c)::value;
+      if constexpr (LAST && tap == SP_TAPS - 1) {
+        mfma_step(cx, cw);
+      } else {
+        asm volatile("s_waitcnt lgkmcnt(0)" ::: "memory");
+        wait_vmcnt_barrier<LAST ? sp_wait_count_last<D, WR>(tap) : sp_wait_count<D, WR>(tap)>();
+        constexpr int tapn = tap == SP_TAPS - 1 ? 0 : tap + 1;
+        const char* xs = Xh + (tap == SP_TAPS - 1 ? xst ^ 1 : xst) * (HALO_LDS_ROWS * ROWB);
+        const char* ws = Ws + ((unsigned)(st + 1) % D) * (BN * ROWB);
+        read_step(nx, nw, xs, ws, tapn);
+        constexpr int nx_pieces = LAST ? 0 : sp_x_issued(tap);
+        constexpr bool w_live = !LAST || tap + D < SP_TAPS;
+#pragma unroll
+        for (int j = 0; j < nx_pieces; ++j) issue_x_piece(tap * (HALO_PPW / 2) + j, ch + 1, xst ^ 1);
+        asm volatile("" ::: "memory");
+        if constexpr (w_live) issue_next_w();
+        mfma_step(cx, cw);
+        constexpr int nv = nx_pieces + (w_live ? WR : 0);
+#pragma unroll
+        for (int g = 0; g < 4; ++g) {
+          __builtin_amdgcn_sched_group_barrier(0x008, 1, 0);
+          __builtin_amdgcn_sched_group_barrier(0x100, 2, 0);
+        }
+        __builtin_amdgcn_sched_group_barrier(0x008, 1, 0);
+        if constexpr (nv >= 1) __builtin_amdgcn_sched_group_barrier(0x010, nv >= 4 ? 2 : 1, 0);
+        __builtin_amdgcn_sched_group_barrier(0x008, 1, 0);
+        if constexpr (nv >= 2) __builtin_amdgcn_sched_group_barrier(0x010, nv >= 5 ? 2 : 1, 0);
+        __builtin_amdgcn_sched_group_barrier(0x008, 1, 0);
+        if constexpr (nv >= 3) __builtin_amdgcn_sched_group_barrier(0x010, 1, 0);
+        __builtin_amdgcn_sched_group_barrier(0x008, 1, 0);
+      }
+      ++st;
+      __builtin_amdgcn_sched_barrier(0);
+    };
+    step(std::integral_constant<int, 0>{}, xfA, wfA, xfB, wfB);
+    step(std::integral_constant<int, 1>{}, xfB, wfB, xfA, wfA);
+    step(std::integral_constant<int, 2>{}, xfA, wfA, xfB, wfB);
+    step(std::integral_constant<int, 3>{}, xfB, wfB, xfA, wfA);
+  };
+  if (ch_begin < ch_end) {
+    int ch = ch_begin;
+    for (; ch + 1 < ch_end; ++ch) chunk(std::false_type{}, ch);
+    chunk(std::true_type{}, ch);
+  }
+  asm volatile("s_waitcnt vmcnt(0) lgkmcnt(0)" ::: "memory");
+  __syncthreads();
+
+  {
+    floatx4* red = reinterpret_cast<floatx4*>(smem);
+#pragma unroll
+    for (int j = 0; j < 2; ++j)
+#pragma unroll
+      for (int q = 0; q < 4; ++q) {
+        floatx4 v;
+#pragma unroll
+        for (int e = 0; e < 4; ++e) v[e] = wk ? acc[0][j][4 * q + e] : acc[1][j][4 * q + e];
+        red[((wave * 2 + j) * 4 + q) * 64 + lane] = v;
+      }
+    if (tid < BN) sconst[tid] = const_b + const_t;
+    __syncthreads();
+  }
+  floatx16 fin[2];
+  {
+    const floatx4* red = reinterpret_cast<const floatx4*>(smem);
+#pragma unroll
+    for (int j = 0; j < 2; ++j)
+#pragma unroll
+      for (int q = 0; q < 4; ++q) {
+        const floatx4 v = red[(((wave ^ 1) * 2 + j) * 4 + q) * 64 + lane];
+#pragma unroll
+        for (int e = 0; e < 4; ++e) fin[j][4 * q + e] = (wk ? acc[1][j][4 * q + e] : acc[0][j][4 * q + e]) + v[e];
+      }
+  }
+  const int ml = (wm * 2 + wk) * 32 + frow;
+  if (a.slab) {
+    const int y = y0 + (ml >> 4), x = x0 + (ml & 15);
+    if (y < H && x < W) {
+      const int m = (b * Ho + 2 * y + pa) * Wo + 2 * x + pb;
+      float* prow = a.partial + ((size_t)split * a.M + m) * a.N;
+#pragma unroll
+      for (int j = 0; j < 2; ++j)
+#pragma unroll
+        for (int q = 0; q < 4; ++q) {
+          const int n = n_blk + j * 32 + 8 * q + 4 * hi;
+          if (n < a.N) {
+            floatx4 v = {fin[j][4 * q], fin[j][4 * q + 1], fin[j][4 * q + 2], fin[j][4 * q + 3]};
+            out_store(reinterpret_cast<floatx4*>(prow + n), v);
+          }
+        }
+    }
+    return;
+  }
+  constexpr int OROW = BN + 8;
+  half_t* ot = reinterpret_cast<half_t*>(smem + 32 * 1024);
+#pragma unroll
+  for (int j = 0; j < 2; ++j)
+#pragma unroll
+    for (int q = 0; q < 4; ++q) {
+      const int nl = j * 32 + 8 * q + 4 * hi;
+      const floatx4 bb = *reinterpret_cast<const floatx4*>(sconst + nl);
+      half4 o = {(half_t)(fin[j][4 * q] + bb[0]), (half_t)(fin[j][4 * q + 1] + bb[1]), (half_t)(fin[j][4 * q + 2] + bb[2]),
+                 (half_t)(fin[j][4 * q + 3] + bb[3])};
+      *reinterpret_cast<half4*>(ot + ml * OROW + nl) = o;
+    }
+  __syncthreads();
+  constexpr int WC = BN / 8;
+  for (int idx = tid; idx < BM * WC; idx += 256) {
+    const int r = idx / WC, c = idx - r * WC;
+    const int y = y0 + (r >> 4), x = x0 + (r & 15);
+    const int n = n_blk + c * 8;
+    if (y < H && x < W && n < a.N) {
+      const size_t m = (size_t)(b * Ho + 2 * y + pa) * Wo + 2 * x + pb;
+      half8 v = *reinterpret_cast<const half8*>(ot + r * OROW + c * 8);
+      half_t* dst = a.out + m * a.N + n;
+      if (n + 8 <= a.N) {
+        if (a.res) {
+          const half8 rr = *reinterpret_cast<const half8*>(a.res + m * a.N + n);
+#pragma unroll
+          for (int e = 0; e < 8; ++e) v[e] = (half_t)((float)v[e] + (float)rr[e]);
+        }
+        out_store(reinterpret_cast<half8*>(dst), v);
+      } else {
+        for (int e = 0; e < a.N - n; ++e) dst[e] = a.res ? (half_t)((float)v[e] + (float)a.res[m * a.N + n + e]) : v[e];
+      }
+    }
+  }
+}
+
+template <int D>
+void launch_halo_sp_d(const HaloSpArgs& ha, hipStream_t s) {
+  constexpr size_t lds = halo_lds_bytes(64, D);
+  static_assert(lds <= 80 * 1024, "two workgroups per CU");
+  auto k = conv3x3_halo_sp_kernel<D>;
+  static DynLdsOnce once;
+  once.set(k, lds);
+  const IgemmArgs& a = ha.a;
+  dim3 grid(4 * a.B * a.tiles_x * a.tiles_y * cdiv(a.N, 64), a.splitk);
+  hipLaunchKernelGGL(k, grid, dim3(256), lds, s, ha);
+}
+
+}
+
+int launch_halo_sp(const ConvDesc& d, const ConvPlan& p, float* partial, hipStream_t s) {
+  SD_REQUIRE(d.subpix && halo_sp_refusal(d) == nullptr && d.w && p.kernel == ConvKernel::HaloSubpix, kInvalidArgument,
+             "plan tile 21 (conv3x3_halo_sp.hip): %s", halo_sp_refusal(d) ? halo_sp_refusal(d) : "not a sub-pixel plan");
+  HaloSpArgs ha;
+  ha.a = planned_args(d, p, partial);
+  IgemmArgs& a = ha.a;
+  a.K = SP_TAPS * a.Ctot;
+  a.tiles_x = cdiv(d.Wi, 16);
+  a.tiles_y = cdiv(d.Hi, 8);
+  a.nk_total = a.Ctot / BK;
+  a.nk_per_split = cdiv(a.nk_total, p.splitk);
+  a.n_fast = choose_tile_order(2.0 * a.B * a.Hi * a.Wi * a.Ctot, 2.0 * a.N * a.K, 4.0 * a.B * a.tiles_x * a.tiles_y, (double)cdiv(a.N, 64), true);
+  static const int phase_outer = tune_env_int("SD_SUBPIX_PHASE_OUTER", 0);
+  ha.phase_outer = phase_outer != 0;
+  switch (p.stages) {
+    case 3: launch_halo_sp_d<3>(ha, s); break;
+    case 4: launch_halo_sp_d<4>(ha, s); break;
+    default: SD_REQUIRE(false, kInternal, "sub-pixel halo conv: no kernel with a ring of %d stages", p.stages);
+  }
+  return 0;
+}
+
+}
diff --git a/ml-stable-diffusion_amd/csrc/conv_plan.cpp b/ml-stable-diffusion_amd/csrc/conv_plan.cpp
--- a/ml-stable-diffusion_amd/csrc/conv_plan.cpp
+++ b/ml-stable-diffusion_amd/csrc/conv_plan.cpp
@@ -210,6 +210,44 @@
          d.C0 % BK == 0 && c1 % BK == 0 && d.N % 4 == 0;
 }
 
+const char* halo_sp_refusal(const ConvDesc& d) {
+  if (d.x1) return "a second source";
+  if (d.ksize != 3) return "not a 3x3 conv";
+  if (d.stride != 1) return "stride is not 1";
+  if (d.up != 2) return "no nearest-x2 upsample (up is not 2)";
+  if (d.pad >= 0) return "explicit padding";
+  if (d.out_mode != kOutHalf) return "the output mode is not plain fp16 (GEGLU / transposed)";
+  if (d.ln_colsum || d.out_t) return "a LayerNorm fold / fused q|k|v epilogue";
+  if (d.Ho != 2 * d.Hi || d.Wo != 2 * d.Wi) return "the output is not twice the input";
+  if (d.Hi < 8) return "Hi < 8";
+  if (d.Wi < 8) return "Wi < 8";
+  if (d.C0 % BK != 0) return "C0 is no multiple of 64";
+  if (d.N % 4 != 0) return "N is no multiple of 4";
+  if (d.gnf_partial) return "GroupNorm in the loader";
+  if (d.n_twins > 0) return "GroupNorm twins";
+  if (d.cw.kind != WeightSource::Fp16) return "a compressed weight source";
+  if (d.debug) return "an ablation build";
+  const size_t lim = (size_t)1 << 31;
+  if ((size_t)d.B * d.Hi * d.Wi * d.C0 * 2 >= lim || (size_t)16 * d.N * d.C0 * 2 >= lim) return "an operand of 2 GiB or more";
+  return nullptr;
+}
+
+bool subpixel_wanted(const ConvDesc& d) {
+  static const int mode = tune_env_int("SD_UP_SUBPIX", 1);
+  if (mode == 0 || !halo_sp_ok(d)) return false;
+  const int M = d.B * d.Ho * d.Wo;
+  static const int only_m = tune_env_int("SD_UP_SUBPIX_M", 0);
+  if (mode >= 2) return only_m == 0 || only_m == M;
+  struct Shape { int ctot, n, m; };
+  static const Shape kMeasured[] = {
+      {1280, 1280, 2048},
+      {640, 640, 8192},
+      {0, 0, 0}};
+  for (const Shape& s : kMeasured)
+    if (s.ctot == d.C0 && s.n == d.N && s.m == M && s.ctot != 0) return true;
+  return false;
+}
+
 bool gemm_pipe_ok(int ksize, int stride, int up, int M, int N, int K, int C0, int C1) {
   const size_t lim = (size_t)1 << 31;
   return ksize == 1 && stride == 1 && up == 1 && (size_t)M * std::max(C0, C1) * 2 < lim && (size_t)N * K * 2 < lim;
@@ -226,6 +264,18 @@
 }
 
 namespace {
+
+int subpix_splits(const ConvDesc& d, const Dims& a) {
+  const int steps = a.Ctot / BK;
+  int s = d.splitk;
+  if (s == 0) {
+    const long blocks = 4L * d.B * cdiv(d.Wi, 16) * cdiv(d.Hi, 8) * cdiv(a.N, 64);
+    s = 1;
+    while (blocks * s < 192 && s < 16 && steps / (s * 2) >= 2) s *= 2;
+  }
+  s = std::min(std::max(s, 1), steps);
+  return cdiv(steps, cdiv(steps, s));
+}
 
 ConvPlan plan_codes(const ConvDesc& d) {
   const CompressedWeights& cw = d.cw;
@@ -241,6 +291,17 @@
     SD_REQUIRE(conv_fast_path_ok(d) && cw.stream && cw.scale && d.staging >= 0 && d.staging <= 2 && smgeglu_i8_shape_ok(d, d.staging), kInvalidArgument,
                "plan tile 20 (smgeglu_i8.hip, int8) needs the int8 weights, the scales and an un-folded shape of the GEGLU kernel with K <= %d "
                "(k=%d C0=%d C1=%d N=%d M=%d mode=%d ln=%d)", kSmI8MaxK, d.ksize, d.C0, d.x1 ? d.C1 : 0, d.N, d.B * d.Ho * d.Wo, d.out_mode, d.ln_colsum ? 1 : 0);
+  if (d.subpix) {
+    SD_REQUIRE(conv_fast_path_ok(d) && halo_sp_ok(d) && (d.tile == 0 || d.tile == 21), kInvalidArgument,
+               "plan tile 21 (conv3x3_halo_sp.hip) does not take this conv: %s (k=%d stride=%d up=%d C0=%d C1=%d N=%d %dx%d tile=%d)",
+               halo_sp_refusal(d) ? halo_sp_refusal(d) : "another tile is pinned", d.ksize, d.stride, d.up, d.C0, d.x1 ? d.C1 : 0, d.N, d.Hi, d.Wi, d.tile);
+    const Dims a = dims_of(d);
+    ConvPlan r{21, d.staging ? d.staging : 3, 1, false, 0};
+    r.splitk = subpix_splits(d, a);
+    r.slab = r.splitk > 1;
+    r.workspace_bytes = slab_bytes(a, r.splitk, r.slab);
+    return r;
+  }
   if (!conv_fast_path_ok(d)) return ConvPlan{-1, 0, 1, false, 0};
   switch (cw.kind) {
     case WeightSource::Fp16: break;
@@ -353,6 +414,12 @@
     p.stages = code >= 3 ? 4 : code == 2 ? 3 : 2;
     return;
   }
+  if (p.tile == 21) {
+    tile_dims(7, p.bm, p.bn);
+    p.kernel = ConvKernel::HaloSubpix;
+    p.stages = code == 2 ? 3 : 4;
+    return;
+  }
   tile_dims(p.tile, p.bm, p.bn);
   if (p.tile == 7) {
     p.kernel = ConvKernel::HaloKs;
@@ -409,6 +476,7 @@
     case ConvKernel::GemmPipe: return "gemm_pipe " + tile + ring;
     case ConvKernel::HaloKs: return "halo_ks" + ring;
     case ConvKernel::HaloI8: return "halo_i8" + ring;
+    case ConvKernel::HaloSubpix: return "conv3x3_halo_sp" + ring;
     case ConvKernel::Wstream: return "wstream waves" + std::to_string(p.waves);
     case ConvKernel::WstreamPal: return "wstream_pal waves" + std::to_string(p.waves);
     case ConvKernel::WstreamI8: return "wstream_i8 waves" + std::to_string(p.waves);
@@ -427,6 +495,7 @@
 size_t conv_workspace_bytes(const ConvDesc& d) {
   if (!conv_fast_path_ok(d) || pal_gemm(d) || pal_geglu(d) || i8_gemm(d) || i8_geglu(d)) return 0;
   const Dims a = dims_of(d);
+  if (d.subpix) return halo_sp_ok(d) ? slab_bytes(a, subpix_splits(d, a), false) : 0;
   const Plan p = choose_plan(d, a);
   int splits = (switches().tuning && can_split(d)) ? std::max(p.splitk, 16) : p.splitk;
   const bool stream = can_stream(d) || ((pal_stream(d) || i8_stream(d)) && can_split(d) && wstream_shape_ok(d));
@@ -436,7 +505,7 @@
 
 ConvWeightCopies conv_plan_copies(const ConvDesc& d0) {
   ConvWeightCopies c{false, false, false};
-  if (!conv_fast_path_ok(d0)) return c;
+  if (!conv_fast_path_ok(d0) || d0.subpix) return c;
   ConvDesc d = d0;
   d.w_tiled = d.w_ws = d.w_bv = nullptr;
   const Switches& sw = switches();
@@ -560,6 +629,9 @@
   else if (p.tile == 18)
     fprintf(stderr, "[sd conv] k%d s%d up%d C0=%d C1=%d M=%d N=%d K=%d mode=%d tile=%d splitk=%d bits=8\n", d.ksize, d.stride, d.up, d.C0, c1, a.M, a.N,
             a.K, d.out_mode, p.tile, p.splitk);
+  else if (p.tile == 21)
+    fprintf(stderr, "[sd conv] k%d s%d up%d C0=%d C1=%d M=%d N=%d K=%d mode=%d tile=%d splitk=%d subpix K'=%d\n", d.ksize, d.stride, d.up, d.C0, c1, a.M,
+            a.N, a.K, d.out_mode, p.tile, p.splitk, 4 * a.Ctot);
   else
     fprintf(stderr, "[sd conv] k%d s%d up%d C0=%d C1=%d M=%d N=%d K=%d mode=%d tile=%d splitk=%d\n", d.ksize, d.stride, d.up, d.C0, c1, a.M, a.N,
             a.K, d.out_mode, p.tile, p.splitk);
diff --git a/ml-stable-diffusion_amd/csrc/conv_plan.h b/ml-stable-diffusion_amd/csrc/conv_plan.h
--- a/ml-stable-diffusion_amd/csrc/conv_plan.h
+++ b/ml-stable-diffusion_amd/csrc/conv_plan.h
@@ -5,7 +5,7 @@
 
 namespace sd {
 
-enum class ConvKernel { Generic, Igemm, GemmPipe, HaloKs, HaloI8, Wstream, WstreamPal, WstreamI8, Wsgemm, Bvgemm, Smgemm, SmgemmPal, SmgemmI8, Smgeglu, SmgegluPal, SmgegluI8 };
+enum class ConvKernel { Generic, Igemm, GemmPipe, HaloKs, HaloI8, HaloSubpix, Wstream, WstreamPal, WstreamI8, Wsgemm, Bvgemm, Smgemm, SmgemmPal, SmgemmI8, Smgeglu, SmgegluPal, SmgegluI8 };
 
 struct ConvPlan {
   int tile;
@@ -47,6 +47,9 @@
 
 constexpr int kConvBK = 64;
 bool halo_ks_ok(const ConvDesc& d);
+const char* halo_sp_refusal(const ConvDesc& d);
+inline bool halo_sp_ok(const ConvDesc& d) { return halo_sp_refusal(d) == nullptr; }
+bool subpixel_wanted(const ConvDesc& d);
 bool gemm_pipe_ok(int ksize, int stride, int up, int M, int N, int K, int C0, int C1);
 
 constexpr size_t kLdsBudget = 160 * 1024;
diff --git a/ml-stable-diffusion_amd/csrc/igemm.hip b/ml-stable-diffusion_amd/csrc/igemm.hip
--- a/ml-stable-diffusion_amd/csrc/igemm.hip
+++ b/ml-stable-diffusion_amd/csrc/igemm.hip
@@ -1032,6 +1032,7 @@
       break;
     case ConvKernel::HaloKs: gn_entries = launch_halo_ks(d, p, ws.partial, s); break;
     case ConvKernel::HaloI8: gn_entries = launch_halo_i8(d, p, ws.partial, s); break;
+    case ConvKernel::HaloSubpix: gn_entries = launch_halo_sp(d, p, ws.partial, s); break;
     case ConvKernel::Igemm:
     case ConvKernel::GemmPipe: {
       const bool trans = d.out_mode == kOutHalfT;
diff --git a/ml-stable-diffusion_amd/csrc/igemm_device.h b/ml-stable-diffusion_amd/csrc/igemm_device.h
--- a/ml-stable-diffusion_amd/csrc/igemm_device.h
+++ b/ml-stable-diffusion_amd/csrc/igemm_device.h
@@ -13,6 +13,7 @@
 
 int launch_halo_ks(const ConvDesc& d, const ConvPlan& p, float* partial, hipStream_t s);
 int launch_halo_i8(const ConvDesc& d, const ConvPlan& p, float* partial, hipStream_t s);
+int launch_halo_sp(const ConvDesc& d, const ConvPlan& p, float* partial, hipStream_t s);
 
 namespace {
 
diff --git a/ml-stable-diffusion_amd/csrc/kernels.h b/ml-stable-diffusion_amd/csrc/kernels.h
--- a/ml-stable-diffusion_amd/csrc/kernels.h
+++ b/ml-stable-diffusion_amd/csrc/kernels.h
@@ -78,6 +78,7 @@
   const half_t* w_bv = nullptr;
   GnTwin twin[2];
   int n_twins = 0;
+  bool subpix = false;
 };
 
 constexpr int kGnMaxSlabs = 256;
diff --git a/ml-stable-diffusion_amd/csrc/net.cpp b/ml-stable-diffusion_amd/csrc/net.cpp
--- a/ml-stable-diffusion_amd/csrc/net.cpp
+++ b/ml-stable-diffusion_amd/csrc/net.cpp
@@ -41,6 +41,17 @@
   retile_ohwi(t.data.data(), cout, cin, k, geglu, host.data());
   half_t* d = ll_.arena.alloc_n<half_t>(expect);
   SD_HIP(hipMemcpy(d, host.data(), expect * sizeof(half_t), hipMemcpyHostToDevice));
+  return d;
+}
+
+half_t* Net::upload_subpixel_weight(const std::string& name, int cout, int cin) {
+  const HostTensor& t = ws_->get(name + ".weight");
+  const size_t expect = (size_t)cout * cin * 9;
+  SD_REQUIRE(t.numel() == expect, kInvalidArgument, "%s.weight has %zu elements, expected %zu (%d,%d,3,3)", name.c_str(), t.numel(), expect, cout, cin);
+  std::vector<half_t> host(subpixel_fold_halves(cout, cin));
+  subpixel_fold(t.data.data(), cout, cin, host.data());
+  half_t* d = ll_.arena.alloc_n<half_t>(host.size());
+  SD_HIP(hipMemcpy(d, host.data(), host.size() * sizeof(half_t), hipMemcpyHostToDevice));
   return d;
 }
 
@@ -99,6 +110,7 @@
     ops.back().label = "absmax " + name;
   }
   if (pin.kind != WeightSource::Fp16) return conv_w(ops, name, upload_compressed(name, pin, cin, a), b, x, a);
+  if (a.subpix && !a.silu_out && subpixel_wanted(conv_shape(name, x, a))) return conv_w(ops, name, ConvWeights(upload_subpixel_weight(name, a.cout, cin), true), b, x, a);
   return conv_w(ops, name, upload_conv_weight(name, a.cout, cin, a.k, geglu), b, x, a);
 }
 
@@ -246,6 +258,7 @@
   d.tile = weights.pin.tile;
   d.staging = weights.pin.staging;
   d.splitk = weights.pin.splitk;
+  d.subpix = weights.subpix;
   Tensor out;
   if (ln && a.n_trans > 0) {
     out = new_tensor(x.B, d.Ho, d.Wo, a.n_trans);
@@ -310,7 +323,7 @@
   const int kind = d.out_t ? 3 : (geglu ? 2 : (ln ? 1 : 0));
   const WeightSource src = d.cw.kind;
   const std::string lnmark = ln ? "+ln" : "", palmark = "+pal" + std::to_string(d.cw.bits);
-  const std::string mark = src == WeightSource::PalGeglu ? palmark + lnmark : lnmark + (d.cw.i8() ? "+w8a8" : src != WeightSource::Fp16 ? palmark : "");
+  const std::string mark = d.subpix ? "+subpix" : src == WeightSource::PalGeglu ? palmark + lnmark : lnmark + (d.cw.i8() ? "+w8a8" : src != WeightSource::Fp16 ? palmark : "");
   snprintf(buf, sizeof(buf), "%s%s %d->%d @%dx%d M=%d K=%d %s #%d,%d,%d,%d,%d,%d,%d",
            k == 3 ? "conv3x3" : (geglu ? (src == WeightSource::PalGeglu ? "geglu" : "geglu1x1") : "gemm1x1"), mark.c_str(), cin, cout, d.Ho, d.Wo,
            x.B * d.Ho * d.Wo, cin * k * k, name.c_str(), kind, k, a.stride, a.up, cin, cout, x.B * d.Ho * d.Wo);
diff --git a/ml-stable-diffusion_amd/csrc/net.h b/ml-stable-diffusion_amd/csrc/net.h
--- a/ml-stable-diffusion_amd/csrc/net.h
+++ b/ml-stable-diffusion_amd/csrc/net.h
@@ -59,6 +59,7 @@
   float q_scale = 1.f;
   int q_cols = 0;
   bool keep_compressed = false;
+  bool subpix = false;
   const int8_t* x_i8 = nullptr;
 };
 
@@ -66,7 +67,8 @@
   const half_t* w = nullptr;
   CompressedWeights cw;
   WeightPin pin;
-  ConvWeights(const half_t* fp16) : w(fp16) {}
+  bool subpix = false;
+  ConvWeights(const half_t* fp16, bool folded = false) : w(fp16), subpix(folded) {}
   ConvWeights(const CompressedWeights& c, const WeightPin& p) : cw(c), pin(p) {}
 };
 
@@ -103,6 +105,7 @@
   Tensor new_tensor(int B, int H, int W, int C);
   half_t* upload_conv_weight(const std::string& name, int cout, int cin, int k, bool geglu);
   float* upload_conv_weight_f32(const std::string& name, int cout, int cin, int k);
+  half_t* upload_subpixel_weight(const std::string& name, int cout, int cin);
   float* upload_vec(const std::string& name, int n, bool geglu = false);
   Tensor conv(std::vector<Op>& ops, const std::string& name, const Tensor& x, const ConvArgs& a);
   Tensor conv_w(std::vector<Op>& ops, const std::string& name, const ConvWeights& w, const float* bias, const Tensor& x, const ConvArgs& a);
diff --git a/ml-stable-diffusion_amd/csrc/unet.cpp b/ml-stable-diffusion_amd/csrc/unet.cpp
--- a/ml-stable-diffusion_amd/csrc/unet.cpp
+++ b/ml-stable-diffusion_amd/csrc/unet.cpp
@@ -705,7 +705,7 @@
                           cfg_.transformer_layers_per_block[lvl]);
       }
       if (i != n - 1)
-        h = conv(ll_.ops, p + ".upsamplers.0.conv", h, {.cout = cout, .k = 3, .up = 2});
+        h = conv(ll_.ops, p + ".upsamplers.0.conv", h, {.cout = cout, .k = 3, .up = 2, .subpix = true});
     }
     SD_REQUIRE(skips.empty(), kInternal, "skip stack not empty");
     Tensor t = group_norm(ll_.ops, "conv_norm_out", h, nullptr, cfg_.norm_eps, true);
diff --git a/ml-stable-diffusion_amd/csrc/weight_prep.h b/ml-stable-diffusion_amd/csrc/weight_prep.h
--- a/ml-stable-diffusion_amd/csrc/weight_prep.h
+++ b/ml-stable-diffusion_amd/csrc/weight_prep.h
@@ -23,6 +23,32 @@
     const int dst_o = geglu ? geglu_row(o, cout) : o;
     for (int c = 0; c < cin; ++c)
       for (int t = 0; t < kk; ++t) dst[((size_t)dst_o * kk + t) * cin + c] = (D)src[((size_t)o * cin + c) * kk + t];
+  }
+}
+
+inline size_t subpixel_fold_halves(int cout, int cin) { return (size_t)16 * cout * cin; }
+inline int subpixel_first(int phase_bit, int d) { return phase_bit == 0 ? d : 2 * d; }
+inline int subpixel_count(int phase_bit, int d) { return (phase_bit == 0) == (d == 0) ? 1 : 2; }
+template <typename S>
+void subpixel_fold(const S* src, int cout, int cin, half_t* dst) {
+  SD_REQUIRE(src && dst && cout > 0 && cin > 0, kInvalidArgument, "subpixel_fold: Cout %d Cin %d", cout, cin);
+  for (int p = 0; p < 4; ++p) {
+    const int a = p >> 1, b = p & 1;
+    for (int o = 0; o < cout; ++o)
+      for (int t = 0; t < 4; ++t) {
+        const int dy = t >> 1, dx = t & 1;
+        const int ky0 = subpixel_first(a, dy), nky = subpixel_count(a, dy), kx0 = subpixel_first(b, dx), nkx = subpixel_count(b, dx);
+        half_t* row = dst + (((size_t)p * cout + o) * 4 + t) * cin;
+        for (int c = 0; c < cin; ++c) {
+          const S* w9 = src + ((size_t)o * cin + c) * 9;
+          float s = 0.f;
+          for (int ky = ky0; ky < ky0 + nky; ++ky)
+            for (int kx = kx0; kx < kx0 + nkx; ++kx) s += (float)w9[ky * 3 + kx];
+          SD_REQUIRE(std::fabs(s) <= 65504.0f, kInvalidArgument, "subpixel_fold: the folded weight of output %d input %d phase %d tap %d is %g, outside fp16",
+                     o, c, p, t, (double)s);
+          row[c] = (half_t)s;
+        }
+      }
   }
 }
 
diff --git a/ml-stable-diffusion_amd/python_hip_stable_diffusion/_lib.py b/ml-stable-diffusion_amd/python_hip_stable_diffusion/_lib.py
--- a/ml-stable-diffusion_amd/python_hip_stable_diffusion/_lib.py
+++ b/ml-stable-diffusion_amd/python_hip_stable_diffusion/_lib.py
@@ -97,6 +97,9 @@
     ("sd_op_w8a8_pack", _I, [_P, _I, _I, _I, _P, C.POINTER(C.c_size_t)]),
     ("sd_op_conv2d_w8a8_halo", _I, [_P, _P, _P, _FP, _F, _FP, _FP, _P, _P, _I, _I, _I, _I, _I, _I, _I, _I, _I, C.POINTER(_I), _I, _FP]),
     ("sd_op_w8a8_pack_halo", _I, [_P, _I, _I, _P, C.POINTER(C.c_size_t)]),
+    ("sd_op_subpixel_fold", _I, [_P, _I, _I, _I, _P, C.POINTER(C.c_size_t)]),
+    ("sd_op_subpixel_refusal", _I, [_I, _I, _I, _I, _I, _I, _I, _I, _I, _I, C.c_char_p, _I]),
+    ("sd_op_conv2d_subpixel", _I, [_P, _P, _FP, _P, _P, _I, _I, _I, _I, _I, _I, _I, C.POINTER(_I), _I, _FP]),
     ("sd_op_gemm_w8a8", _I, [_P, _P, _FP, _F, _FP, _P, _P, _I, _I, _I, _I, _I, _I, C.POINTER(_I), _I, _FP]),
     ("sd_op_w8a8_pack_gemm", _I, [_P, _I, _I, _P, C.POINTER(C.c_size_t)]),
     ("sd_op_layernorm_q8", _I, [_P, _FP, _FP, _F, _F, _P, _I, _I, _I, _FP]),
@@ -419,6 +422,44 @@
     return out, ms.value
 
 
+def subpixel_fold(w):
+    w = np.ascontiguousarray(w)
+    if w.dtype not in (np.float16, np.float32) or w.ndim != 4 or w.shape[2:] != (3, 3):
+        raise ValueError("subpixel_fold: w must be (Cout, Cin, 3, 3) float16 or float32")
+    Cout, Cin = w.shape[:2]
+    out = np.empty((4, Cout, 4, Cin), np.float16)
+    n = C.c_size_t(0)
+    check(lib().sd_op_subpixel_fold(ptr(w), int(w.dtype == np.float32), Cout, Cin, ptr(out), C.byref(n)))
+    assert n.value == out.size
+    return out
+
+
+def subpixel_refusal(C0, N, B, Hi, Wi, ksize=3, stride=1, up=2, C1=0, out_mode=0):
+    text = C.create_string_buffer(128)
+    check(lib().sd_op_subpixel_refusal(ksize, stride, up, C0, C1, N, B, Hi, Wi, out_mode, text, len(text)))
+    return text.value.decode()
+
+
+def conv2d_subpixel(x, w, bias=None, res=None, splitk=0, staging=0, iters=1):
+    x, w = f16(x), f16(w)
+    B, Cin, H, W = x.shape
+    if w.ndim != 4 or w.shape[1:] != (Cin, 3, 3):
+        raise ValueError("conv2d_subpixel: w must be (Cout, Cin, 3, 3)")
+    Cout = w.shape[0]
+    bias = None if bias is None else f32(bias)
+    res = None if res is None else f16(res)
+    if bias is not None and bias.shape != (Cout,):
+        raise ValueError("conv2d_subpixel: bias must be (Cout,)")
+    if res is not None and res.shape != (B, Cout, 2 * H, 2 * W):
+        raise ValueError(f"conv2d_subpixel: res must be (B, Cout, 2H, 2W) = {(B, Cout, 2 * H, 2 * W)}, got {res.shape}")
+    out = np.empty((B, Cout, 2 * H, 2 * W), np.float16)
+    plan = (C.c_int * 4)()
+    ms = C.c_float(0)
+    check(lib().sd_op_conv2d_subpixel(ptr(x), ptr(w), fptr(bias), ptr(res), ptr(out), B, Cin, H, W, Cout, splitk, staging, plan, iters,
+                                      C.byref(ms)))
+    return out, list(plan), ms.value
+
+
 def conv2d_ex(x, w, bias=None, res=None, x1=None, temb=None, stride=1, upsample=False, pad_mode=0, twin=None, tile=0, splitk=0,
               force_generic=False, iters=1):
     x, w = f16(x), f16(w)
```

After: 245.0 it/s (median of 6 runs). +1.1%, better.
